# Tony-Tseng/deep-rawburst-sr

Hardware: AMD Instinct MI355X
Metric: bursts/sec 14x48x48 RAW->4x (SyntheticBurstVal shape), DBSR forward (higher is better)
Workload: dtype fp16; 1 GPU; configs[1]: SyntheticBurstVal 14-frame 48x48 -> 384x384 (sr x8 of RAW, x4 of full-res), batch 8 per GPU, full PWC-Net + warp + fusion + decoder; global_batch=8, frames=14, height=48, width=48, out_size=384, parallelism=dp1 (independent bursts per rank), hip_graph=True, fusion_weights_written=True

## Files before the change

deep-rawburst-sr_amd/_lib.py:

```python
import ctypes
import os

import torch

_HERE = os.path.dirname(os.path.abspath(__file__))
LIB_PATH = os.environ.get('DBSR_HIP_LIB', os.path.join(_HERE, 'libdbsr_hip.so'))

DBSR_F32, DBSR_BF16, DBSR_F16 = 0, 1, 2
ACT_NONE, ACT_RELU, ACT_LRELU = 0, 1, 2
OUT_NHWC, OUT_SHUFFLE, OUT_NCHW_F32 = 0, 1, 2
ABI_VERSION = 23
SRC_F32_NCHW, SRC_U8_NHWC = 0, 1
POST_GAINS, POST_CCM, POST_GAMMA, POST_SMOOTHSTEP = 1, 2, 4, 8
LS_SCALE, LS_GROWTH_TRACKER, LS_FOUND_INF, LS_ADAM_STEP, LS_SKIPPED, LS_WORDS = 0, 1, 2, 3, 4, 8


class FrameMap(ctypes.Structure):
    _fields_ = [('fpg', ctypes.c_int), ('group_stride', ctypes.c_int), ('group_offset', ctypes.c_int),
                ('inner_stride', ctypes.c_int)]


IDENTITY = (1, 1, 0, 1)


class Tensor(ctypes.Structure):
    _fields_ = [('ptr', ctypes.c_void_p), ('dtype', ctypes.c_int), ('img_stride', ctypes.c_longlong),
                ('ld', ctypes.c_int), ('c0', ctypes.c_int), ('map', FrameMap)]


class PwcDenseConv(ctypes.Structure):
    _fields_ = [('w', ctypes.c_void_p), ('bias', ctypes.c_void_p), ('kp', ctypes.c_int), ('cg', ctypes.c_int),
                ('start', ctypes.c_int), ('cout', ctypes.c_int), ('out_off', ctypes.c_int)]


class PwcRefineConv(ctypes.Structure):
    _fields_ = [('w', ctypes.c_void_p), ('bias', ctypes.c_void_p), ('cin', ctypes.c_int), ('cout', ctypes.c_int),
                ('ksize', ctypes.c_int), ('dil', ctypes.c_int)]


class PwcExtConv(ctypes.Structure):
    _fields_ = [('w', ctypes.c_void_p), ('bias', ctypes.c_void_p), ('cin', ctypes.c_int), ('cout', ctypes.c_int),
                ('stride', ctypes.c_int)]


class PackJob(ctypes.Structure):
    _fields_ = [('w', ctypes.c_void_p), ('bias', ctypes.c_void_p), ('w_packed', ctypes.c_void_p),
                ('bias_out', ctypes.c_void_p), ('cout', ctypes.c_int), ('cin', ctypes.c_int), ('kh', ctypes.c_int),
                ('kw', ctypes.c_int), ('dtype', ctypes.c_int), ('shuffle', ctypes.c_int), ('transposed', ctypes.c_int),
                ('lo', ctypes.c_int), ('src_cin', ctypes.c_int), ('pad_', ctypes.c_int), ('blk0', ctypes.c_longlong)]


class ConvDesc(ctypes.Structure):
    _fields_ = [('n_frames', ctypes.c_int),
                ('x', Tensor), ('in_h', ctypes.c_int), ('in_w', ctypes.c_int), ('cin', ctypes.c_int),
                ('w', ctypes.c_void_p), ('bias', ctypes.c_void_p), ('cout', ctypes.c_int), ('kh', ctypes.c_int),
                ('kw', ctypes.c_int), ('stride', ctypes.c_int), ('pad', ctypes.c_int), ('dil', ctypes.c_int),
                ('y', Tensor), ('out_h', ctypes.c_int), ('out_w', ctypes.c_int),
                ('act', ctypes.c_int),
                ('res', Tensor), ('post_act', ctypes.c_int),
                ('out_mode', ctypes.c_int), ('shuffle', ctypes.c_int),
                ('workspace', ctypes.c_void_p), ('workspace_bytes', ctypes.c_size_t), ('precise', ctypes.c_int),
                ('max_blocks', ctypes.c_int), ('gate', Tensor), ('plan_h', ctypes.c_int)]


_lib = None


class DBSRLibError(RuntimeError):
    pass


def lib():
    global _lib
    if _lib is None:
        if not os.path.exists(LIB_PATH):
            raise DBSRLibError('libdbsr_hip.so not found at %s: build it with `make` (or __graft_entry__.build())'
                               % LIB_PATH)
        L = ctypes.CDLL(LIB_PATH)
        c_int, c_void_p, c_float, c_ll, c_size_t = (ctypes.c_int, ctypes.c_void_p, ctypes.c_float,
                                                    ctypes.c_longlong, ctypes.c_size_t)
        sigs = {
            'dbsr_abi_version': ([], c_int),
            'dbsr_last_error': ([], ctypes.c_char_p),
            'dbsr_conv_packed_elems': ([c_int, c_int, c_int, c_int], c_size_t),
            'dbsr_weights_round_diffuse': ([c_void_p, c_int, c_int, c_int, c_int, c_int, c_void_p, c_void_p], c_int),
            'dbsr_conv_pack_weights': ([c_void_p, c_void_p, c_int, c_int, c_int, c_int, c_int, c_int, c_void_p,
                                        c_void_p, c_void_p], c_int),
            'dbsr_pack_batch_prepare': ([ctypes.POINTER(PackJob), c_int], c_ll),
            'dbsr_conv_pack_weights_batch': ([c_void_p, c_int, c_ll, c_void_p], c_int),
            'dbsr_conv2d': ([ctypes.POINTER(ConvDesc), c_void_p], c_int),
            'dbsr_set_conv_algo': ([c_int], c_int),
            'dbsr_conv_kernel_for': ([ctypes.POINTER(ConvDesc)], c_int),
            'dbsr_conv_dispatch_variant': ([ctypes.POINTER(ConvDesc)], c_int),
            'dbsr_conv_lane_reach': ([ctypes.POINTER(ConvDesc), c_int], c_int),
            'dbsr_conv_workspace_bytes': ([ctypes.POINTER(ConvDesc)], c_size_t),
            'dbsr_conv2d_head': ([ctypes.POINTER(ConvDesc), c_void_p, c_void_p, c_int, Tensor, c_void_p], c_int),
            'dbsr_conv_head_ok': ([ctypes.POINTER(ConvDesc)], c_int),
            'dbsr_conv_shuffle_blur': ([ctypes.POINTER(ConvDesc), c_void_p, c_void_p], c_int),
            'dbsr_conv_shuffle_blur_ok': ([ctypes.POINTER(ConvDesc)], c_int),
            'dbsr_resblock': ([ctypes.POINTER(ConvDesc), ctypes.POINTER(ConvDesc), c_void_p], c_int),
            'dbsr_resblock_ok': ([ctypes.POINTER(ConvDesc), ctypes.POINTER(ConvDesc)], c_int),
            'dbsr_resblock_head': ([ctypes.POINTER(ConvDesc), ctypes.POINTER(ConvDesc), c_void_p, c_void_p, c_int, Tensor,
                                    c_void_p], c_int),
            'dbsr_correlation': ([c_int, c_int, c_int, c_int, Tensor, Tensor, Tensor, c_int, c_void_p], c_int),
            'dbsr_correlation_backward': ([c_int, c_int, c_int, c_int, Tensor, Tensor, Tensor, Tensor, c_int, Tensor,
                                           Tensor, c_void_p], c_int),
            'dbsr_backwarp': ([c_int, c_int, c_int, c_int, Tensor, Tensor, c_float, Tensor, c_void_p], c_int),
            'dbsr_warp_bilinear': ([c_int, c_int, c_int, c_int, Tensor, c_void_p, c_ll, Tensor, c_void_p], c_int),
            'dbsr_warp_project': ([c_int, c_int, c_int, c_int, Tensor, c_void_p, c_ll, Tensor, c_void_p, c_void_p, c_int,
                                   Tensor, c_void_p], c_int),
            'dbsr_fuse_relu_norm': ([c_int, c_int, c_int, c_int, Tensor, Tensor, Tensor, Tensor, Tensor, c_void_p], c_int),
            'dbsr_burst_mean': ([c_int, c_int, c_int, c_int, Tensor, Tensor, c_void_p], c_int),
            'dbsr_fuse_softmax': ([c_int, c_int, c_int, c_int, Tensor, Tensor, Tensor, Tensor, Tensor, c_void_p],
                                  c_int),
            'dbsr_conv_fuse_softmax': ([ctypes.POINTER(ConvDesc), c_int, c_int, Tensor, Tensor, Tensor, Tensor,
                                        c_void_p], c_int),
            'dbsr_conv_fuse_relu_norm': ([ctypes.POINTER(ConvDesc), c_int, c_int, Tensor, Tensor, Tensor, Tensor,
                                          c_void_p], c_int),
            'dbsr_conv_fuse_ok': ([ctypes.POINTER(ConvDesc), c_int, c_int], c_int),
            'dbsr_fuse_partial': ([c_int, c_int, c_int, c_int, c_int, Tensor, Tensor, Tensor, c_void_p, c_void_p], c_int),
            'dbsr_fuse_combine': ([c_int, c_int, c_int, c_int, c_void_p, Tensor, c_void_p], c_int),
            'dbsr_conv_transpose_k4s2': ([c_int, c_int, c_int, c_int, c_int, Tensor, c_void_p, c_void_p, Tensor,
                                          c_void_p], c_int),
            'dbsr_pack_burst': ([c_int, c_int, c_int, c_int, c_void_p, Tensor, c_int, c_int, Tensor, c_void_p], c_int),
            'dbsr_flow_finalize': ([c_int, c_int, c_int, c_int, Tensor, c_int, c_int, c_int, c_int, c_void_p, c_float,
                                    Tensor, c_void_p], c_int),
            'dbsr_gauss_blur3': ([c_int, c_int, c_int, c_int, Tensor, c_void_p, Tensor, c_void_p], c_int),
            'dbsr_merge_prep': ([c_int, c_int, c_int, c_int, Tensor, Tensor, c_void_p], c_int),
            'dbsr_pwc_assemble': ([c_int, c_int, c_int, c_int, Tensor, Tensor, Tensor, Tensor, c_void_p], c_int),
            'dbsr_zero': ([c_void_p, c_size_t, c_void_p], c_int),
            'dbsr_nhwc_to_nchw_f32': ([c_int, c_int, c_int, Tensor, c_void_p, c_void_p], c_int),
            'dbsr_conv_wgrad_workspace_bytes': ([c_int, c_int, c_int, c_int, c_int, c_int], c_size_t),
            'dbsr_conv_wgrad': ([c_int, c_int, c_int, Tensor, c_int, Tensor, c_int, c_int, c_void_p, c_int, c_void_p,
                                 c_size_t, c_void_p], c_int),
            'dbsr_set_wgrad_algo': ([c_int], c_int),
            'dbsr_conv_wgrad_bias': ([c_int, c_int, c_int, Tensor, c_int, Tensor, c_int, c_int, c_void_p, c_void_p,
                                      c_int, c_void_p, c_size_t, c_void_p], c_int),
            'dbsr_head_forward': ([c_int, c_int, Tensor, c_int, c_void_p, c_void_p, c_int, c_void_p, c_void_p], c_int),
            'dbsr_head_backward_workspace_bytes': ([c_int, c_int, c_int, c_int], c_size_t),
            'dbsr_head_backward': ([c_int, c_int, Tensor, c_int, Tensor, c_void_p, c_int, Tensor, c_void_p, c_void_p,
                                    c_int, c_void_p, c_size_t, c_void_p], c_int),
            'dbsr_chan_sum_workspace_bytes': ([c_int, c_int, c_int], c_size_t),
            'dbsr_chan_sum': ([c_int, c_int, c_int, Tensor, c_void_p, c_int, c_void_p, c_size_t, c_void_p], c_int),
            'dbsr_l1_loss_backward': ([c_int, c_int, c_int, c_int, c_int, c_void_p, c_void_p, Tensor, c_void_p,
                                       c_void_p, c_size_t, c_void_p], c_int),
            'dbsr_relu_grad': ([c_int, c_int, c_int, c_int, c_void_p, c_void_p, Tensor, c_void_p], c_int),
            'dbsr_unshuffle_gate': ([c_int, c_int, c_int, c_int, c_int, Tensor, Tensor, Tensor, c_void_p], c_int),
            'dbsr_fuse_backward': ([c_int, c_int, c_int, c_int, Tensor, Tensor, Tensor, Tensor, Tensor, Tensor, Tensor,
                                    Tensor, c_void_p], c_int),
            'dbsr_merge_prep_backward': ([c_int, c_int, c_int, c_int, Tensor, Tensor, Tensor, c_void_p], c_int),
            'dbsr_warp_backward': ([c_int, c_int, c_int, c_int, Tensor, c_void_p, c_ll, c_void_p, FrameMap, c_ll,
                                    c_void_p], c_int),
            'dbsr_enc_grad_gate': ([c_int, c_int, c_int, c_int, Tensor, c_void_p, Tensor, Tensor, c_void_p], c_int),
            'dbsr_warp_backward_gather_workspace_bytes': ([c_int, c_int, c_int], c_size_t),
            'dbsr_warp_backward_gather': ([c_int, c_int, c_int, c_int, Tensor, c_void_p, c_ll, Tensor, Tensor, c_void_p,
                                           c_size_t, c_void_p], c_int),
            'dbsr_gate_copy': ([c_int, c_int, c_int, Tensor, Tensor, Tensor, c_void_p], c_int),
            'dbsr_warp_flow_backward': ([c_int, c_int, c_int, c_int, Tensor, Tensor, c_void_p, c_ll, c_void_p, c_ll,
                                         c_int, c_void_p], c_int),
            'dbsr_backwarp_backward': ([c_int, c_int, c_int, c_int, Tensor, Tensor, c_float, Tensor, Tensor, Tensor,
                                        c_void_p], c_int),
            'dbsr_offsets_export': ([c_int, c_int, c_int, c_int, c_void_p, c_ll, c_void_p, c_float, Tensor, c_void_p],
                                    c_int),
            'dbsr_adam_step': ([c_ll, c_void_p, c_void_p, c_void_p, c_void_p, c_float, c_float, c_float, c_float, c_int,
                                c_float, c_void_p], c_int),
            'dbsr_l1_loss_backward_scaled': ([c_int, c_int, c_int, c_int, c_int, c_void_p, c_void_p, c_void_p, Tensor,
                                              c_void_p, c_void_p, c_size_t, c_void_p], c_int),
            'dbsr_grad_unscale_check': ([c_ll, c_void_p, c_void_p, c_void_p], c_int),
            'dbsr_adam_step_guarded': ([c_ll, c_void_p, c_void_p, c_void_p, c_void_p, c_float, c_float, c_float,
                                        c_float, c_float, c_void_p, c_void_p], c_int),
            'dbsr_loss_scale_update': ([c_void_p, c_float, c_float, c_int, c_void_p], c_int),
            'dbsr_dgrad_weights': ([c_void_p, c_int, c_int, c_int, c_int, c_void_p, c_void_p], c_int),
            'dbsr_conv_wgrad_sd_workspace_bytes': ([c_int, c_int, c_int, c_int, c_int, c_int], c_size_t),
            'dbsr_conv_wgrad_sd': ([c_int, c_int, c_int, Tensor, c_int, c_int, c_int, Tensor, c_int, c_int, c_int, c_int,
                                    c_int, c_void_p, c_void_p, c_int, c_void_p, c_size_t, c_void_p], c_int),
            'dbsr_dgrad_sd_packed_elems': ([c_int, c_int, c_int], c_size_t),
            'dbsr_dgrad_sd_pack': ([c_void_p, c_int, c_int, c_int, c_int, c_void_p, c_void_p], c_int),
            'dbsr_conv_dgrad_sd': ([c_int, c_int, c_int, Tensor, c_int, c_int, c_int, Tensor, c_int, c_int, c_int, c_int,
                                    c_int, c_void_p, c_void_p], c_int),
            'dbsr_act_backward': ([c_int, c_int, c_int, c_int, Tensor, Tensor, Tensor, c_void_p], c_int),
            'dbsr_flow_finalize_backward': ([c_int, c_int, c_int, c_int, c_int, c_int, c_int, c_void_p, Tensor,
                                             c_void_p], c_int),
            'dbsr_pwc_dense': ([c_int, c_int, c_int, Tensor, c_int, c_void_p, Tensor, c_void_p], c_int),
            'dbsr_pwc_dense_supported': ([c_int, c_int, c_int], c_int),
            'dbsr_pwc_refine': ([c_int, c_int, c_int, Tensor, c_void_p, Tensor, Tensor, c_void_p], c_int),
            'dbsr_pwc_refine_supported': ([c_int, c_int, c_int], c_int),
            'dbsr_pwc_extract': ([c_int, c_int, c_int, Tensor, c_void_p, c_void_p, c_void_p], c_int),
            'dbsr_pwc_extract_supported': ([c_int, c_int], c_int),
            'dbsr_pwc_level_prep': ([c_int, c_int, c_int, c_int, c_float, Tensor, Tensor, Tensor, Tensor, c_int, Tensor,
                                     c_void_p, c_void_p, c_void_p, c_void_p, c_void_p], c_int),
            'dbsr_pwc_level_prep_supported': ([c_int, c_int, c_int], c_int),
            'dbsr_resize_bilinear': ([c_int, c_int, c_int, c_void_p, c_int, c_int, c_float, c_float, c_float, c_void_p,
                                      c_void_p], c_int),
            'dbsr_gauss_reflect': ([c_int, c_int, c_int, c_int, c_void_p, c_void_p, c_void_p, c_void_p], c_int),
            'dbsr_color_fit': ([c_int, c_int, c_int, c_int, c_void_p, c_void_p, c_void_p, c_void_p], c_int),
            'dbsr_color_apply': ([c_int, c_int, c_int, c_int, c_void_p, c_void_p, c_void_p, c_float, c_void_p, c_int,
                                  c_int, c_float, c_float, c_void_p, c_void_p, c_void_p], c_int),
            'dbsr_aligned_l1_workspace_bytes': ([c_int, c_int, c_int], c_size_t),
            'dbsr_aligned_l1_forward': ([c_int, c_int, c_int, c_int, c_void_p, c_void_p, c_void_p, c_void_p, c_void_p,
                                         c_float, c_void_p, c_void_p, c_void_p, c_void_p, c_size_t, c_void_p], c_int),
            'dbsr_aligned_l1_backward': ([c_int, c_int, c_int, c_void_p, c_void_p, c_void_p, c_void_p, c_void_p,
                                          c_void_p, Tensor, c_void_p, c_size_t, c_void_p], c_int),
            'dbsr_ssim_workspace_bytes': ([c_int, c_int, c_int, c_int, c_int], c_size_t),
            'dbsr_ssim_forward': ([c_int, c_int, c_int, c_int, c_int, c_void_p, c_void_p, c_void_p, c_float, c_void_p,
                                   c_void_p, c_void_p, c_void_p, c_size_t, c_void_p], c_int),
            'dbsr_ssim_backward': ([c_int, c_int, c_int, c_int, c_int, c_void_p, c_void_p, c_void_p, c_float,
                                    c_void_p, c_void_p, c_void_p, c_size_t, c_void_p], c_int),
            'dbsr_unprocess_rgb': ([c_int, c_int, c_int, c_void_p, c_int, c_void_p, c_void_p, c_void_p], c_int),
            'dbsr_burst_synth': ([c_int, c_int, c_int, c_int, c_int, c_int, c_void_p, c_void_p, c_void_p, c_void_p,
                                  c_void_p, c_void_p, c_void_p, c_void_p], c_int),
            'dbsr_postprocess_rgb': ([c_int, c_int, c_int, c_void_p, c_void_p, c_int, c_void_p, c_void_p, c_void_p],
                                     c_int),
        }
        for name, (args, res) in sigs.items():
            fn = getattr(L, name)
            fn.argtypes = args
            fn.restype = res
        if L.dbsr_abi_version() != ABI_VERSION:
            raise DBSRLibError('libdbsr_hip.so ABI %d != expected %d' % (L.dbsr_abi_version(), ABI_VERSION))
        _lib = L
    return _lib


EXPORTED = ['dbsr_abi_version', 'dbsr_last_error', 'dbsr_conv_packed_elems', 'dbsr_conv_pack_weights',
            'dbsr_pack_batch_prepare', 'dbsr_conv_pack_weights_batch',
            'dbsr_weights_round_diffuse', 'dbsr_fuse_relu_norm', 'dbsr_burst_mean', 'dbsr_conv2d',
            'dbsr_set_conv_algo', 'dbsr_conv_kernel_for', 'dbsr_conv_dispatch_variant', 'dbsr_conv_lane_reach', 'dbsr_conv_workspace_bytes', 'dbsr_conv2d_head',
            'dbsr_conv_head_ok', 'dbsr_conv_shuffle_blur', 'dbsr_conv_shuffle_blur_ok', 'dbsr_resblock', 'dbsr_resblock_ok', 'dbsr_resblock_head',
            'dbsr_correlation', 'dbsr_correlation_backward', 'dbsr_backwarp', 'dbsr_warp_bilinear', 'dbsr_warp_project', 'dbsr_fuse_softmax',
            'dbsr_fuse_partial', 'dbsr_fuse_combine', 'dbsr_conv_fuse_softmax', 'dbsr_conv_fuse_relu_norm', 'dbsr_conv_fuse_ok',
            'dbsr_conv_transpose_k4s2', 'dbsr_pack_burst', 'dbsr_flow_finalize', 'dbsr_gauss_blur3',
            'dbsr_merge_prep', 'dbsr_pwc_assemble', 'dbsr_zero', 'dbsr_nhwc_to_nchw_f32', 'dbsr_conv_wgrad_workspace_bytes', 'dbsr_conv_wgrad', 'dbsr_conv_wgrad_bias', 'dbsr_set_wgrad_algo', 'dbsr_head_forward', 'dbsr_head_backward_workspace_bytes', 'dbsr_head_backward',
            'dbsr_chan_sum_workspace_bytes', 'dbsr_chan_sum', 'dbsr_l1_loss_backward', 'dbsr_relu_grad', 'dbsr_unshuffle_gate',
            'dbsr_fuse_backward', 'dbsr_merge_prep_backward', 'dbsr_warp_backward', 'dbsr_enc_grad_gate',
            'dbsr_warp_backward_gather_workspace_bytes', 'dbsr_warp_backward_gather', 'dbsr_gate_copy',
            'dbsr_warp_flow_backward', 'dbsr_backwarp_backward', 'dbsr_offsets_export',
            'dbsr_adam_step', 'dbsr_dgrad_weights',
            'dbsr_conv_wgrad_sd_workspace_bytes', 'dbsr_conv_wgrad_sd', 'dbsr_dgrad_sd_packed_elems',
            'dbsr_dgrad_sd_pack', 'dbsr_conv_dgrad_sd', 'dbsr_act_backward', 'dbsr_flow_finalize_backward',
            'dbsr_l1_loss_backward_scaled', 'dbsr_grad_unscale_check', 'dbsr_adam_step_guarded',
            'dbsr_loss_scale_update',
            'dbsr_resize_bilinear', 'dbsr_gauss_reflect', 'dbsr_color_fit', 'dbsr_color_apply', 'dbsr_pwc_dense',
            'dbsr_pwc_dense_supported', 'dbsr_pwc_refine', 'dbsr_pwc_refine_supported', 'dbsr_pwc_extract',
            'dbsr_pwc_extract_supported', 'dbsr_pwc_level_prep', 'dbsr_pwc_level_prep_supported',
            'dbsr_aligned_l1_workspace_bytes', 'dbsr_aligned_l1_forward', 'dbsr_aligned_l1_backward',
            'dbsr_ssim_workspace_bytes', 'dbsr_ssim_forward', 'dbsr_ssim_backward',
            'dbsr_unprocess_rgb', 'dbsr_burst_synth', 'dbsr_postprocess_rgb']


def check(rc, what):
    if rc != 0:
        msg = lib().dbsr_last_error().decode(errors='replace')
        raise DBSRLibError('%s failed (rc=%d): %s' % (what, rc, msg))


def dtype_code(dt):
    if dt == torch.float32:
        return DBSR_F32
    if dt == torch.bfloat16:
        return DBSR_BF16
    if dt == torch.float16:
        return DBSR_F16
    raise ValueError('unsupported dtype %s' % dt)


def tensor_desc(t, ld, c0=0, img_stride=None, fmap=IDENTITY, dtype=None):
    if t is None:
        return Tensor(None, 0, 0, 0, 0, FrameMap(1, 1, 0, 1))
    if img_stride is None:
        img_stride = t[0].numel() if t.dim() > 1 else t.numel()
    return Tensor(t.data_ptr(), dtype_code(t.dtype if dtype is None else dtype), int(img_stride), int(ld), int(c0),
                  FrameMap(*fmap))


NULL_TENSOR = Tensor(None, 0, 0, 0, 0, FrameMap(1, 1, 0, 1))


def stream_ptr(device=None):
    return torch.cuda.current_stream(device).cuda_stream
```

deep-rawburst-sr_amd/csrc/conv2d.hip:

```cpp
#include "conv_core.hpp"

#include <algorithm>
#include <type_traits>
#include <cstdlib>
#include <cstring>
#include <vector>

using namespace dbsr;

namespace {

int g_tiled_enabled = 1;

const dbsr_conv_desc* sel_view(const dbsr_conv_desc* d, dbsr_conv_desc& v) {
    if (d->plan_h <= 0 || d->plan_h == d->out_h) return d;
    v = *d;
    v.in_h = d->in_h + (d->plan_h - d->out_h) * d->stride;
    v.out_h = d->plan_h;
    return &v;
}

__host__ __device__ __forceinline__ int pipe_lane_ch(int cb, int h, int g, int cout) {
    const int c = cb + 32 * h + 8 * g;
    return c < cout ? c : cb;
// ... 986 lines not shown
                    for (int it = 0; it < C::PER; ++it)
                        if ((it * 8) / C::PER == tap) dma(it, nxt, nc, nbuf);
                }
            };
            auto read_frags = [&](int tap, Frag<T> (&a)[WM / 16], Frag<T> (&bq)[C::GW]) {
                const int ky = tap / 3, kx = tap % 3;
#pragma unroll
                for (int i = 0; i < WM / 16; ++i) a[i].v = __builtin_bit_cast(bf16x8_t, lb_w[(tap * (WM / 16) + i) * 64]);
#pragma unroll
                for (int j = 0; j < C::GW; ++j) {
                    const int imm = (j / C::GPR + ky) * C::HWD + (j % C::GPR) * 16 + kx;
                    bq[j].v = __builtin_bit_cast(bf16x8_t, lb_st[in_base[imm & 7] + 4 * imm]);
                }
            };
            auto mfmas = [&](const Frag<T> (&a)[WM / 16], const Frag<T> (&bq)[C::GW]) {
#pragma unroll
                for (int i = 0; i < WM / 16; ++i)
#pragma unroll
                    for (int j = 0; j < C::GW; ++j) acc[i][j] = mma(a[i], bq[j], acc[i][j]);
            };
            Frag<T> a0[WM / 16], b0[C::GW], a1[WM / 16], b1[C::GW];
            read_frags(0, a0, b0);
#pragma unroll
            for (int tap = 0; tap < 9; tap += 2) {
                if (tap == 6) PIPE_STAMP(5 + s * 5);
                vmem(tap);
                if (tap + 1 < 9) read_frags(tap + 1, a1, b1);
                mfmas(a0, b0);
                if (tap + 1 < 9) {
                    vmem(tap + 1);
                    if (tap + 2 < 9) read_frags(tap + 2, a0, b0);
                    mfmas(a1, b1);
                }
            }
            PIPE_STAMP(6 + s * 5);
            if (last) {
                prev = cur;
                cur = nxt;
            }
        }
    }
    dma_barrier();
    epilogue(prev);
#pragma unroll
    for (int q = 0; q < C::NOUT; ++q) store_piece(q, prev);
    PIPE_STAMP(1);
}

int g_num_cus = 0;
int num_cus() {
    if (g_num_cus == 0) {
        int dev = 0, n = 0;
        if (hipGetDevice(&dev) == hipSuccess && hipDeviceGetAttribute(&n, hipDeviceAttributeMultiprocessorCount, dev) == hipSuccess && n > 0)
            g_num_cus = n;
        else
            g_num_cus = 256;
    }
    return g_num_cus;
}

template <typename T, int WM, int TW, int TH>
int launch_pipe(const ConvK& k, int n_frames, hipStream_t s) {
    const int tiles_x = (k.out_w + TW - 1) / TW, tiles_y = (k.out_h + TH - 1) / TH;
    const int nct = (k.cout + WM - 1) / WM;
    const long long nt = (long long)n_frames * tiles_x * tiles_y * nct;
    if (nt >= (1LL << 31)) {
        dbsr_set_error("conv2d: grid too large");
        return DBSR_E_ARG;
    }
    const int cap = k.max_blocks > 0 ? std::min(k.max_blocks, num_cus()) : num_cus();
    int grid = (int)std::min<long long>(nt, cap);
    grid = (grid + 7) / 8 * 8;
    int epi = 0;
    if (k.gt) epi = (TW == 32 && TH == 16) ? 5 : 0;
    else if (k.head_cout > 0) epi = 4;
    else if (!k.r && k.act == DBSR_ACT_RELU) epi = 1;
    else if (k.r && k.act == DBSR_ACT_NONE && k.post_act == DBSR_ACT_RELU) epi = 2;
    else if (!k.r && k.act == DBSR_ACT_NONE) epi = 3;
    else if (!k.r && k.act == DBSR_ACT_LRELU) epi = 6;
#define DBSR_PIPE_LAUNCH(E)                                                                                    \
    hipLaunchKernelGGL((conv3x3_pipe_kernel<T, WM, TW, TH, E>), dim3(grid), dim3(512), 0, s, k, tiles_x, tiles_y, \
                       nct, (int)nt)
    switch (epi) {
        case 4:
            if constexpr (WM == 32) DBSR_PIPE_LAUNCH(4);
            break;
        case 1: DBSR_PIPE_LAUNCH(1); break;
        case 2: DBSR_PIPE_LAUNCH(2); break;
        case 3: DBSR_PIPE_LAUNCH(3); break;
        case 5:
            if constexpr (TW == 32 && TH == 16) DBSR_PIPE_LAUNCH(5);
            break;
        case 6: DBSR_PIPE_LAUNCH(6); break;
        default: DBSR_PIPE_LAUNCH(0); break;
    }
#undef DBSR_PIPE_LAUNCH
    DBSR_LAUNCH_CHECK();
    return 0;
}

int g_pipe_enabled = 1;
int pick_pipe(const dbsr_conv_desc* d) {
    if (!g_pipe_enabled || !is16(d->x.dtype) || d->precise || d->kh != 3 || d->kw != 3 || d->stride != 1 ||
        d->pad != 1 || d->dil != 1 || d->cin <= 16 || d->out_mode != DBSR_OUT_NHWC || d->y.dtype != d->x.dtype)
        return 0;
    if (d->y.ld % 8 || d->y.c0 % 8 || d->cout % 8 || (d->res.ptr && (d->res.ld % 8 || d->res.c0 % 8))) return 0;
    if (d->gate.ptr && (d->gate.ld % 8 || d->gate.c0 % 8 || d->gate.dtype != d->y.dtype)) return 0;
    if (cin_pad(d->cin) * 2 + 64 > ZERO_PAGE_BYTES || d->cout > 512) return 0;
    if ((long long)d->in_h * d->in_w * d->x.ld * 2 >= (1LL << 31)) return 0;
    int cfg = 0, tw = 0, th = 8, wm = 0;
    if (d->cout > 32 && d->out_w % 48 == 0) { cfg = 1; tw = 48; wm = 64; }
    else if (d->cout <= 32 && d->out_w % 64 == 0) { cfg = 2; tw = 64; wm = 32; }
    else if (d->cout > 32 && d->out_w == 16 && d->out_h == 16) { cfg = 3; tw = 16; th = 16; wm = 64; }
    else if (d->cout > 32 && d->out_w % 32 == 0 && d->out_h % 16 == 0) { cfg = 4; tw = 32; th = 16; wm = 64; }
    if (!cfg || d->out_h % th) return 0;
    const long long nt = (long long)d->n_frames * (d->out_w / tw) * (d->out_h / th) * ((d->cout + wm - 1) / wm);
    return (nt >= (cfg == 3 ? 64 : 256) || g_pipe_enabled == 2) ? cfg : 0;
}
bool pipe_fits(int cfg, const dbsr_conv_desc* g) {
    if (cfg == 3) return g->out_h == 16;
    return g->out_h % (cfg == 4 ? 16 : 8) == 0;
}

template <int WM, int TW, int TH, int NCH>
struct WsCfg {
    static constexpr int NWAVES = 8;
    static constexpr int WC = WM / 32;
    static constexpr int WP = NWAVES / WC;
    static constexpr int RPW = TH / WP;
    static constexpr int GPR = TW / 16;
    static constexpr int GW = RPW * GPR;
    static constexpr int HWD = TW + 2, HHT = TH + 2, NQ = HWD * HHT;
    static constexpr int IN_ITEMS = (NQ + 15) / 16;
    static constexpr int ITEMS = NCH * IN_ITEMS;
    static constexpr int PER = (ITEMS + NWAVES - 1) / NWAVES;
    static constexpr int STAGE_U4 = ITEMS * 64;
    static constexpr int STEPS = NCH * 9;
    static constexpr int DMA_STEPS = (STEPS + 1) / 2;
    static constexpr int SPP = WM / 8;
    static constexpr int RES_U4 = TW * TH * SPP;
    static constexpr int RES_ITEMS = RES_U4 / 64;
    static constexpr int RPER = (RES_ITEMS + NWAVES - 1) / NWAVES;
    static_assert(TH % WP == 0 && TW % 16 == 0 && (WM == 64 || WM == 32), "tile shape");
    static constexpr int W_PIECES = (WM / 16) * NCH * 9;
    static constexpr int W_PER = (W_PIECES + NWAVES - 1) / NWAVES;
    static_assert((2 * STAGE_U4 + 2 * RES_U4 + WM / 4) * 16 <= 160 * 1024, "halo + residual stages must fit the LDS");
    static_assert((STAGE_U4 + W_PIECES * 64 + WM / 4) * 16 <= 160 * 1024, "weight staging must fit the LDS");
};

template <typename T, int WM, int TW, int TH, int NCH, int EPI>
__global__ __launch_bounds__(512, 1) void conv3x3_ws_kernel(ConvK k, int tiles_x, int tiles_y, int nct, int nsp,
                                                            int px) {
    using C = WsCfg<WM, TW, TH, NCH>;
    static_assert(EPI >= 0 && EPI <= 5 && EPI != 4, "epilogues 0-3, 5");
    DBSR_OWN_SIMDS();
    constexpr int RES_BUFS = (EPI == 0 || EPI == 2 || EPI == 5) ? 2 : 0;
    constexpr int DMA_STEPS = RES_BUFS > 0 ? C::DMA_STEPS : (2 * C::STEPS) / 3;
    constexpr int BUF_U4 = 2 * C::STAGE_U4 + RES_BUFS * C::RES_U4;
    constexpr int STG_U4 = C::STAGE_U4 + C::W_PIECES * 64;
    __shared__ __attribute__((aligned(16))) u32x4_t lds[(BUF_U4 > STG_U4 ? BUF_U4 : STG_U4) + WM / 4];
    u32x4_t* lres = lds + 2 * C::STAGE_U4;
    float* lbias = (float*)(lds + (BUF_U4 > STG_U4 ? BUF_U4 : STG_U4));

    const int lane = threadIdx.x & 63, wave = __builtin_amdgcn_readfirstlane(threadIdx.x >> 6);
    const int g = lane >> 4, col = lane & 15;
    const int wc = wave % C::WC, wp = wave / C::WC;
    const bool has_res = EPI == 2 || ((EPI == 0 || EPI == 5) && k.r != nullptr);
    const bool has_gate = EPI == 5;
    auto act1 = [&](float v) {
        if constexpr (EPI == 1) return fmaxf(v, 0.f);
        else if constexpr (EPI == 0 || EPI == 5) return apply_act(v, k.act);
        else return v;
    };
    auto act2 = [&](float v) {
        if constexpr (EPI == 2) return fmaxf(v, 0.f);
        else if constexpr (EPI == 0 || EPI == 5) return apply_act(v, k.post_act);
        else return v;
    };

    const int b = blockIdx.x, slot = b >> 3, spx = px / nct;
    const int ct = slot % nct, S = 8 * spx, sid = (b & 7) * spx + slot / nct;
    const int my_tiles = sid < nsp ? (nsp - sid + S - 1) / S : 0;
    if (my_tiles == 0) return;
    PIPE_STAMP(0);

    const int cb = ct * WM + wc * 32;
    {
        const __amdgpu_buffer_rsrc_t w_rsrc = buf_rsrc(k.w_pipe, 0xffffffffu);
        const int p0 = (ct * WM >> 4) * NCH * 9;
#pragma unroll
        for (int it = 0; it < C::W_PER; ++it) {
            const int piece = min(wave + C::NWAVES * it, C::W_PIECES - 1);
            blds16(w_rsrc, lane * 16, (p0 + piece) * 1024, lds + C::STAGE_U4 + piece * 64);
        }
    }
    if (threadIdx.x < WM) {
        const int co = ct * WM + threadIdx.x;
        lbias[threadIdx.x] = (k.bias && co < k.cout) ? k.bias[co] : 0.f;
    }
    const bool cout_ok = cb + 8 * g < k.cout;

    struct Tile { const T* xf; long long y_off, r_off, g_off; int y0, x0; };
    auto decode = [&](int i) {
        int L = sid + i * S;
        const int tx = L % tiles_x; L /= tiles_x;
        const int ty = L % tiles_y;
        const int f = L / tiles_y;
        Tile t;
        t.y0 = ty * TH; t.x0 = tx * TW;
        t.xf = (const T*)k.x + map_frame(k.xm, f) * k.x_is;
        const long long pix = (long long)t.y0 * k.out_w + t.x0;
        t.y_off = map_frame(k.ym, f) * k.y_is + k.y_c0 + cb + pix * k.y_ld;
        t.r_off = has_res ? map_frame(k.rm, f) * k.r_is : 0;
        t.g_off = has_gate ? map_frame(k.gm, f) * k.g_is + k.g_c0 + cb + pix * k.g_ld : 0;
        return t;
    };
    auto px_off = [&](int j) {
        return (long long)(wp * C::RPW + j / C::GPR) * k.out_w + (j % C::GPR) * 16 + col;
    };

    const int pix_b = k.x_ld * (int)sizeof(T);
    const unsigned frame_bytes = (unsigned)((long long)k.in_h * k.in_w * pix_b);
    int h_rc[C::PER], h_off[C::PER];
#pragma unroll
    for (int it = 0; it < C::PER; ++it) {
        const int item = min(wave + C::NWAVES * it, C::ITEMS - 1);
        const int cch = item / C::IN_ITEMS, ii = item - cch * C::IN_ITEMS;
        const int p = ii * 16 + (lane >> 2), ph = lane & 3;
        const int gg = 2 * ((ph & 1) ^ ((p >> 2) & 1)) + (ph >> 1);
        const int r = p / C::HWD, cc = p - r * C::HWD;
        h_rc[it] = p < C::NQ ? (r << 16) | cc : 0x7fff7fff;
        h_off[it] = (r * k.in_w + cc) * pix_b + cch * 64 + gg * 16;
    }
    auto dma = [&](int it, const Tile& t, int buf) {
        const int item = min(wave + C::NWAVES * it, C::ITEMS - 1);
        const int hy = t.y0 - 1 + (h_rc[it] >> 16), hx = t.x0 - 1 + (h_rc[it] & 0xffff);
        const bool ok = (unsigned)hy < (unsigned)k.in_h && (unsigned)hx < (unsigned)k.in_w;
        const int base = ((t.y0 - 1) * k.in_w + (t.x0 - 1)) * pix_b;
        blds16(buf_rsrc(t.xf, frame_bytes), ok ? base + h_off[it] : BUF_OOB, 0, lds + buf * C::STAGE_U4 + item * 64);
    };

    const int P0 = wp * C::RPW * C::HWD + col;
    int in_base[8];
#pragma unroll
    for (int rho = 0; rho < 8; ++rho) in_base[rho] = 4 * P0 + halo_phys(P0 + rho, g);
    auto read_b = [&](const u32x4_t* lb, int step, int j) {
        const int c = step / 9, tap = step % 9, ky = tap / 3, kx = tap % 3;
        const int imm = (j / C::GPR + ky) * C::HWD + (j % C::GPR) * 16 + kx;
        Frag<T> f;
        f.v = __builtin_bit_cast(bf16x8_t, lb[c * C::IN_ITEMS * 64 + in_base[imm & 7] + 4 * imm]);
        return f;
    };

    f32x4_t acc[2][C::GW];
    const unsigned rframe_bytes = (unsigned)((long long)k.out_h * k.out_w * k.r_ld * (int)sizeof(T));
    const int r_cb = k.r_c0 + ct * WM;
    auto res_dma = [&](int it, const Tile& t, int buf) {
        const int q = min(wave + C::NWAVES * it, C::RES_ITEMS - 1);
        const int pp = q * (64 / C::SPP) + lane / C::SPP, ls = (lane % C::SPP) ^ (pp % C::SPP);
        const int off = (((t.y0 + pp / TW) * k.out_w + t.x0 + pp % TW) * k.r_ld + r_cb + ls * 8) * (int)sizeof(T);
        blds16(buf_rsrc((const T*)k.r + t.r_off, rframe_bytes), off, 0, lres + buf * C::RES_U4 + q * 64);
    };
    u32x4_t packed[C::GW];
    auto epilogue = [&](const Tile& t, int rbuf) {
        u32x4_t gatev[EPI == 5 ? C::GW : 1];
        if constexpr (EPI == 5) {
#pragma unroll
            for (int j = 0; j < C::GW; ++j)
                gatev[j] = *(const u32x4_t*)((const T*)k.gt + t.g_off + px_off(j) * k.g_ld +
                                             (ws_lane_ch(ct * WM, wc, g, k.cout) - cb));
        }
        const float4 b0 = *(const float4*)(lbias + wc * 32 + 8 * g);
        const float4 b1 = *(const float4*)(lbias + wc * 32 + 8 * g + 4);
        const float bv[8] = {b0.x, b0.y, b0.z, b0.w, b1.x, b1.y, b1.z, b1.w};
#pragma unroll
        for (int j = 0; j < C::GW; ++j) {
            float v[8];
#pragma unroll
            for (int r = 0; r < 4; ++r) {
                v[r] = act1(acc[0][j][r] + bv[r]);
                v[4 + r] = act1(acc[1][j][r] + bv[4 + r]);
            }
            if (has_res) {
                const int pp = (wp * C::RPW + j / C::GPR) * TW + (j % C::GPR) * 16 + col;
                const u32x4_t rq = lres[rbuf * C::RES_U4 + pp * C::SPP + ((wc * 4 + g) ^ (pp % C::SPP))];
#pragma unroll
                for (int e = 0; e < 4; ++e) {
                    v[2 * e] = act2(v[2 * e] + H16<T>::lo(rq[e]));
                    v[2 * e + 1] = act2(v[2 * e + 1] + H16<T>::hi(rq[e]));
                }
            }
            if constexpr (EPI == 5) {
#pragma unroll
                for (int e = 0; e < 4; ++e) {
                    v[2 * e] = H16<T>::lo(gatev[j][e]) > 0.f ? v[2 * e] : 0.f;
                    v[2 * e + 1] = H16<T>::hi(gatev[j][e]) > 0.f ? v[2 * e + 1] : 0.f;
                }
            }
#pragma unroll
            for (int e = 0; e < 4; ++e) packed[j][e] = H16<T>::pack(v[2 * e], v[2 * e + 1]);
        }
    };
    auto store = [&](const Tile& t) {
#pragma unroll
        for (int j = 0; j < C::GW; ++j)
            if (cout_ok) *(u32x4_t*)((T*)k.y + t.y_off + px_off(j) * k.y_ld + 8 * g) = packed[j];
    };

    Tile cur = decode(0), prev = cur;
#pragma unroll
    for (int it = 0; it < C::PER; ++it) dma(it, cur, 0);
    dma_barrier();
    Frag<T> wr[NCH][9][2];
#pragma unroll
    for (int c = 0; c < NCH; ++c)
#pragma unroll
        for (int tap = 0; tap < 9; ++tap)
#pragma unroll
            for (int h = 0; h < 2; ++h)
                wr[c][tap][h].v = __builtin_bit_cast(
                    bf16x8_t, lds[C::STAGE_U4 + (((wc * 2 + h) * NCH + c) * 9 + tap) * 64 + lane]);

    PIPE_STAMP(2);
    for (int ti = 0; ti < my_tiles; ++ti) {
        PIPE_STAMP(3 + ti * 5);
        vm_drain();
        PIPE_STAMP(4 + ti * 5);
        __syncthreads();
        PIPE_STAMP(5 + ti * 5);
        const bool more = ti + 1 < my_tiles;
        if (ti > 0) store(prev);
        PIPE_STAMP(6 + ti * 5);
        const Tile nxt = more ? decode(ti + 1) : cur;
        const u32x4_t* lb = lds + (ti & 1) * C::STAGE_U4;
        const int nbuf = (ti + 1) & 1;
        Frag<T> bq[C::GW];
#pragma unroll
        for (int j = 0; j < C::GW; ++j) bq[j] = read_b(lb, 0, j);
#pragma unroll
        for (int step = 0; step < C::STEPS; ++step) {
            if (more) {
#pragma unroll
                for (int it = 0; it < C::PER; ++it)
                    if ((it * DMA_STEPS) / C::PER == step) dma(it, nxt, nbuf);
            }
            if constexpr (RES_BUFS > 0) {
                if (has_res && ti == 0) {
#pragma unroll
                    for (int it = 0; it < C::RPER; ++it)
                        if (it == step) res_dma(it, cur, 0);
                }
                if (has_res && more) {
#pragma unroll
                    for (int it = 0; it < C::RPER; ++it)
                        if (DMA_STEPS + (it * (C::STEPS - 2 - DMA_STEPS)) / C::RPER == step)
                            res_dma(it, nxt, nbuf);
                }
            }
            const int c = step / 9, tap = step % 9;
#pragma unroll
            for (int j = 0; j < C::GW; ++j) {
                const f32x4_t z = {0.f, 0.f, 0.f, 0.f};
                acc[0][j] = mma(wr[c][tap][0], bq[j], step == 0 ? z : acc[0][j]);
                acc[1][j] = mma(wr[c][tap][1], bq[j], step == 0 ? z : acc[1][j]);
                if (step + 1 < C::STEPS) bq[j] = read_b(lb, step + 1, j);
            }
#pragma unroll
            for (int j = 0; j < C::GW; ++j) {
                __builtin_amdgcn_sched_group_barrier(0x008, 2, 0);
                __builtin_amdgcn_sched_group_barrier(0x100, 1, 0);
            }
        }
        PIPE_STAMP(7 + ti * 5);
        if constexpr (RES_BUFS > 0) {
            if (has_res && ti == 0) {
                dma_barrier();
            }
        }
        epilogue(cur, ti & 1);
        prev = cur;
        cur = nxt;
    }
    store(prev);
    PIPE_STAMP(1);
}

int g_ws_enabled = 1;
inline bool ws_narrow(const dbsr_conv_desc* d) { return d->cout <= 32; }
inline bool ws_short(const dbsr_conv_desc* d) {
    if (d->gate.ptr && d->cout > 32 && d->cin > 32) return true;
    return !ws_narrow(d) && d->cin > 32 && d->out_w % 16 == 0 && d->out_h % 16 == 0 &&
           (long long)d->n_frames * (d->out_w / 16) * (d->out_h / 16) * ((d->cout + 63) / 64) < 128;
}
int pick_ws(const dbsr_conv_desc* d, const dbsr_conv_desc* g = nullptr) {
    if (!g_ws_enabled || !is16(d->x.dtype) || d->precise || d->kh != 3 || d->kw != 3 || d->stride != 1 ||
        d->pad != 1 || d->dil != 1 || d->cin <= 16 || d->cin > 64 || d->out_mode != DBSR_OUT_NHWC ||
        d->y.dtype != d->x.dtype)
        return 0;
    if (d->gate.ptr && (d->gate.ld % 8 || d->gate.c0 % 8 || d->gate.dtype != d->y.dtype)) return 0;
    if (d->y.ld % 8 || d->y.c0 % 8 || d->cout % 8 || d->cout > 512 ||
        (d->res.ptr && (d->res.ld % 8 || d->res.c0 % 8)))
        return 0;
    const bool narrow = ws_narrow(d);
    const int tw = narrow ? 64 : 16, th = (narrow || ws_short(d)) ? 8 : 16, wm = narrow ? 32 : 64;
    if (narrow && (d->cout < 16 || d->cin > 32)) return 0;
    if (d->out_w % tw || d->out_h % th) return 0;
    if ((long long)d->in_h * d->in_w * d->x.ld * 2 >= (1LL << 31)) return 0;
    if (d->res.ptr && (long long)d->out_h * d->out_w * d->res.ld * 2 >= (1LL << 31)) return 0;
    const int nct = (d->cout + wm - 1) / wm;
    const long long nsp = (long long)d->n_frames * (d->out_w / tw) * (d->out_h / th);
    const int cus = d->max_blocks > 0 ? std::min(d->max_blocks, num_cus()) : num_cus();
    if (cus / 8 / nct < 1 || nsp * nct < 64) return 0;
    if (!g) g = d;
    if (g->out_h % th) return -1;
    const long long nsp_g = (long long)g->n_frames * (g->out_w / tw) * (g->out_h / th);
    const long long want = (nsp_g + 7) / 8;
    const long long spx = std::max<long long>(1, std::min<long long>(cus / 8 / nct, want));
    return (int)(spx * nct);
}

template <typename T, int WM, int TW, int TH, int NCH>
int launch_ws(const ConvK& k, const dbsr_conv_desc* d, int px, hipStream_t s) {
    const int tiles_x = k.out_w / TW, tiles_y = k.out_h / TH;
    const int nct = (k.cout + WM - 1) / WM;
    const int nsp = d->n_frames * tiles_x * tiles_y;
    int epi = 0;
    if (k.gt) epi = 5;
    else if (!k.r && k.act == DBSR_ACT_RELU) epi = 1;
    else if (k.r && k.act == DBSR_ACT_NONE && k.post_act == DBSR_ACT_RELU) epi = 2;
    else if (!k.r && k.act == DBSR_ACT_NONE) epi = 3;
#define DBSR_WS_LAUNCH(E)                                                                                         \
    hipLaunchKernelGGL((conv3x3_ws_kernel<T, WM, TW, TH, NCH, E>), dim3(8 * px), dim3(512), 0, s, k, tiles_x,    \
                       tiles_y, nct, nsp, px)
    switch (epi) {
        case 1: DBSR_WS_LAUNCH(1); break;
        case 2: DBSR_WS_LAUNCH(2); break;
        case 3: DBSR_WS_LAUNCH(3); break;
        case 5: DBSR_WS_LAUNCH(5); break;
        default: DBSR_WS_LAUNCH(0); break;
    }
#undef DBSR_WS_LAUNCH
    DBSR_LAUNCH_CHECK();
    return 0;
}

int g_ks128_enabled = 1;
bool use_ks128(const dbsr_conv_desc* d) {
    if (!g_ks128_enabled || !is16(d->x.dtype) || d->precise || d->kh != 3 || d->kw != 3 || d->stride != 1 ||
        d->pad != 1 || d->dil != 1 || cin_pad(d->cin) != 128 || d->cout != 128 || d->out_mode != DBSR_OUT_NHWC ||
        d->y.dtype != d->x.dtype)
        return false;
    if (d->y.ld % 8 || d->y.c0 % 8 || (d->res.ptr && (d->res.ld % 8 || d->res.c0 % 8))) return false;
    if (d->gate.ptr && (d->gate.ld % 8 || d->gate.c0 % 8 || d->gate.dtype != d->y.dtype)) return false;
    if (d->out_w % ks128::TW || d->out_h % ks128::TH || (d->plan_h > 0 && d->plan_h != d->out_h)) return false;
    if ((long long)d->in_h * d->in_w * d->x.ld * 2 >= (1LL << 31)) return false;
    return (long long)d->n_frames * (d->out_w / ks128::TW) * (d->out_h / ks128::TH) >= 128;
}
int launch_ks128(const ConvK& k, const dbsr_conv_desc* d, hipStream_t s) {
    int epi = 0;
    if (k.gt) epi = 5;
    else if (!k.r && k.act == DBSR_ACT_RELU) epi = 1;
    else if (k.r && k.act == DBSR_ACT_NONE && k.post_act == DBSR_ACT_RELU) epi = 2;
    else if (!k.r && k.act == DBSR_ACT_NONE) epi = 3;
    return ks128_launch(k, d->n_frames, d->x.dtype == DBSR_F16, epi, k.max_blocks, num_cus(), s);
}

namespace rbk {
constexpr int TW = 32, TH = 16;
constexpr int MW = TW + 2, MH = TH + 2, MPX = MW * MH;
constexpr int IW = TW + 4, IH = TH + 4, IPX = IW * IH;
constexpr int IN_PIECES = (IPX + 15) / 16;
constexpr int IN_U4 = IN_PIECES * 64;
constexpr int G1 = (MPX + 15) / 16;
constexpr int MID_U4 = G1 * 16 * 4;
constexpr int G2 = TW * TH / 16;
constexpr int NW = 8;
constexpr int PER = (IN_PIECES + NW - 1) / NW;
constexpr int Q1 = (G1 + NW - 1) / NW;
constexpr int Q2 = G2 / NW;
constexpr int NG = 2;
constexpr int LDS_BYTES = (2 * IN_U4 + MID_U4) * 16 + 64 * 4;
static_assert(LDS_BYTES <= 160 * 1024, "resblock LDS");
}

template <typename T, bool HEAD>
__global__ __launch_bounds__(512, 1) void resblock32_kernel(ConvK k1, ConvK k2, int tiles_x, int tiles_y,
                                                            int ntiles) {
    using namespace rbk;
    DBSR_OWN_SIMDS();
    __shared__ __attribute__((aligned(16))) u32x4_t lds[2 * IN_U4 + MID_U4 + 16 + 34];
    u32x4_t* lmid = lds + 2 * IN_U4;
    float* lbias = (float*)(lds + 2 * IN_U4 + MID_U4);
    float* lhead = lbias + 64;
    const int lane = threadIdx.x & 63, wave = __builtin_amdgcn_readfirstlane(threadIdx.x >> 6);
    const int H = k1.in_h, W = k1.in_w;

    Frag<T> w1[9][2], w2[9][2];
#pragma unroll
    for (int tap = 0; tap < 9; ++tap)
#pragma unroll
        for (int h = 0; h < 2; ++h) {
            w1[tap][h].load((const T*)((const char*)k1.w_pipe + (h * 9 + tap) * 1024 + lane * 16));
            w2[tap][h].load((const T*)((const char*)k2.w_pipe + (h * 9 + tap) * 1024 + lane * 16));
        }
    if (threadIdx.x < 64) {
        const ConvK& kb = threadIdx.x < 32 ? k1 : k2;
        lbias[threadIdx.x] = kb.bias ? kb.bias[threadIdx.x & 31] : 0.f;
    }
    if constexpr (HEAD) {
        if (threadIdx.x < 128) lhead[threadIdx.x] = (int)threadIdx.x < k2.head_cout * 32 ? k2.head_w[threadIdx.x] : 0.f;
        if (threadIdx.x < 4)
            lhead[128 + threadIdx.x] = (k2.head_b && (int)threadIdx.x < k2.head_cout) ? k2.head_b[threadIdx.x] : 0.f;
    }

    struct Tile { const T* xf; long long y_off; int y0, x0; };
    auto decode = [&](int i) {
        const int t = rb_tile(i, blockIdx.x, gridDim.x, ntiles);
        Tile tl;
        const int tx = t % tiles_x, r = t / tiles_x, ty = r % tiles_y, f = r / tiles_y;
        tl.y0 = ty * TH; tl.x0 = tx * TW;
        tl.xf = (const T*)k1.x + map_frame(k1.xm, f) * k1.x_is;
        tl.y_off = HEAD ? map_frame(k2.ym, f) * k2.y_is + (long long)tl.y0 * W + tl.x0
                        : map_frame(k2.ym, f) * k2.y_is + k2.y_c0 + ((long long)tl.y0 * W + tl.x0) * k2.y_ld;
        return tl;
    };
    const int my_tiles = ntiles / (int)gridDim.x + ((int)blockIdx.x < ntiles % (int)gridDim.x ? 1 : 0);
    const int pix_b = k1.x_ld * (int)sizeof(T);
    const unsigned frame_bytes = (unsigned)((long long)H * W * pix_b);
    const unsigned lds0 = (unsigned)(unsigned long long)(__attribute__((address_space(3))) u32x4_t*)lds;
    auto dma = [&](const Tile& tl, int buf) {
        int ln = lane;
        asm volatile("" : "+v"(ln));
#pragma unroll
        for (int it = 0; it < PER; ++it) {
            const int piece = min(wave + NW * it, IN_PIECES - 1);
            const int p = piece * 16 + (ln >> 2), ph = ln & 3;
            const int gg = 2 * ((ph & 1) ^ ((p >> 2) & 1)) + (ph >> 1);
            const int r = p / IW, c = p - r * IW;
            const int hy = tl.y0 - 2 + r, hx = tl.x0 - 2 + c;
            const bool ok = p < IPX && (unsigned)hy < (unsigned)H && (unsigned)hx < (unsigned)W;
            lds_dma16(tl.xf, frame_bytes, ok ? (hy * W + hx) * pix_b + gg * 16 : BUF_OOB, 0,
                      lds0 + (buf * IN_U4 + piece * 64) * 16);
        }
    };

    auto taps = [&](const u32x4_t* img, int iw, int g, const auto& P0, const Frag<T> (&w)[9][2], auto& acc) {
        constexpr int NB = std::extent<std::remove_reference_t<decltype(P0)>>::value;
        int bs[NB][8];
#pragma unroll
        for (int j = 0; j < NB; ++j)
#pragma unroll
            for (int rho = 0; rho < 8; ++rho) bs[j][rho] = 4 * P0[j] + halo_phys(P0[j] + rho, g);
        Frag<T> bq[NB][3];
        auto rd = [&](int j, int tap) {
            const int imm = (tap / 3) * iw + tap % 3;
            Frag<T> b;
            b.v = __builtin_bit_cast(bf16x8_t, img[bs[j][imm & 7] + 4 * imm]);
            return b;
        };
#pragma unroll
        for (int j = 0; j < NB; ++j) {
            bq[j][0] = rd(j, 0);
            bq[j][1] = rd(j, 1);
        }
        StaticFor<0, 9>::run([&](auto t_) {
            constexpr int tap = decltype(t_)::value;
            const f32x4_t z = {0.f, 0.f, 0.f, 0.f};
#pragma unroll
            for (int j = 0; j < NB; ++j) {
                acc[j][0] = mma(w[tap][0], bq[j][tap % 3], tap == 0 ? z : acc[j][0]);
                acc[j][1] = mma(w[tap][1], bq[j][tap % 3], tap == 0 ? z : acc[j][1]);
                if constexpr (tap + 2 < 9) bq[j][(tap + 2) % 3] = rd(j, tap + 2);
            }
        });
        __builtin_amdgcn_iglp_opt(0);
    };

    auto store_out = [&](const Tile& tl, int i, int g, int col, const u32x4_t& o) {
        const int q = wave + NW * i;
        const long long px = (long long)(q >> 1) * W + 16 * (q & 1) + col;
        if constexpr (HEAD) {
            if (g < k2.head_cout) ((float*)k2.y)[tl.y_off + px + (long long)g * H * W] = __uint_as_float(o[0]);
        } else {
            *(u32x4_t*)((T*)k2.y + tl.y_off + px * k2.y_ld + 8 * g) = o;
        }
    };
    Tile cur = decode(0), prev = cur;
    if (my_tiles > 0) dma(cur, 0);
    u32x4_t outv[Q2];
    for (int ti = 0; ti < my_tiles; ++ti) {
        dma_barrier();
        int ln = lane;
        asm volatile("" : "+v"(ln));
        const int g = ln >> 4, col = ln & 15;
        if (ti > 0) {
#pragma unroll
            for (int i = 0; i < Q2; ++i) store_out(prev, i, g, col, outv[i]);
        }
// ... 76 lines not shown
                        float hs[4];
#pragma unroll
                        for (int c = 0; c < 4; ++c) {
                            const float4 w0 = *(const float4*)(lhead + c * 32 + 8 * g);
                            const float4 w1 = *(const float4*)(lhead + c * 32 + 8 * g + 4);
                            float a = v[0] * w0.x;
                            a = fmaf(v[1], w0.y, a); a = fmaf(v[2], w0.z, a); a = fmaf(v[3], w0.w, a);
                            a = fmaf(v[4], w1.x, a); a = fmaf(v[5], w1.y, a); a = fmaf(v[6], w1.z, a);
                            a = fmaf(v[7], w1.w, a);
                            a += __shfl_xor(a, 16, 64);
                            a += __shfl_xor(a, 32, 64);
                            hs[c] = a;
                        }
                        const float hv = g == 0 ? hs[0] : g == 1 ? hs[1] : g == 2 ? hs[2] : hs[3];
                        o = u32x4_t{__float_as_uint(fmaxf(hv + lhead[128 + g], 0.f)), 0u, 0u, 0u};
                    } else {
#pragma unroll
                        for (int e = 0; e < 4; ++e)
                            o[e] = relu16x2(H16<T>::pack(v[2 * e] + H16<T>::lo(rq[e]), v[2 * e + 1] + H16<T>::hi(rq[e])));
                    }
                    outv[NG * bt + j] = o;
                }
            });
        }
        prev = cur;
        cur = nxt;
    }
    if (my_tiles > 0) {
#pragma unroll
        for (int i = 0; i < Q2; ++i) store_out(prev, i, lane >> 4, lane & 15, outv[i]);
    }
    vm_drain();
}

void tensor_span(const dbsr_tensor& t, int n, long long per_img, int es, unsigned long long& lo,
                 unsigned long long& hi) {
    long long mn = 0, mx = 0;
    for (int f = 0; f < n; ++f) {
        const long long img = (long long)(f / t.map.fpg) * t.map.group_stride + t.map.group_offset +
                              (long long)(f % t.map.fpg) * t.map.inner_stride;
        if (f == 0 || img < mn) mn = img;
        if (f == 0 || img > mx) mx = img;
    }
    const unsigned long long base = (unsigned long long)(uintptr_t)t.ptr;
    lo = base + (unsigned long long)((mn * t.img_stride + t.c0) * es);
    hi = base + (unsigned long long)((mx * t.img_stride + per_img) * es);
}
bool resblock_out_disjoint(const dbsr_conv_desc* c1, const dbsr_conv_desc* c2, const dbsr_tensor* head_out,
                           int head_cout) {
    const long long hw = (long long)c1->in_h * c1->in_w;
    const int C = c1->cin;
    unsigned long long xl, xh, yl, yh;
    tensor_span(c1->x, c1->n_frames, (hw - 1) * c1->x.ld + c1->x.c0 + C, 2, xl, xh);
    if (head_out) tensor_span(*head_out, c1->n_frames, (long long)head_cout * hw, 4, yl, yh);
    else tensor_span(c2->y, c1->n_frames, (hw - 1) * c2->y.ld + c2->y.c0 + C, 2, yl, yh);
    return yh <= xl || xh <= yl;
}

int resblock_channels(const dbsr_conv_desc* c1, const dbsr_conv_desc* c2) {
    if (!c1 || !c2) return 0;
    const int C = c1->cin;
    if (C != 32 && C != 64) return 0;
    auto conv_ok = [C](const dbsr_conv_desc* d) {
        return is16(d->x.dtype) && d->y.dtype == d->x.dtype && !d->precise && d->kh == 3 && d->kw == 3 &&
               d->stride == 1 && d->pad == 1 && d->dil == 1 && d->cin == C && d->cout == C &&
               d->out_mode == DBSR_OUT_NHWC && !d->gate.ptr && d->in_h == d->out_h && d->in_w == d->out_w;
    };
    if (!conv_ok(c1) || !conv_ok(c2)) return 0;
    if (c1->act != DBSR_ACT_RELU || c1->res.ptr || c2->act != DBSR_ACT_NONE || c2->post_act != DBSR_ACT_RELU)
        return 0;
    if (c2->res.ptr != c1->x.ptr || c2->res.c0 != c1->x.c0 || c2->res.ld != c1->x.ld ||
        c2->res.img_stride != c1->x.img_stride || c2->res.dtype != c1->x.dtype ||
        std::memcmp(&c2->res.map, &c1->x.map, sizeof(dbsr_frame_map)) != 0)
        return 0;
    if (c1->n_frames != c2->n_frames || c1->in_h != c2->in_h || c1->in_w != c2->in_w || c1->x.dtype != c2->y.dtype)
        return 0;
    if (C == 32 ? (c1->in_w % rbk::TW || c1->in_h % rbk::TH) : (c1->in_w % rb64::TW || c1->in_h % rb64::TH)) return 0;
    if (C == 64) {
        const long long tiles = (long long)c1->n_frames * (c1->in_w / rb64::TW) * (c1->in_h / rb64::TH);
        const int cus = c1->max_blocks > 0 ? std::min(c1->max_blocks, num_cus()) : num_cus();
        if (tiles > 2LL * cus) return 0;
    }
    if (c1->x.ld % 8 || c1->x.c0 % 8 || c1->x.c0 + C > c1->x.ld) return 0;
    if (c2->y.ld % 8 || c2->y.c0 % 8 || c2->y.c0 + C > c2->y.ld) return 0;
    return (long long)c1->in_h * c1->in_w * c1->x.ld * 2 < (1LL << 31) ? C : 0;
}

template <typename T>
int dispatch_ws(int px, const ConvK& k, const dbsr_conv_desc* d, const dbsr_conv_desc* sel, hipStream_t s) {
    if (ws_narrow(sel)) return launch_ws<T, 32, 64, 8, 1>(k, d, px, s);
    if (ws_short(sel)) return launch_ws<T, 64, 16, 8, 2>(k, d, px, s);
    if (k.CG / 4 == 1) return launch_ws<T, 64, 16, 16, 1>(k, d, px, s);
    return launch_ws<T, 64, 16, 16, 2>(k, d, px, s);
}

template <typename T>
int dispatch_pipe(int cfg, const ConvK& k, const dbsr_conv_desc* d, hipStream_t s) {
    if (cfg == 1) return launch_pipe<T, 64, 48, 8>(k, d->n_frames, s);
    if (cfg == 3) return launch_pipe<T, 64, 16, 16>(k, d->n_frames, s);
    if (cfg == 4) return launch_pipe<T, 64, 32, 16>(k, d->n_frames, s);
    return launch_pipe<T, 32, 64, 8>(k, d->n_frames, s);
}

template <typename T, int MT, int NT, typename XT = T>
int launch_conv(const ConvK& k0, hipStream_t s) {
    ConvK k = k0;
    k.stage_epi = MT * NT >= 2 && sizeof(T) == 2 && sizeof(XT) == 2 && k.ksplit == 1 &&
                  k.out_mode == DBSR_OUT_NHWC && !k.y_f32 && !k.r && !k.gt && k.cout % 8 == 0 && k.y_ld % 8 == 0 &&
                  k.y_c0 % 8 == 0 && k.head_cout == 0;
    dim3 grid((k.npix + 4 * NT * 16 - 1) / (4 * NT * 16), (k.cout + MT * 16 - 1) / (MT * 16), k.ksplit);
    hipLaunchKernelGGL((conv2d_kernel<T, MT, NT, XT>), grid, dim3(256), 0, s, k);
    DBSR_LAUNCH_CHECK();
    if (k.ksplit > 1) {
        const long long n = (long long)k.npix * (k.cw / 4);
        hipLaunchKernelGGL((conv_splitk_finalize<T>), dim3((unsigned)((n + 255) / 256)), dim3(256), 0, s, k);
        DBSR_LAUNCH_CHECK();
    }
    return 0;
}

int choose_ksplit(const ConvK& k, int mt, int nt) {
    const long long blocks = (long long)((k.npix + 64 * nt - 1) / (64 * nt)) * ((k.cout + 16 * mt - 1) / (16 * mt));
    const int nks = k.KGp >> 2;
    const long long target = nks >= 64 ? 1024 : 512;
    if (blocks >= target / 2 || nks < 16) return 1;
    int sp = (int)((target + blocks - 1) / blocks);
    sp = std::min(sp, nks / 8);
    sp = std::min(sp, 32);
    return std::max(sp, 1);
}
size_t splitk_bytes(const ConvK& k, int sp) {
    return sp > 1 ? (size_t)sp * k.npix * k.cw * sizeof(float) : 0;
}
void pick_generic_tile(const ConvK& k, int& best_m, int& best_n) {
    const int mts[3] = {4, 2, 1}, nts[3] = {4, 2, 1};
    const long long minb = 512;
    best_m = 1;
    best_n = 1;
    for (int a = 0; a < 3; ++a) {
        if (mts[a] > 1 && k.cout <= (mts[a] / 2) * 16) continue;
        for (int b = 0; b < 3; ++b) {
            const long long blocks = (long long)((k.npix + 64 * nts[b] - 1) / (64 * nts[b])) *
                                     ((k.cout + 16 * mts[a] - 1) / (16 * mts[a]));
            if (blocks >= minb) {
                best_m = mts[a];
                best_n = nts[b];
                return;
            }
        }
    }
}

template <typename T>
__global__ __launch_bounds__(256) void conv3x3_small_kernel(ConvK k, int groups_x, long long ngroups) {
    const int lane = threadIdx.x & 63, g = lane >> 4, col = lane & 15;
    const int nco = k.cout / 16;
    Frag<T> a[4][3];
    f32x4_t bias[4];
#pragma unroll
    for (int b = 0; b < 4; ++b) {
        bias[b] = load_bias4(k, min(b, nco - 1) * 16 + g * 4);
#pragma unroll
        for (int st = 0; st < 3; ++st)
            a[b][st].load((const T*)k.w + (long long)(min(b, nco - 1) * 16 + col) * k.Kp + 32 * st + 8 * g);
    }
    const long long wave0 = ((long long)blockIdx.x * blockDim.x + threadIdx.x) >> 6;
    const long long nwaves = ((long long)gridDim.x * blockDim.x) >> 6;
    for (long long gi = wave0; gi < ngroups; gi += nwaves) {
        const int gx = (int)(gi % groups_x);
        const long long r = gi / groups_x;
        const int y = (int)(r % k.out_h), f = (int)(r / k.out_h);
        const int x = gx * 16 + col;
        const T* xf = (const T*)k.x + map_frame(k.xm, f) * k.x_is;
        Frag<T> bq[3];
#pragma unroll
        for (int st = 0; st < 3; ++st) {
            const int tap = 4 * st + g, ky = tap / 3, kx = tap - 3 * (tap / 3);
            const int iy = y + ky - 1, ix = x + kx - 1;
            if (tap < 9 && (unsigned)iy < (unsigned)k.in_h && (unsigned)ix < (unsigned)k.in_w)
                bq[st].load(xf + ((long long)iy * k.in_w + ix) * k.x_ld);
            else
                bq[st].zero();
        }
        f32x4_t acc[4];
#pragma unroll
        for (int b = 0; b < 4; ++b) {
            acc[b] = f32x4_t{0.f, 0.f, 0.f, 0.f};
#pragma unroll
            for (int st = 0; st < 3; ++st) acc[b] = mma(a[b][st], bq[st], acc[b]);
        }
        if (x < k.out_w) {
            T* yp = (T*)k.y + map_frame(k.ym, f) * k.y_is + k.y_c0 + ((long long)y * k.out_w + x) * k.y_ld + 4 * g;
#pragma unroll
            for (int b = 0; b < 4; ++b) {
                if (b >= nco) break;
                uint2 o;
                o.x = H16<T>::pack(apply_act(acc[b][0] + bias[b][0], k.act), apply_act(acc[b][1] + bias[b][1], k.act));
                o.y = H16<T>::pack(apply_act(acc[b][2] + bias[b][2], k.act), apply_act(acc[b][3] + bias[b][3], k.act));
                *(uint2*)(yp + 16 * b) = o;
            }
        }
    }
}

int g_small_enabled = 1;
bool use_small(const dbsr_conv_desc* d) {
    return g_small_enabled && is16(d->x.dtype) && !d->precise && d->kh == 3 && d->kw == 3 && d->stride == 1 &&
           d->pad == 1 && d->dil == 1 && d->cin <= 8 && d->cout % 16 == 0 && d->cout <= 64 &&
           d->out_mode == DBSR_OUT_NHWC && d->y.dtype == d->x.dtype && d->y.ld % 4 == 0 && d->y.c0 % 4 == 0 &&
           !d->res.ptr && !d->gate.ptr;
}
template <typename T>
int launch_small(const ConvK& k, const dbsr_conv_desc* d, hipStream_t s) {
    const int gx = (d->out_w + 15) / 16;
    const long long ng = (long long)d->n_frames * d->out_h * gx;
    const long long want = (ng + 15) / 16;
    const unsigned grid = (unsigned)std::max<long long>(1, std::min<long long>(want, 4096));
    hipLaunchKernelGGL((conv3x3_small_kernel<T>), dim3(grid), dim3(256), 0, s, k, gx, ng);
    DBSR_LAUNCH_CHECK();
    return 0;
}

int g_narrow_enabled = 1;
bool use_narrow(const dbsr_conv_desc* d) {
    return g_narrow_enabled && is16(d->x.dtype) && !d->precise && d->kh == 3 && d->kw == 3 && d->stride == 1 &&
           d->pad == 1 && d->dil == 1 && d->cout <= 4 && d->cin >= 256 && d->out_mode == DBSR_OUT_NHWC &&
           !d->gate.ptr;
}
template <typename T>
int launch_narrow(const ConvK& k, const dbsr_conv_desc* d, hipStream_t s) {
    const int tiles_x = (d->out_w + 15) / 16, tiles_y = (d->out_h + 3) / 4;
    const long long blocks = (long long)d->n_frames * tiles_x * tiles_y;
    DBSR_CHECK_ARG(blocks < (1LL << 31), "conv2d: too many narrow tiles");
    hipLaunchKernelGGL((conv3x3_narrow_kernel<T>), dim3((unsigned)blocks), dim3(256), 0, s, k, tiles_x, tiles_y);
    DBSR_LAUNCH_CHECK();
    return 0;
}

bool use_tiled(const dbsr_conv_desc* d) {
    const bool bf = is16(d->x.dtype);
    const bool dil_ok = (d->dil == 1 || d->dil == 2 || d->dil == 4 || (d->dil == 8 && bf)) && d->pad == d->dil;
    return !d->precise && cin_pad(d->cin) * (bf ? 2 : 4) + 64 <= ZERO_PAGE_BYTES && d->kh == 3 && d->kw == 3 &&
           d->stride == 1 && dil_ok && d->cin > 16 && d->out_h >= 8 && d->out_w >= 8 &&
           d->out_mode == DBSR_OUT_NHWC && g_tiled_enabled;
}

int tiled_blocks(const dbsr_conv_desc* d, int wm, int wn) {
    const int th = 4 * wn / 16;
    return d->n_frames * ((d->out_w + 15) / 16) * ((d->out_h + th - 1) / th) * ((d->cout + wm - 1) / wm);
}
#ifndef DBSR_TILE_WM32_MAX_COUT
#define DBSR_TILE_WM32_MAX_COUT 64
#endif
void pick_tiled_tile(const dbsr_conv_desc* d, int& wm, int& wn) {
    wm = d->cout <= 32 ? 32 : 64;
    wn = (wm == 32 && d->out_h >= 32) ? 128 : 64;
    if (tiled_blocks(d, wm, wn) >= 512) return;
    if (wm == 64) {
        if (d->cout > DBSR_TILE_WM32_MAX_COUT && d->out_w > 8) return;
        wm = 32;
        if (tiled_blocks(d, wm, wn) >= 512) return;
    }
    wn = 64;
    if (tiled_blocks(d, wm, wn) >= 512) return;
    wn = 16;
}

int g_tiled_split_enabled = 1;
int tiled_ksplit(const dbsr_conv_desc* d, int& wm, int& wn) {
    if (!g_tiled_split_enabled || !is16(d->x.dtype) || d->dil != 1 || d->cout < 64) return 1;
    const int nch = cin_pad(d->cin) / 32;
    const int wm0 = 64;
    const int nb = tiled_blocks(d, wm0, 64);
    if (nb >= 256 || nch < 8) return 1;
    const int sp = std::min(nch / 2, (512 + nb - 1) / nb);
    if (sp < 2) return 1;
    wm = wm0;
    wn = 64;
    return sp;
}

template <typename T, int D>
int dispatch_tiled_d(const ConvK& k0, const dbsr_conv_desc* d, const dbsr_conv_desc* sel, hipStream_t s) {
    int wm, wn;
    pick_tiled_tile(sel, wm, wn);
    ConvK k = k0;
    k.ksplit = tiled_ksplit(sel, wm, wn);
    if (k.ksplit > 1 && splitk_bytes(k, k.ksplit) > d->workspace_bytes) {
        k.ksplit = 1;
        pick_tiled_tile(sel, wm, wn);
    }
    if (wm == 64) return launch_tiled<T, 64, 64, D>(k, d->n_frames, s);
    if (wn == 128) return launch_tiled<T, 32, 128, D>(k, d->n_frames, s);
    if (wn == 64) return launch_tiled<T, 32, 64, D>(k, d->n_frames, s);
    return launch_tiled<T, 32, 16, D>(k, d->n_frames, s);
}

ConvK make_convk(const dbsr_conv_desc* d);

int slab_misfit(const dbsr_conv_desc* d, const dbsr_conv_desc* sel) {
    dbsr_set_error("conv2d: a %d-row slab cannot take the tile chosen for plan_h = %d rows (use a multiple of 16)",
                   d->out_h, sel->out_h);
    return DBSR_E_ARG;
}

template <typename T>
int dispatch_conv(const ConvK& k, const dbsr_conv_desc* d, const dbsr_conv_desc* sel, hipStream_t s) {
    if constexpr (sizeof(T) == 2) {
        const int px = pick_ws(sel, d);
        if (px < 0) return slab_misfit(d, sel);
        if (px) return dispatch_ws<T>(px, k, d, sel, s);
        if (use_ks128(sel)) return launch_ks128(k, d, s);
        const int cfg = pick_pipe(sel);
        if (cfg && !pipe_fits(cfg, d)) return slab_misfit(d, sel);
        if (cfg) return dispatch_pipe<T>(cfg, k, d, s);
        if (use_narrow(sel)) return launch_narrow<T>(k, d, s);
        if (use_small(sel)) return launch_small<T>(k, d, s);
    }
    if (use_tiled(sel)) {
        switch (d->dil) {
            case 1: return dispatch_tiled_d<T, 1>(k, d, sel, s);
            case 2: return dispatch_tiled_d<T, 2>(k, d, sel, s);
            case 4: return dispatch_tiled_d<T, 4>(k, d, sel, s);
            default:
                if constexpr (sizeof(T) == 2) return dispatch_tiled_d<T, 8>(k, d, sel, s);
                dbsr_set_error("conv2d: no fp32 tile for dilation %d", d->dil);
                return DBSR_E_ARG;
        }
    }
    int best_m, best_n;
    const ConvK ksel = sel == d ? k : make_convk(sel);
    pick_generic_tile(ksel, best_m, best_n);
    ConvK kk = k;
    kk.ksplit = choose_ksplit(ksel, best_m, best_n);
    if (kk.ksplit > 1 && splitk_bytes(k, kk.ksplit) > d->workspace_bytes) kk.ksplit = 1;
#define DBSR_CONV_CASE(M, N) if (best_m == M && best_n == N) return launch_conv<T, M, N>(kk, s);
    DBSR_CONV_CASE(4, 4) DBSR_CONV_CASE(4, 2) DBSR_CONV_CASE(4, 1)
    DBSR_CONV_CASE(2, 4) DBSR_CONV_CASE(2, 2) DBSR_CONV_CASE(2, 1)
    DBSR_CONV_CASE(1, 4) DBSR_CONV_CASE(1, 2) DBSR_CONV_CASE(1, 1)
#undef DBSR_CONV_CASE
    return launch_conv<T, 1, 1>(kk, s);
}

template <typename T, int PG, int KS>
__global__ __launch_bounds__(512) void upsample_shuffle_kernel(ConvK k) {
    const int lane = threadIdx.x & 63, wave = threadIdx.x >> 6;
    const int g = lane >> 4, col = lane & 15;
    const int s = k.shuffle, s2 = s * s;
    const int hw = k.out_h * k.out_w;
    Frag<T> b[PG][KS];
    int pf[PG], py[PG], px[PG];
#pragma unroll
    for (int j = 0; j < PG; ++j) {
        const int p = blockIdx.x * (PG * 16) + j * 16 + col;
        const bool ok = p < k.npix;
        const int f = ok ? p / hw : 0, rr = ok ? p - f * hw : 0;
        pf[j] = ok ? f : -1;
        py[j] = rr / k.out_w;
        px[j] = rr - py[j] * k.out_w;
        const T* xp = (const T*)k.x + map_frame(k.xm, f) * k.x_is + (long long)rr * k.x_ld + g * 8;
#pragma unroll
        for (int ks = 0; ks < KS; ++ks) {
            if (ok) b[j][ks].load(xp + ks * 32);
            else b[j][ks].zero();
        }
    }
    const int m_row = 8 * (col >> 2) + (col & 3);
    auto load_a = [&](int sub, Frag<T> (&a)[2][KS]) {
#pragma unroll
        for (int h = 0; h < 2; ++h)
#pragma unroll
// ... 559 lines not shown
        pick_tiled_tile(sel, wm, wn);
        return splitk_bytes(make_convk(d), tiled_ksplit(sel, wm, wn));
    }
    if (kf != 0) return 0;
    const ConvK ksel = make_convk(sel);
    int m, n;
    pick_generic_tile(ksel, m, n);
    return splitk_bytes(make_convk(d), choose_ksplit(ksel, m, n));
}

extern "C" int dbsr_set_conv_algo(int algo) {
    DBSR_CHECK_ARG(algo >= 0 && algo <= 5, "set_conv_algo: 0 generic, 1 two-barrier tiled, 2 weight-stationary + "
                   "K-split 128-channel + pipelined + tiled (default), 3 pipelined wherever the shape allows, 4 as 2 "
                   "without the weight-stationary kernels, 5 as 2 without the K-split 128-channel kernel");
    g_tiled_enabled = algo >= 1;
    g_pipe_enabled = algo == 3 ? 2 : algo >= 2 ? 1 : 0;
    g_ws_enabled = algo == 2 || algo == 5;
    g_ks128_enabled = algo == 2;
    g_narrow_enabled = algo >= 2;
    g_small_enabled = algo >= 2;
    return 0;
}

inline bool has_pipe_copy(int cin, int kh, int kw) { return kh == 3 && kw == 3 && cin > 16; }

extern "C" size_t dbsr_conv_packed_elems(int cout, int cin, int kh, int kw) {
    const int KGp = round_up(kh * kw * (cin_pad(cin) / 8), 4);
    const size_t rows = (size_t)round_up(cout, 64) * KGp * 8;
    return has_pipe_copy(cin, kh, kw) ? 2 * rows : rows;
}

extern "C" int dbsr_conv_pack_weights(const float* w_f32, const float* bias_f32, int cout, int cin, int kh, int kw,
                                      int dtype, int shuffle, void* w_packed, float* bias_out, void* stream) {
    DBSR_CHECK_ARG(w_f32 && w_packed, "pack_weights: null pointer");
    DBSR_CHECK_ARG(cout > 0 && cin > 0 && kh > 0 && kw > 0, "pack_weights: bad shape");
    DBSR_CHECK_ARG(dtype == DBSR_F32 || is16(dtype), "pack_weights: bad dtype");
    if (shuffle > 1)
        DBSR_CHECK_ARG(cout % (shuffle * shuffle) == 0 && (cout / (shuffle * shuffle)) % 4 == 0,
                       "pack_weights: cout %d not divisible for shuffle %d", cout, shuffle);
    const int CG = cin_pad(cin) / 8, KG = kh * kw * CG, KGp = round_up(KG, 4), Kp = KGp * 8;
    const int cout_pad = round_up(cout, 64);
    const long long total = (long long)cout_pad * Kp;
    hipLaunchKernelGGL(pack_weights_kernel, dim3((unsigned)((total + 255) / 256)), dim3(256), 0, (hipStream_t)stream,
                       w_f32, bias_f32, cout, cin, kh, kw, CG, KG, Kp, cout_pad, shuffle, dtype,
                       w_packed, bias_out);
    DBSR_LAUNCH_CHECK();
    if (has_pipe_copy(cin, kh, kw) && is16(dtype)) {
        hipLaunchKernelGGL(pack_weights_pipe_kernel, dim3((unsigned)((total + 255) / 256)), dim3(256), 0,
                           (hipStream_t)stream, (const bf16_t*)w_packed, CG, Kp, cout <= 32 ? 32 : 64, total,
                           (bf16_t*)w_packed + total);
        DBSR_LAUNCH_CHECK();
    }
    return 0;
}

extern "C" long long dbsr_pack_batch_prepare(dbsr_pack_job* jobs, int n) {
    if (!jobs || n <= 0) { dbsr_set_error("pack_batch_prepare: no jobs"); return -1; }
    long long blk = 0;
    for (int i = 0; i < n; ++i) {
        dbsr_pack_job& j = jobs[i];
        if (!j.w || !j.w_packed || j.cout <= 0 || j.cin <= 0 || j.kh <= 0 || j.kw <= 0 ||
            !(j.dtype == DBSR_F32 || is16(j.dtype)) || j.shuffle < 1) {
            dbsr_set_error("pack_batch_prepare: bad job %d", i);
            return -1;
        }
        if (j.shuffle > 1 && (j.transposed || j.cout % (j.shuffle * j.shuffle) || (j.cout / (j.shuffle * j.shuffle)) % 4)) {
            dbsr_set_error("pack_batch_prepare: job %d: cout %d not divisible for shuffle %d", i, j.cout, j.shuffle);
            return -1;
        }
        if (j.transposed && (j.lo < 0 || j.src_cin < j.lo + j.cout)) {
            dbsr_set_error("pack_batch_prepare: job %d: rows [%d, %d) past the source's %d input channels", i, j.lo,
                      j.lo + j.cout, j.src_cin);
            return -1;
        }
        const PackGeom g = pack_geom(j);
        j.blk0 = blk;
        blk += ((g.pipe ? 2 : 1) * g.rows + 255) / 256;
    }
    if (blk >= (1LL << 31)) { dbsr_set_error("pack_batch_prepare: too many elements"); return -1; }
    return blk;
}

extern "C" int dbsr_conv_pack_weights_batch(const dbsr_pack_job* jobs_dev, int n, long long n_blocks, void* stream) {
    DBSR_CHECK_ARG(jobs_dev && n > 0 && n_blocks > 0 && n_blocks < (1LL << 31), "pack_weights_batch: bad arguments");
    hipLaunchKernelGGL(pack_weights_batch_kernel, dim3((unsigned)n_blocks), dim3(256), 0, (hipStream_t)stream,
                       jobs_dev, n);
    DBSR_LAUNCH_CHECK();
    return 0;
}

extern "C" int dbsr_conv2d(const dbsr_conv_desc* d, void* stream) {
    DBSR_CHECK_ARG(d, "conv2d: null desc");
    DBSR_CHECK_ARG(d->x.ptr && d->w && d->y.ptr, "conv2d: null pointer");
    DBSR_CHECK_ARG(d->x.dtype == DBSR_F32 || is16(d->x.dtype), "conv2d: bad input dtype");
    DBSR_CHECK_ARG(d->y.dtype == DBSR_F32 || d->y.dtype == d->x.dtype, "conv2d: output dtype must be f32 or input dtype");
    DBSR_CHECK_ARG(d->n_frames > 0 && d->in_h > 0 && d->in_w > 0 && d->out_h > 0 && d->out_w > 0, "conv2d: bad sizes");
    DBSR_CHECK_ARG(d->cin > 0 && d->cout > 0 && d->kh > 0 && d->kw > 0 && d->stride > 0 && d->dil > 0, "conv2d: bad shape");
    DBSR_CHECK_ARG(d->x.ld % 8 == 0 && d->x.c0 % 8 == 0, "conv2d: input ld/c0 must be multiples of 8 (got %d/%d)",
                   d->x.ld, d->x.c0);
    DBSR_CHECK_ARG(d->x.c0 + cin_pad(d->cin) <= d->x.ld, "conv2d: input slice [c0, c0+cin_pad) exceeds ld");
    DBSR_CHECK_ARG(d->x.map.fpg > 0 && d->y.map.fpg > 0, "conv2d: frame map fpg must be > 0");
    DBSR_CHECK_ARG(d->out_h == (d->in_h + 2 * d->pad - d->dil * (d->kh - 1) - 1) / d->stride + 1 &&
                   d->out_w == (d->in_w + 2 * d->pad - d->dil * (d->kw - 1) - 1) / d->stride + 1,
                   "conv2d: output size inconsistent with conv geometry");
    DBSR_CHECK_ARG(d->out_mode >= 0 && d->out_mode <= 2, "conv2d: bad out_mode");
    if (d->out_mode == DBSR_OUT_SHUFFLE) {
        const int s2 = d->shuffle * d->shuffle;
        DBSR_CHECK_ARG(d->shuffle > 1 && d->cout % s2 == 0 && (d->cout / s2) % 4 == 0, "conv2d: bad shuffle");
        DBSR_CHECK_ARG(d->res.ptr == nullptr, "conv2d: residual not supported with shuffle output");
    }
    if (d->out_mode == DBSR_OUT_NHWC) DBSR_CHECK_ARG(d->y.c0 + d->cout <= d->y.ld, "conv2d: output slice exceeds ld");
    if (d->out_mode == DBSR_OUT_NCHW_F32) DBSR_CHECK_ARG(d->y.dtype == DBSR_F32 && !d->res.ptr, "conv2d: NCHW out is f32, no residual");
    if (d->res.ptr) DBSR_CHECK_ARG(d->res.dtype == d->y.dtype && d->res.map.fpg > 0, "conv2d: residual dtype must equal output dtype");
    if (d->gate.ptr)
        DBSR_CHECK_ARG(d->gate.dtype == d->y.dtype && d->gate.map.fpg > 0 && d->out_mode == DBSR_OUT_NHWC && !d->precise,
                       "conv2d: gate must be an NHWC tensor of the output dtype (NHWC output)");
    if (d->res.ptr) DBSR_CHECK_ARG(d->res.c0 + d->cout <= d->res.ld, "conv2d: residual slice exceeds ld");
    if (d->gate.ptr) DBSR_CHECK_ARG(d->gate.c0 + d->cout <= d->gate.ld, "conv2d: gate slice exceeds ld");
    for (int w = 0; w < 3; ++w) {
        const dbsr_tensor& t = w == 0 ? d->y : w == 1 ? d->res : d->gate;
        const int reach = conv_lane_reach(d, w);
        DBSR_CHECK_ARG(reach < t.ld, "conv2d: a lane of the %s would address channel %d of a %d-channel pixel",
                       w == 0 ? "output" : w == 1 ? "residual" : "gate", reach, t.ld);
    }
    const long long npix = (long long)d->n_frames * d->out_h * d->out_w;
    DBSR_CHECK_ARG(npix < (1LL << 31), "conv2d: too many pixels");

    DBSR_CHECK_ARG(d->plan_h >= 0, "conv2d: plan_h must be >= 0");
    ConvK k = make_convk(d);
    hipStream_t s = (hipStream_t)stream;
    dbsr_conv_desc v;
    const dbsr_conv_desc* sel = sel_view(d, v);
    const long long npix_sel = (long long)sel->n_frames * sel->out_h * sel->out_w;
    if (d->precise && d->x.dtype == DBSR_F16) {
        DBSR_CHECK_ARG(d->y.dtype == DBSR_F32 && d->cout <= 16, "conv2d: precise mode needs fp32 output, cout <= 16");
        k.ksplit = 1;
        if (npix_sel >= 512 * 256) return launch_conv<float, 1, 4, f16_t>(k, s);
        if (npix_sel >= 512 * 128) return launch_conv<float, 1, 2, f16_t>(k, s);
        return launch_conv<float, 1, 1, f16_t>(k, s);
    }
    if (d->precise && d->x.dtype == DBSR_BF16) {
        DBSR_CHECK_ARG(d->y.dtype == DBSR_F32 && d->cout <= 16, "conv2d: precise mode needs fp32 output, cout <= 16");
        k.ksplit = 1;
        if (npix_sel >= 512 * 256) return launch_conv<float, 1, 4, bf16_t>(k, s);
        if (npix_sel >= 512 * 128) return launch_conv<float, 1, 2, bf16_t>(k, s);
        return launch_conv<float, 1, 1, bf16_t>(k, s);
    }
    if (use_upsample(sel, k)) return d->x.dtype == DBSR_F16 ? launch_upsample<f16_t>(k, s) : launch_upsample<bf16_t>(k, s);
    if (use_pointwise(sel)) return d->x.dtype == DBSR_F16 ? launch_pointwise<f16_t>(k, s) : launch_pointwise<bf16_t>(k, s);
    if (d->x.dtype == DBSR_F16) return dispatch_conv<f16_t>(k, d, sel, s);
    return d->x.dtype == DBSR_BF16 ? dispatch_conv<bf16_t>(k, d, sel, s) : dispatch_conv<float>(k, d, sel, s);
}

extern "C" int dbsr_resblock_ok(const dbsr_conv_desc* c1, const dbsr_conv_desc* c2) {
    return resblock_channels(c1, c2) && c2->y.ptr && resblock_out_disjoint(c1, c2, nullptr, 0) ? 1 : 0;
}

int resblock_launch(const dbsr_conv_desc* c1, const dbsr_conv_desc* c2, const float* head_w, const float* head_b,
                    int head_cout, const dbsr_tensor* head_out, void* stream) {
    DBSR_CHECK_ARG(c1 && c2 && c1->x.ptr && c1->w && c2->w, "resblock: null pointer");
    DBSR_CHECK_ARG(head_out || c2->y.ptr, "resblock: null output");
    DBSR_CHECK_ARG(c1->x.map.fpg > 0 && c2->y.map.fpg > 0 && c1->n_frames > 0, "resblock: bad frame map / sizes");
    const int C = resblock_channels(c1, c2);
    DBSR_CHECK_ARG(C, "resblock: needs two 16-bit 3x3/s1/p1 C -> C convs, C = 32 or 64 (conv1 ReLU; conv2 residual = "
                   "conv1's input, post-ReLU), frames a multiple of 32 x 16 (C 32) / 16 x 16 (C 64), NHWC slices "
                   "aligned to 8");
    DBSR_CHECK_ARG(!head_out || C == 32, "resblock_head: 32-channel ResBlocks only");
    const ConvK k1 = make_convk(c1);
    ConvK k2 = make_convk(c2);
    if (C == 64) {
        DBSR_CHECK_ARG(resblock_out_disjoint(c1, c2, nullptr, 0),
                       "resblock: the output must not overlap the input x (other blocks still read x's halos)");
        return resblock64_launch(k1, k2, c1->n_frames, c1->x.dtype == DBSR_F16, c1->max_blocks, num_cus(),
                                 (hipStream_t)stream);
    }
    if (head_out) {
        DBSR_CHECK_ARG(head_w && head_out->ptr, "resblock_head: null pointer");
        DBSR_CHECK_ARG(head_cout >= 1 && head_cout <= 4, "resblock_head: head_cout must be 1..4");
        DBSR_CHECK_ARG(head_out->dtype == DBSR_F32 && head_out->map.fpg > 0, "resblock_head: fp32 NCHW output");
        k2.head_w = head_w; k2.head_b = head_b; k2.head_cout = head_cout;
        k2.y = head_out->ptr; k2.y_f32 = 1; k2.y_is = head_out->img_stride; k2.y_ld = 1; k2.y_c0 = 0;
        k2.ym = head_out->map;
    }
    DBSR_CHECK_ARG(resblock_out_disjoint(c1, c2, head_out, head_cout),
                   "resblock: the output must not overlap the input x (other blocks still read x's halos)");
    const int tiles_x = c1->in_w / rbk::TW, tiles_y = c1->in_h / rbk::TH;
    const int ntiles = c1->n_frames * tiles_x * tiles_y;
    int grid = c1->max_blocks > 0 ? std::min(c1->max_blocks, num_cus()) : num_cus();
    grid = std::min(grid, ntiles);
    DBSR_CHECK_ARG(rb_mapping_ok(grid, ntiles), "resblock: tile mapping out of range (grid %d, %d tiles)", grid, ntiles);
    hipStream_t s = (hipStream_t)stream;
    if (k2.head_w) {
        if (c1->x.dtype == DBSR_F16)
            hipLaunchKernelGGL((resblock32_kernel<f16_t, true>), dim3(grid), dim3(512), 0, s, k1, k2, tiles_x, tiles_y, ntiles);
        else
            hipLaunchKernelGGL((resblock32_kernel<bf16_t, true>), dim3(grid), dim3(512), 0, s, k1, k2, tiles_x, tiles_y, ntiles);
    } else {
        if (c1->x.dtype == DBSR_F16)
            hipLaunchKernelGGL((resblock32_kernel<f16_t, false>), dim3(grid), dim3(512), 0, s, k1, k2, tiles_x, tiles_y, ntiles);
        else
            hipLaunchKernelGGL((resblock32_kernel<bf16_t, false>), dim3(grid), dim3(512), 0, s, k1, k2, tiles_x, tiles_y, ntiles);
    }
    DBSR_LAUNCH_CHECK();
    return 0;
}

extern "C" int dbsr_resblock(const dbsr_conv_desc* c1, const dbsr_conv_desc* c2, void* stream) {
    return resblock_launch(c1, c2, nullptr, nullptr, 0, nullptr, stream);
}

extern "C" int dbsr_resblock_head(const dbsr_conv_desc* c1, const dbsr_conv_desc* c2, const float* head_w,
                                  const float* head_b, int head_cout, dbsr_tensor head_out, void* stream) {
    return resblock_launch(c1, c2, head_w, head_b, head_cout, &head_out, stream);
}

extern "C" int dbsr_conv_shuffle_blur_ok(const dbsr_conv_desc* d) { return use_upsample_blur(d) ? 1 : 0; }

extern "C" int dbsr_conv_shuffle_blur(const dbsr_conv_desc* d, const float* k9, void* stream) {
    DBSR_CHECK_ARG(d && k9 && d->x.ptr && d->w && d->y.ptr, "conv_shuffle_blur: null pointer");
    DBSR_CHECK_ARG(d->x.map.fpg > 0 && d->y.map.fpg > 0, "conv_shuffle_blur: frame map fpg must be > 0");
    DBSR_CHECK_ARG(d->n_frames > 0, "conv_shuffle_blur: bad sizes");
    DBSR_CHECK_ARG(use_upsample_blur(d), "conv_shuffle_blur: needs a 16-bit 1x1 conv cin <= 64 -> 2048 with "
                   "PixelShuffle(8) output (32 channels), a low-res frame of multiples of 4, aligned NHWC slices");
    const ConvK k = make_convk(d);
    Blur3 kk;
    DBSR_CHECK_ARG(blur_separable(k9, kk), "conv_shuffle_blur: the blur kernel must be separable (a Gaussian)");
    const int tiles_x = d->in_w / ub::LT, tiles_y = d->in_h / ub::LT;
    const int ntiles = d->n_frames * tiles_x * tiles_y;
    int grid = d->max_blocks > 0 ? std::min(d->max_blocks, num_cus()) : num_cus();
    grid = std::min(grid, ntiles);
    hipStream_t s = (hipStream_t)stream;
#define DBSR_UB(TT, KS, ACT) \
    hipLaunchKernelGGL((upsample_blur_kernel<TT, KS, ACT>), dim3(grid), dim3(512), 0, s, k, kk, tiles_x, tiles_y, ntiles)
#define DBSR_UB_ACT(TT, KS)                                   \
    switch (d->act) {                                         \
        case DBSR_ACT_RELU: DBSR_UB(TT, KS, DBSR_ACT_RELU); break;   \
        case DBSR_ACT_LRELU: DBSR_UB(TT, KS, DBSR_ACT_LRELU); break; \
        default: DBSR_UB(TT, KS, DBSR_ACT_NONE); break;             \
    }
    if (k.Kp == 64) {
        if (d->x.dtype == DBSR_F16) { DBSR_UB_ACT(f16_t, 2) } else { DBSR_UB_ACT(bf16_t, 2) }
    } else {
        if (d->x.dtype == DBSR_F16) { DBSR_UB_ACT(f16_t, 1) } else { DBSR_UB_ACT(bf16_t, 1) }
    }
#undef DBSR_UB_ACT
#undef DBSR_UB
    DBSR_LAUNCH_CHECK();
    return 0;
}

extern "C" int dbsr_conv2d_head(const dbsr_conv_desc* d, const float* head_w, const float* head_b, int head_cout,
                                dbsr_tensor head_out, void* stream) {
    DBSR_CHECK_ARG(d && head_w && head_out.ptr, "conv2d_head: null pointer");
    DBSR_CHECK_ARG(dbsr_conv_head_ok(d), "conv2d_head: the conv must be a pipelined 32-channel ResBlock conv2 "
                   "(bf16 3x3/s1/p1, residual, act none, post-act ReLU, width %% 64 == 0, height %% 8 == 0)");
    DBSR_CHECK_ARG(head_cout >= 1 && head_cout <= 4, "conv2d_head: head_cout must be 1..4");
    DBSR_CHECK_ARG(head_out.dtype == DBSR_F32 && head_out.map.fpg > 0, "conv2d_head: fp32 NCHW output");
    DBSR_CHECK_ARG(d->x.ld % 8 == 0 && d->x.c0 % 8 == 0 && d->x.c0 + cin_pad(d->cin) <= d->x.ld,
                   "conv2d_head: bad input slice");
    DBSR_CHECK_ARG(d->res.dtype == d->x.dtype && d->res.map.fpg > 0, "conv2d_head: residual dtype must equal input dtype");
    ConvK k = make_convk(d);
    k.head_w = head_w; k.head_b = head_b; k.head_cout = head_cout;
    k.y = head_out.ptr; k.y_f32 = 1; k.y_is = head_out.img_stride; k.y_ld = 1; k.y_c0 = 0; k.ym = head_out.map;
    if (d->x.dtype == DBSR_F16) return launch_pipe<f16_t, 32, 64, 8>(k, d->n_frames, (hipStream_t)stream);
    return launch_pipe<bf16_t, 32, 64, 8>(k, d->n_frames, (hipStream_t)stream);
}
```

deep-rawburst-sr_amd/engine.py:

```python
import ctypes
import math
import os
import types

import torch

from . import _lib as L
from ._lib import IDENTITY

BACKWARP_SCALE = {5: 0.625, 4: 1.25, 3: 2.5, 2: 5.0}
PWC_LEVEL_CH = {1: 16, 2: 32, 3: 64, 4: 96, 5: 128, 6: 196}
DENSE_OUT = [128, 128, 96, 64, 32]
DENSE_OFF = [320, 192, 96, 32, 0]
BASE_OFF = 448
REFINER_TAIL = [(128, 128, 3, 2), (128, 128, 3, 4), (128, 96, 3, 8), (96, 64, 3, 16), (64, 32, 3, 1), (32, 2, 3, 1)]


def r8(c):
    return (c + 7) // 8 * 8


def cpad(c):
    return r8(c) if c <= 16 else (c + 31) // 32 * 32

# ... 31 lines not shown
    def __init__(self, n, h, w, ld, dtype, device):
        self.n, self.h, self.w, self.ld, self.dtype = n, h, w, ld, dtype
        self.t = torch.zeros(n, h, w, ld, dtype=dtype, device=device)

    def d(self, c0=0, fmap=IDENTITY):
        return L.tensor_desc(self.t, self.ld, c0, img_stride=self.h * self.w * self.ld, fmap=fmap)

    def rows(self, y0, y1):
        v = NHWC.__new__(NHWC)
        v.n, v.h, v.w, v.ld, v.dtype = self.n, y1 - y0, self.w, self.ld, self.dtype
        v.t = self.t[:, y0:y1]
        v.full_h = self.h
        v.d = lambda c0=0, fmap=IDENTITY: L.tensor_desc(v.t, v.ld, c0, img_stride=self.h * self.w * self.ld,
                                                        fmap=fmap)
        return v


class DBSRAux(dict):

    def __init__(self, offsets, native_fw):
        super().__init__(offsets=offsets, fusion_weights=None)
        self.native_fusion_weights = native_fw
        self._done = native_fw is None

    def _materialize(self):
        if self._done:
            return
        v = self.native_fusion_weights
        B, N, C, H, W = v.shape
        src = v.permute(0, 1, 3, 4, 2)
        out = torch.empty(B, N, C, H, W, dtype=torch.float32, device=v.device)
        L.check(L.lib().dbsr_nhwc_to_nchw_f32(B * N, H * W, C, L.tensor_desc(src, src.stride(-2), 0,
                                                                               img_stride=src.stride(1)),
                                              out.data_ptr(), L.stream_ptr(v.device)), 'dbsr_nhwc_to_nchw_f32')
        dict.__setitem__(self, 'fusion_weights', out)
        self._done = True

    def __getitem__(self, k):
        if k == 'fusion_weights':
            self._materialize()
        return dict.__getitem__(self, k)

    def get(self, k, default=None):
        if k == 'fusion_weights':
            self._materialize()
        return dict.get(self, k, default)

    def items(self):
        self._materialize()
        return dict.items(self)

    def values(self):
        self._materialize()
        return dict.values(self)

    def copy(self):
        self._materialize()
        return dict(self)


class PackedConv:
    def __init__(self, conv, dtype, device, stream, shuffle=1, recipe=None, rounding='nearest'):
        self.recipe = recipe or (lambda: (conv.weight, conv.bias))
        self.dtype, self.device, self.shuffle = dtype, device, shuffle
        self.rounding = rounding if dtype in (torch.float16, torch.bfloat16) else 'nearest'
        w, b = self.recipe()
        self.cout, self.cin, self.kh, self.kw = w.shape
        self.stride, self.pad, self.dil = conv.stride[0], conv.padding[0], conv.dilation[0]
        n = L.lib().dbsr_conv_packed_elems(self.cout, self.cin, self.kh, self.kw)
        self.w = torch.empty(n, dtype=dtype, device=device)
        self.bias = torch.empty(self.cout, dtype=torch.float32, device=device) if b is not None else None
        self.repack(stream)

    def repack(self, stream):
        w, b = self.recipe()
        w = w.detach().to(device=self.device, dtype=torch.float32).contiguous()
        b = b.detach().to(device=self.device, dtype=torch.float32).contiguous() if b is not None else None
        if self.rounding == 'diffuse':
            wr = torch.empty_like(w)
            L.check(L.lib().dbsr_weights_round_diffuse(w.data_ptr(), self.cout, self.cin, self.kh, self.kw,
                                                       L.dtype_code(self.dtype), wr.data_ptr(), stream),
                    'dbsr_weights_round_diffuse')
            w = wr
        L.check(L.lib().dbsr_conv_pack_weights(w.data_ptr(), b.data_ptr() if b is not None else None, self.cout,
                                               self.cin, self.kh, self.kw, L.dtype_code(self.dtype), self.shuffle,
                                               self.w.data_ptr(),
                                               self.bias.data_ptr() if self.bias is not None else None, stream),
                'dbsr_conv_pack_weights')
        self._keep = (w, b)

    def out_hw(self, h, w):
        return ((h + 2 * self.pad - self.dil * (self.kh - 1) - 1) // self.stride + 1,
                (w + 2 * self.pad - self.dil * (self.kw - 1) - 1) // self.stride + 1)


class Plan:
    FORK, JOIN = '__fork__', '__join__'
    MULTI_STREAM = os.environ.get('DBSR_SINGLE_STREAM', '0') != '1'

    def __init__(self):
        self.ops = []
        self.keep = []
        self.work = {}
        self.kernel = {}
        self.hbm = {}
        self.convs = []
        self.lane = 0
        self.lanes = {0}
        self.streams = {}
        self.max_blocks = 0
        self.max_blocks_cap = 0
        self.early_names, self.early_cap = (), 0
        self.plan_rows = None

    def add(self, name, fn, *args, work=None):
        if work is not None:
            self.work[len(self.ops)] = work
        self.ops.append((fn, args, name, self.lane))

    def fork(self, lane, device, priority=0):
        assert self.lane == 0 and lane != 0
        if not Plan.MULTI_STREAM:
            return
        if lane not in self.streams:
            self.streams[lane] = Plan.side_stream(device, lane, priority)
        self.lanes.add(lane)
        self.ops.append((Plan.FORK, (torch.cuda.Event(),), f'sync.fork{lane}', lane))
        self.lane = lane

    _side_streams = {}

    @staticmethod
    def side_stream(device, lane, priority):
        dev = torch.device(device)
        key = (dev.index if dev.index is not None else torch.cuda.current_device(), lane, priority)
        st = Plan._side_streams.get(key)
        if st is None:
            st = Plan._side_streams[key] = torch.cuda.Stream(device=device, priority=priority)
        return st

    def switch(self, lane):
        assert lane == 0 or lane in self.streams or not Plan.MULTI_STREAM
        self.lane = lane if Plan.MULTI_STREAM else 0

    def join(self, lane):
        if not Plan.MULTI_STREAM:
            return
        assert lane != 0 and lane in self.streams
        self.ops.append((Plan.JOIN, (torch.cuda.Event(),), f'sync.join{lane}', lane))
        self.lane = 0

    def conv(self, name, pc, n_frames, x, xc0, in_hw, y, yc0, act, xmap=IDENTITY, ymap=IDENTITY, res=None,
             rc0=0, rmap=IDENTITY, post_act=L.ACT_NONE, out_mode=L.OUT_NHWC, shuffle=0, y_desc=None, cin=None,
             precise=False, head=None, gate=None, gc0=0, gmap=IDENTITY):
        d = self._desc(name, pc, n_frames, x, xc0, in_hw, y, yc0, act, xmap, ymap, res, rc0, rmap, post_act,
                       out_mode, shuffle, y_desc, cin, precise, gate, gc0, gmap)
        self.convs.append((d, self.lane))
        oh, ow = d.out_h, d.out_w
        flop = 2.0 * n_frames * oh * ow * pc.cout * d.cin * pc.kh * pc.kw
        d.fused_head = bool(head is not None and L.lib().dbsr_conv_head_ok(ctypes.byref(d)))
        if d.fused_head:
            hname, hw, hb, hdesc = head
            self.keep.extend([hw, hb, hdesc])
            flop += 2.0 * n_frames * oh * ow * hw.shape[0] * hw.shape[1]
            self.add(name + '+' + hname, L.lib().dbsr_conv2d_head, ctypes.byref(d), hw.data_ptr(),
                     hb.data_ptr() if hb is not None else None, hw.shape[0], hdesc, work=('flop', flop))
            self.kernel[len(self.ops) - 1] = 'conv3x3_pipe'
            return d
        self.add(name, L.lib().dbsr_conv2d, ctypes.byref(d), work=('flop', flop))
        self.kernel[len(self.ops) - 1] = {4: 'conv3x3_ws', 7: 'conv3x3_ks128', 2: 'conv3x3_pipe', 1: 'conv3x3_tiled', 3: 'conv1x1_shuffle', 5: 'conv1x1', 6: 'conv3x3_narrow', 8: 'conv3x3_small'}.get(L.lib().dbsr_conv_kernel_for(d),
                                                                                      'conv2d_generic')
        return d

    def conv_fuse(self, name, pc, B, N, x, in_hw, ref, oth, fused, weights, xmap=IDENTITY, softmax=True):
        d = self._desc(name, pc, B * N, x, 0, in_hw, None, 0, L.ACT_NONE, xmap, IDENTITY, None, 0, IDENTITY,
                       L.ACT_NONE, L.OUT_NHWC, 0, L.NULL_TENSOR, None, False, None, 0, IDENTITY)
        if not L.lib().dbsr_conv_fuse_ok(ctypes.byref(d), B, N):
            return None
        H, W = in_hw
        flop = 2.0 * B * N * H * W * pc.cout * d.cin * pc.kh * pc.kw
        fn = L.lib().dbsr_conv_fuse_softmax if softmax else L.lib().dbsr_conv_fuse_relu_norm
        self.add(name, fn, ctypes.byref(d), B, N, ref, oth, fused, weights,
                 work=('flop', flop))
        self.kernel[len(self.ops) - 1] = 'conv_fuse'
        es, C = (4 if x.dtype == torch.float32 else 2), pc.cout
        self.hbm[len(self.ops) - 1] = es * B * H * W * (N * d.cin + N * C + (N * C if weights.ptr else 0) + C)
        return len(self.ops) - 1

    def resblock(self, name, c1, c2, n_frames, x, mid, y, hw, head=None, yc0=0):
        d1 = self._desc(name + '.conv1', c1, n_frames, x, 0, hw, mid, 0, L.ACT_RELU, IDENTITY, IDENTITY, None, 0,
                        IDENTITY, L.ACT_NONE, L.OUT_NHWC, 0, None, None, False, None, 0, IDENTITY)
        d2 = self._desc(name + '.conv2', c2, n_frames, mid, 0, hw, y, yc0, L.ACT_NONE, IDENTITY, IDENTITY, x, 0,
                        IDENTITY, L.ACT_RELU, L.OUT_NHWC, 0, None, None, False, None, 0, IDENTITY)
        if (c1.cout == 64 and not DBSREngine.FUSED_RESBLOCK64) or \
                not L.lib().dbsr_resblock_ok(ctypes.byref(d1), ctypes.byref(d2)):
            return False
        self.convs.extend([(d1, self.lane), (d2, self.lane)])
        oh, ow = d1.out_h, d1.out_w
        flop = 2.0 * n_frames * oh * ow * (c1.cout * d1.cin * 9 + c2.cout * d2.cin * 9)
        if head is not None:
            hname, hw_, hb, hdesc = head
            self.keep.extend([hw_, hb, hdesc])
            flop += 2.0 * n_frames * oh * ow * hw_.shape[0] * hw_.shape[1]
            self.add(name + '+' + hname, L.lib().dbsr_resblock_head, ctypes.byref(d1), ctypes.byref(d2),
                     hw_.data_ptr(), hb.data_ptr() if hb is not None else None, hw_.shape[0], hdesc,
                     work=('flop', flop))
        else:
            self.add(name, L.lib().dbsr_resblock, ctypes.byref(d1), ctypes.byref(d2), work=('flop', flop))
        self.kernel[len(self.ops) - 1] = 'resblock32' if c1.cout == 32 else 'resblock64'
        self.hbm[len(self.ops) - 1] = n_frames * oh * ow * (2 * d1.cin + (4 * head[1].shape[0] if head is not None
                                                                         else 2 * c2.cout))
        return True

    def conv_shuffle_blur(self, name, pc, n_frames, x, in_hw, y, act, k9):
        d = self._desc(name, pc, n_frames, x, 0, in_hw, y, 0, act, IDENTITY, IDENTITY, None, 0, IDENTITY,
                       L.ACT_NONE, L.OUT_SHUFFLE, pc.shuffle, None, None, False, None, 0, IDENTITY)
        if not L.lib().dbsr_conv_shuffle_blur_ok(ctypes.byref(d)):
            return None
        kbuf = (ctypes.c_float * 9)(*k9)
        self.keep.append(kbuf)
        self.convs.append((d, self.lane))
        flop = 2.0 * n_frames * d.out_h * d.out_w * pc.cout * d.cin
        self.add(name, L.lib().dbsr_conv_shuffle_blur, ctypes.byref(d), kbuf, work=('flop', flop))
        self.kernel[len(self.ops) - 1] = 'conv1x1_shuffle_blur'
        s = pc.shuffle
        self.hbm[len(self.ops) - 1] = 2 * n_frames * d.out_h * d.out_w * (d.cin + pc.cout // (s * s) * s * s)
        return d

    def _desc(self, name, pc, n_frames, x, xc0, in_hw, y, yc0, act, xmap, ymap, res, rc0, rmap, post_act, out_mode,
              shuffle, y_desc, cin, precise, gate, gc0, gmap):
        oh, ow = pc.out_hw(*in_hw)
        assert cin is None or cin == pc.cin, (name, cin, pc.cin)
        d = L.ConvDesc()
        d.n_frames = n_frames
        d.x = x.d(xc0, xmap)
        d.in_h, d.in_w = in_hw
        d.cin = pc.cin if cin is None else cin
        d.w = pc.w.data_ptr()
        d.bias = pc.bias.data_ptr() if pc.bias is not None else None
        d.cout, d.kh, d.kw, d.stride, d.pad, d.dil = pc.cout, pc.kh, pc.kw, pc.stride, pc.pad, pc.dil
        d.y = y_desc if y_desc is not None else y.d(yc0, ymap)
        d.out_h, d.out_w = oh, ow
        d.act = act
        d.res = res.d(rc0, rmap) if res is not None else L.NULL_TENSOR
        d.gate = gate.d(gc0, gmap) if gate is not None else L.NULL_TENSOR
        d.post_act = post_act
        d.out_mode, d.shuffle = out_mode, shuffle
        d.workspace, d.workspace_bytes = None, 0
        d.precise = 1 if precise else 0
        d.max_blocks = (self.early_cap if name in self.early_names and self.max_blocks else self.max_blocks) \
            if self.lane == 0 else 0
        if self.plan_rows is not None:
            slab, full = self.plan_rows
            if oh % slab == 0:
                d.plan_h = full * (oh // slab)
        self.keep.append(d)
        return d

    def finalize_workspace(self, device):
        assert self.lane == 0, 'unjoined side lane'
        self.ws = {}
        for lane in sorted(self.lanes):
            ds = [d for d, ln in self.convs if ln == lane]
            need = max([L.lib().dbsr_conv_workspace_bytes(d) for d in ds] + [0])
            self.ws[lane] = torch.zeros(max(need // 4, 1), dtype=torch.float32, device=device)
            for d in ds:
                d.workspace, d.workspace_bytes = self.ws[lane].data_ptr(), need

    def run(self, stream):
        main = torch.cuda.current_stream()
        if self.streams:
            assert main.cuda_stream == stream, 'Plan.run: lanes fork from the current stream'
        for fn, args, name, lane in self.ops:
            if fn is Plan.FORK:
                args[0].record(main)
                self.streams[lane].wait_event(args[0])
            elif fn is Plan.JOIN:
                args[0].record(self.streams[lane])
                main.wait_event(args[0])
            else:
                rc = fn(*args, stream if lane == 0 else self.streams[lane].cuda_stream)
                if rc != 0:
                    L.check(rc, name)

    def run_list(self, ops, stream):
        for fn, args, name, lane in ops:
            if fn is Plan.FORK or fn is Plan.JOIN:
                continue
            rc = fn(*args, stream)
            if rc != 0:
                L.check(rc, name)

    def time_ops(self, stream, reps=10, full_chip=True):
        capped = [(d, d.max_blocks) for d, _ in self.convs if d.max_blocks] if full_chip else []
        for d, _ in capped:
            d.max_blocks = 0
        try:
            return self._time_ops(stream, reps)
        finally:
            for d, mb in capped:
                d.max_blocks = mb

    def time_ops_in_step(self, stream, reps=3, hold_cycles=40_000_000):
        main = torch.cuda.current_stream()
        assert main.cuda_stream == stream, 'time_ops_in_step: lanes fork from the current stream'
        tot = [0.0] * len(self.ops)
        for _ in range(reps):
            torch.cuda._sleep(hold_cycles)
            evs = []
            for fn, args, name, lane in self.ops:
                if fn is Plan.FORK:
                    args[0].record(main)
                    self.streams[lane].wait_event(args[0])
                    evs.append(None)
                    continue
                if fn is Plan.JOIN:
                    args[0].record(self.streams[lane])
                    main.wait_event(args[0])
                    evs.append(None)
                    continue
                st = main if lane == 0 else self.streams[lane]
                e0, e1 = torch.cuda.Event(enable_timing=True), torch.cuda.Event(enable_timing=True)
                e0.record(st)
                rc = fn(*args, stream if lane == 0 else st.cuda_stream)
                if rc != 0:
                    L.check(rc, name)
                e1.record(st)
                evs.append((e0, e1))
            torch.cuda.synchronize()
            for i, ev in enumerate(evs):
                if ev is not None:
                    tot[i] += ev[0].elapsed_time(ev[1])
        return [(name, t / reps) for (fn, args, name, lane), t in zip(self.ops, tot)]

    def _time_ops(self, stream, reps):
        out = []
        for fn, args, name, lane in self.ops:
            if fn is Plan.FORK or fn is Plan.JOIN:
                out.append((name, 0.0))
                continue
            e0, e1 = torch.cuda.Event(enable_timing=True), torch.cuda.Event(enable_timing=True)
            fn(*args, stream)
            torch.cuda._sleep(2_000_000)
            e0.record()
            for _ in range(reps):
                fn(*args, stream)
            e1.record()
            e1.synchronize()
            out.append((name, e0.elapsed_time(e1) / reps))
        return out


class _Weights:
    def __init__(self, dtype, device, stream, rounding='nearest'):
        self.dtype, self.device, self.stream, self.rounding = dtype, device, stream, rounding

    def conv(self, module, shuffle=1, recipe=None):
        return PackedConv(module, self.dtype, self.device, self.stream, shuffle=shuffle, recipe=recipe,
                          rounding=self.rounding)


def _param_signature(module):
    return tuple((p.data_ptr(), p._version) for p in module.parameters())


class PWCPlanner:
    FUSED_DENSE = True
    FUSED_EXTRACT = True
    FUSED_PREP = True
    FUSED_REFINER = os.environ.get('DBSR_FUSED_REFINER', '1') != '0'
    def __init__(self, pwc_module, W):
        net = pwc_module.net
        ex = net.netExtractor
        self.ext = []
        for lvl in ['netOne', 'netTwo', 'netThr', 'netFou', 'netFiv', 'netSix']:
            seq = getattr(ex, lvl)
            self.ext.append([W.conv(seq[0]), W.conv(seq[2]), W.conv(seq[4])])
        self.dec = {}
        for level, name in zip([2, 3, 4, 5, 6], ['netTwo', 'netThr', 'netFou', 'netFiv', 'netSix']):
            d = getattr(net, name)
            ent = {'dense': [W.conv(getattr(d, n)[0]) for n in ['netOne', 'netTwo', 'netThr', 'netFou', 'netFiv']],
                   'flow': W.conv(d.netSix[0])}
            if level < 6:
                ent['upflow'] = pack_convt(d.netUpflow, W.device)
                ent['upfeat'] = pack_convt(d.netUpfeat, W.device)
                if W.dtype != torch.float32:
                    wt = ent['upfeat'][0]
                    cin = wt.shape[-1]
                    ent['upfeat16'] = torch.nn.functional.pad(wt.reshape(32, cin), (0, (cin + 31) // 32 * 32 - cin)) \
                        .to(W.dtype).contiguous()
            self.dec[level] = ent
        self.ref = [W.conv(net.netRefiner.netMain[i]) for i in range(0, 13, 2)]
        self._W, self._refiner, self._ref_center = W, net.netRefiner, {}

    def ref_center(self, i):
        if i not in self._ref_center:
            m = self._refiner.netMain[2 * i]
            self._ref_center[i] = self._W.conv(types.SimpleNamespace(
                weight=m.weight.detach()[:, :, 1:2, 1:2].contiguous(), bias=m.bias, stride=(1,), padding=(0,),
                dilation=(1,)))
        return self._ref_center[i]

    def build(self, plan, dtype, device, nF, Hp, Wp, P, first_map, second_map, rgb, flow_out, rgb_map=IDENTITY):
        lib = L.lib()
        levels = {}
        if PWCPlanner.FUSED_EXTRACT and dtype != torch.float32 and lib.dbsr_pwc_extract_supported(Hp, Wp):
            convs = (L.PwcExtConv * 18)()
            lv = (L.Tensor * 6)()
            hw, flop = (Hp, Wp), 0.0
            for k in range(6):
                C = PWC_LEVEL_CH[k + 1]
                oh, ow = self.ext[k][0].out_hw(*hw)
                levels[k + 1] = NHWC(nF, oh, ow, cpad(C), dtype, device)
                lv[k] = levels[k + 1].d(0)
                for j in range(3):
                    pc = self.ext[k][j]
                    convs[3 * k + j] = L.PwcExtConv(pc.w.data_ptr(), pc.bias.data_ptr(), pc.cin, pc.cout, pc.stride)
                    flop += 2.0 * nF * oh * ow * pc.cout * pc.cin * 9
                hw = (oh, ow)
            plan.keep.extend([convs, lv])
            plan.add('pwc.extract', lib.dbsr_pwc_extract, nF, Hp, Wp, rgb.d(0, rgb_map), convs, lv, work=('flop', flop))
            plan.kernel[len(plan.ops) - 1] = 'pwc_extract'
        else:
            x, hw = rgb, (Hp, Wp)
            for k in range(6):
                C = PWC_LEVEL_CH[k + 1]
                oh, ow = self.ext[k][0].out_hw(*hw)
                ta = NHWC(nF, oh, ow, cpad(C), dtype, device)
                tb = NHWC(nF, oh, ow, cpad(C), dtype, device)
                lv = NHWC(nF, oh, ow, cpad(C), dtype, device)
                plan.conv(f'pwc.ext{k + 1}.0', self.ext[k][0], nF, x, 0, hw, ta, 0, L.ACT_LRELU,
                          xmap=rgb_map if k == 0 else IDENTITY)
                plan.conv(f'pwc.ext{k + 1}.2', self.ext[k][1], nF, ta, 0, (oh, ow), tb, 0, L.ACT_LRELU)
                plan.conv(f'pwc.ext{k + 1}.4', self.ext[k][2], nF, tb, 0, (oh, ow), lv, 0, L.ACT_LRELU)
                levels[k + 1] = lv
                plan.keep.extend([ta, tb])
                x, hw = lv, (oh, ow)
        plan.keep.append(levels)
        prev = None
        for level in [6, 5, 4, 3, 2]:
            feat = levels[level]
            h, w, C = feat.h, feat.w, PWC_LEVEL_CH[level]
            base_real = 81 if level == 6 else 81 + C + 4
            ld = BASE_OFF + cpad(base_real)
            D = NHWC(P, h, w, ld, dtype, device)
            ent = self.dec[level]
            if PWCPlanner.FUSED_PREP and dtype != torch.float32 and lib.dbsr_pwc_level_prep_supported(h, w, C):
                if prev is None:
                    pargs = (L.NULL_TENSOR, 0, L.NULL_TENSOR, None, None, None, None)
                else:
                    pD, pflow, pbase = prev
                    wf, bf = ent['upflow']
                    bt = ent['upfeat'][1]
                    pargs = (pD.d(0), BASE_OFF + pbase, pflow.d(0), wf.data_ptr(), bf.data_ptr(),
                             ent['upfeat16'].data_ptr(), bt.data_ptr())
                plan.add(f'pwc.dec{level}.prep', lib.dbsr_pwc_level_prep, P, h, w, C, BACKWARP_SCALE.get(level, 1.0),
                         feat.d(0, first_map), feat.d(0, second_map), D.d(BASE_OFF), *pargs)
            else:
                if prev is None:
                    second = feat.d(0, second_map)
                else:
                    pD, pflow, pbase = prev
                    fu = NHWC(P, h, w, 8, torch.float32, device)
                    fe = NHWC(P, h, w, 2, torch.float32, device)
                    wt, bs = ent['upflow']
                    plan.add(f'pwc.dec{level}.upflow', lib.dbsr_conv_transpose_k4s2, P, pD.h, pD.w, 2, 2, pflow.d(0),
                             wt.data_ptr(), bs.data_ptr(), fu.d(0))
                    wt, bs = ent['upfeat']
                    plan.add(f'pwc.dec{level}.upfeat', lib.dbsr_conv_transpose_k4s2, P, pD.h, pD.w, BASE_OFF + pbase,
                             2, pD.d(0), wt.data_ptr(), bs.data_ptr(), fe.d(0))
                    ws = NHWC(P, h, w, cpad(C), dtype, device)
                    plan.add(f'pwc.dec{level}.backwarp', lib.dbsr_backwarp, P, h, w, C, feat.d(0, second_map), fu.d(0),
                             BACKWARP_SCALE[level], ws.d(0))
                    plan.add(f'pwc.dec{level}.assemble', lib.dbsr_pwc_assemble, P, h, w, C, feat.d(0, first_map),
                             fu.d(0), fe.d(0), D.d(BASE_OFF))
                    second = ws.d(0)
                    plan.keep.extend([fu, fe, ws])
                plan.add(f'pwc.dec{level}.corr', lib.dbsr_correlation, P, h, w, C, feat.d(0, first_map), second,
                         D.d(BASE_OFF), 1)
            fl = NHWC(P, h, w, 8, torch.float32, device)
            if PWCPlanner.FUSED_DENSE and dtype != torch.float32 and lib.dbsr_pwc_dense_supported(h, w, ld):
                convs = (L.PwcDenseConv * 6)()
                cin, flop = base_real, 0.0
                for i, pc in enumerate(ent['dense'] + [ent['flow']]):
                    start = 0 if i == 5 else (BASE_OFF if i == 0 else DENSE_OFF[i - 1])
                    cg = cpad(pc.cin) // 8
                    convs[i] = L.PwcDenseConv(pc.w.data_ptr(), pc.bias.data_ptr() if pc.bias is not None else None,
                                              9 * cg * 8, cg, start, pc.cout, DENSE_OFF[i] if i < 5 else 0)
                    flop += 2.0 * P * h * w * pc.cout * pc.cin * 9
                plan.keep.append(convs)
                plan.add(f'pwc.dec{level}.dense', lib.dbsr_pwc_dense, P, h, w, D.d(0), BASE_OFF, convs, fl.d(0),
                         work=('flop', flop))
                plan.kernel[len(plan.ops) - 1] = 'pwc_dense'
                cin = base_real + sum(DENSE_OUT)
            else:
                cin = base_real
                for i, (pc, off) in enumerate(zip(ent['dense'], DENSE_OFF)):
                    start = BASE_OFF if i == 0 else DENSE_OFF[i - 1]
                    plan.conv(f'pwc.dec{level}.dense{i}', pc, P, D, start, (h, w), D, off, L.ACT_LRELU, cin=cin)
                    cin += DENSE_OUT[i]
                plan.conv(f'pwc.dec{level}.flow', ent['flow'], P, D, 0, (h, w), None, 0, L.ACT_NONE, cin=cin,
                          y_desc=fl.d(0))
            plan.keep.extend([D, fl])
            prev = (D, fl, base_real)
        D2, fl2, base2 = prev
        h, w = D2.h, D2.w
        chans = [128, 128, 128, 96, 64, 32]
        bufs = [NHWC(P, h, w, cpad(c), dtype, device) for c in chans]
        x, xc0, cin = D2, 0, BASE_OFF + base2
        fused = PWCPlanner.FUSED_REFINER and dtype != torch.float32 and \
            lib.dbsr_pwc_refine_supported(h, w, L.dtype_code(dtype)) and \
            [(pc.cin, pc.cout, pc.kh, pc.dil) for pc in self.ref[1:]] == REFINER_TAIL
        for i in range(1 if fused else 6):
            pc = self.ref[i]
            if pc.dil >= h and pc.dil >= w and pc.kh == 3:
                pc = self.ref_center(i)
            plan.conv(f'pwc.refiner{i}', pc, P, x, xc0, (h, w), bufs[i], 0, L.ACT_LRELU, cin=cin)
            x, xc0, cin = bufs[i], 0, chans[i]
        if fused:
            pcs = [self.ref_center(i) if i == 4 else self.ref[i] for i in range(1, 7)]
            convs = (L.PwcRefineConv * 6)(*[
                L.PwcRefineConv(pc.w.data_ptr(), pc.bias.data_ptr() if pc.bias is not None else None, pc.cin, pc.cout,
                                pc.kh, pc.dil) for pc in pcs])
            flop = sum(2.0 * P * h * w * pc.cout * pc.cin * pc.kh * pc.kw for pc in pcs)
            plan.keep.append(convs)
            plan.add('pwc.refiner1-6', lib.dbsr_pwc_refine, P, h, w, x.d(0), convs, fl2.d(0), flow_out.d(0),
                     work=('flop', flop))
            plan.kernel[len(plan.ops) - 1] = 'pwc_dense'
        else:
            plan.conv('pwc.refiner6', self.ref[6], P, x, 0, (h, w), None, 0, L.ACT_NONE, y_desc=flow_out.d(0),
                      res=fl2)
        plan.keep.extend(bufs)


class DBSREngine:
    LANE0_CU_SHARE = 0.5625
    LANE0_EARLY_CONVS = 0
    LANE0_EARLY_SHARE = 0.5
    FUSED_HEAD = True
    FUSED_UPSAMPLE_BLUR = True
    FUSED_RESBLOCK = True
    FUSED_RESBLOCK64 = True
    FUSED_WARP_PROJ = False
    LINEAR_SPLIT = True
    FUSED_WP_OUT = True
    WEIGHT_ROUNDING = 'diffuse'

    def __init__(self, net):
        self.net = net
        self.dtype = net.compute_dtype
        self.zero_flow = bool(getattr(net, 'zero_flow', False))
        self.device = None
        self.sig = None
        self.plans = {}
        self.slots = {}
        self.graphs = {}
        self.weights_stale = False

    def matches(self, net):
        return (net is self.net and self.dtype == net.compute_dtype and self.sig == _param_signature(net)
                and self.zero_flow == bool(getattr(net, 'zero_flow', False)))

    def _pack(self, device):
        net = self.net
        stream = L.stream_ptr(device)
        W = _Weights(self.dtype, device, stream, rounding=DBSREngine.WEIGHT_ROUNDING)
        enc, mer, dec = net.encoder, net.merging, net.decoder
        self.pwc = PWCPlanner(enc.alignment_net, _Weights(self.dtype, device, stream))
        self.enc_init = W.conv(enc.init_layer[0])
        self.enc_res = [(W.conv(b.conv1[0]), W.conv(b.conv2[0])) for b in enc.res_layers]
        self.enc_out = W.conv(enc.out_layer[0])
        self.proj = W.conv(mer.feat_project_layer[0])
        ofe = list(mer.offset_feat_extractor)
        self.ofe_init = W.conv(ofe[0][0])
        self.ofe_res = [(W.conv(b.conv1[0]), W.conv(b.conv2[0])) for b in ofe[1:]]
        wp = list(mer.weight_predictor)
        self.wp_init = W.conv(wp[0][0])
        self.softmax, self.ref_base, self.offset_modulo = merging_variant(mer)
        pd = mer.feat_project_layer[0].out_channels
        self.wp_split = None
        if DBSREngine.LINEAR_SPLIT and pd % 32 == 0:
            c0 = wp[0][0]
            geo = types.SimpleNamespace(stride=(1,), padding=c0.padding, dilation=c0.dilation)
            rest = lambda: (c0.weight.detach().float()[:, pd:], c0.bias)
            base = lambda: (c0.weight.detach().float()[:, :pd] - c0.weight.detach().float()[:, pd:2 * pd], None)
            self.wp_split = (W.conv(geo, recipe=rest), W.conv(geo, recipe=base))
        elif not self.ref_base:
            raise NotImplementedError('use_base_frame=False runs on the linearity split: needs project_dim % 32 == 0 '
                                      '(and DBSREngine.LINEAR_SPLIT)')
        self.wp_res = [(W.conv(b.conv1[0]), W.conv(b.conv2[0])) for b in wp[1:-1]]
        self.wp_out = W.conv(wp[-1][0])
        self.dec_init = W.conv(dec.init_layer[0])
        self.dec_pre = [(W.conv(b.conv1[0]), W.conv(b.conv2[0])) for b in dec.pre_res_layers]
        up = dec.upsample_layer
        self.s = up.upsample_factor
        self.dec_up = W.conv(up.conv_layer[0], shuffle=self.s)
        self.blur = gauss_kernel3(up.gauss_blur_sd, up.gauss_ksz) if up.gauss_blur_sd is not None else None
        if self.blur is not None and up.gauss_ksz != 3:
            raise NotImplementedError('gauss_ksz != 3')
        self.dec_post = [(W.conv(b.conv1[0]), W.conv(b.conv2[0])) for b in dec.post_res_layers]
        self.pred = PackedConv(dec.predictor[0], torch.float32, device, stream)
        pm = dec.predictor[0]
        self.head_w = pm.weight.detach().to(device=device, dtype=torch.float32).reshape(pm.out_channels, -1).contiguous()
        self.head_b = (pm.bias.detach().to(device=device, dtype=torch.float32).contiguous()
                       if pm.bias is not None else None)
        self.device = device
        self.sig = _param_signature(net)
        self.plans, self.slots, self.graphs = {}, {}, {}
        self.weights_stale = False

    def refresh_weights(self):
        stream = L.stream_ptr(self.device)
        convs = [self.enc_init, self.enc_out, self.proj, self.ofe_init, self.wp_init, self.wp_out, self.dec_init,
                 self.dec_up, self.pred]
        for lst in (self.enc_res, self.ofe_res, self.wp_res, self.dec_pre, self.dec_post):
            for c1, c2 in lst:
                convs += [c1, c2]
        if self.wp_split is not None:
            convs += list(self.wp_split)
        for pc in convs:
            pc.repack(stream)
        pm = self.net.decoder.predictor[0]
        self.head_w.copy_(pm.weight.detach().reshape(pm.out_channels, -1))
        if self.head_b is not None:
            self.head_b.copy_(pm.bias.detach())
        self.weights_stale = False

    def _resblocks(self, plan, name, blocks, n, hw, bufs, x_idx, dtype, head=None):
        a = x_idx
        fused = False
        for i, (c1, c2) in enumerate(blocks):
            b, c = [j for j in range(3) if j != a]
            hd = head if head is not None and i == len(blocks) - 1 else None
            if DBSREngine.FUSED_RESBLOCK and \
                    plan.resblock(f'{name}{i}', c1, c2, n, bufs[a], bufs[b], bufs[c], hw, head=hd):
                fused = hd is not None
                a = c
                continue
            plan.conv(f'{name}{i}.conv1', c1, n, bufs[a], 0, hw, bufs[b], 0, L.ACT_RELU)
            d = plan.conv(f'{name}{i}.conv2', c2, n, bufs[b], 0, hw, bufs[c], 0, L.ACT_NONE, res=bufs[a],
                          post_act=L.ACT_RELU, head=head if i == len(blocks) - 1 else None)
            fused = d.fused_head
            a = c
        return (a, fused) if head is not None else a

    def _emit_flow(self, plan, grp, N, H, W, sh):
        dt, dev = self.dtype, self.device
        lib = L.lib()
        g0, g1 = grp
        Bg, Fg, Pg = g1 - g0, (g1 - g0) * N, (g1 - g0) * (N - 1)
        off_f, off_p = g0 * N, g0 * (N - 1)
        Hp, Wp = sh['Hp'], sh['Wp']
        hw = (H, W)
        fmap = (1, 1, off_f, 0)
        if not self.zero_flow:
            flow_out = NHWC(Pg, Hp // 4, Wp // 4, 2, torch.float32, dev)
            self.pwc.build(plan, dt, dev, Fg, Hp, Wp, Pg, first_map=(N - 1, N, 0, 0), second_map=(N - 1, N, 1, 1),
                           rgb=sh['rgb'], flow_out=flow_out, rgb_map=fmap)
            plan.add('flow_finalize', lib.dbsr_flow_finalize, Bg, N, Hp // 4, Wp // 4, flow_out.d(0), H, W, Hp, Wp,
                     sh['offsets'][off_p:].data_ptr(), self.offset_modulo, sh['om'].d(0, fmap))
            plan.keep.append(flow_out)
        pd, od = self.proj.cout, self.ofe_init.cout
        oc = pd if self.wp_split is not None else 2 * pd
        WP = NHWC(Fg, H, W, oc + od, dt, dev)
        plan.keep.append(WP)
        return WP

    def _emit_ofe(self, plan, grp, N, H, W, sh, WP):
        dt, dev = self.dtype, self.device
        g0, g1 = grp
        Fg = (g1 - g0) * N
        fmap = (1, 1, g0 * N, 0)
        hw = (H, W)
        pd, od = self.proj.cout, self.ofe_init.cout
        oc = pd if self.wp_split is not None else 2 * pd
        o = [NHWC(Fg, H, W, od, dt, dev) for _ in range(3)]
        plan.conv('merge.ofe.init', self.ofe_init, Fg, sh['om'], 0, hw, o[0], 0, L.ACT_RELU, xmap=fmap)
        a = 0
        if not self.ofe_res:
            raise NotImplementedError('num_offset_feat_extractor_res must be >= 1')
        for k, (c1, c2) in enumerate(self.ofe_res):
            b, c = [j for j in range(3) if j != a]
            last = k == len(self.ofe_res) - 1
            if DBSREngine.FUSED_RESBLOCK and plan.resblock(f'merge.ofe.res{k}', c1, c2, Fg, o[a], o[b],
                                                           WP if last else o[c], hw, yc0=oc if last else 0):
                a = c
                continue
            plan.conv(f'merge.ofe.res{k}.conv1', c1, Fg, o[a], 0, hw, o[b], 0, L.ACT_RELU)
            if last:
                plan.conv(f'merge.ofe.res{k}.conv2', c2, Fg, o[b], 0, hw, WP, oc, L.ACT_NONE, res=o[a],
                          post_act=L.ACT_RELU)
            else:
                plan.conv(f'merge.ofe.res{k}.conv2', c2, Fg, o[b], 0, hw, o[c], 0, L.ACT_NONE, res=o[a],
                          post_act=L.ACT_RELU)
                a = c
        plan.keep.append(o)

    def _emit_base(self, plan, grp, N, H, W, sh, WP):
        g0, g1 = grp
        Bg = g1 - g0
        rest, basec = self.wp_split
        plan.conv('merge.proj_ref', self.proj, Bg, sh['E'], 0, (H, W), WP, 0, L.ACT_RELU, xmap=(1, N, g0 * N, 1),
                  ymap=(1, N, 0, 1))
        if not self.ref_base:
            return None
        BS = NHWC(Bg, H, W, r8(basec.cout), self.dtype, self.device)
        plan.conv('merge.wp.base', basec, Bg, WP, 0, (H, W), BS, 0, L.ACT_NONE, xmap=(1, N, 0, 1))
        plan.keep.append(BS)
        return BS

    def _emit_mean_base(self, plan, grp, N, H, W, WP):
        g0, g1 = grp
        Bg = g1 - g0
        basec = self.wp_split[1]
        pd = self.proj.cout
        MB = NHWC(Bg, H, W, cpad(pd), self.dtype, self.device)
        plan.add('merge.base_mean', L.lib().dbsr_burst_mean, Bg, N, H * W, pd, WP.d(0), MB.d(0),
                 work=('byte', (N + 1.0) * Bg * H * W * pd * (4 if self.dtype == torch.float32 else 2)))
        BS = NHWC(Bg, H, W, r8(basec.cout), self.dtype, self.device)
        plan.conv('merge.wp.base', basec, Bg, MB, 0, (H, W), BS, 0, L.ACT_NONE)
        plan.keep.extend([MB, BS])
        return BS

    def _emit_warp(self, plan, grp, N, H, W, sh, WP):
        dt, dev = self.dtype, self.device
        g0, g1 = grp
        Pg = (g1 - g0) * (N - 1)
        off_f, off_p = g0 * N, g0 * (N - 1)
        C, E = self.enc_out.cout, sh['E']
        Wf = NHWC(max(Pg, 1), H, W, C, dt, dev)
        es = 4 if dt == torch.float32 else 2
        if Pg > 0:
            pd = self.proj.cout
            fused = (self.wp_split is not None and DBSREngine.FUSED_WARP_PROJ and dt != torch.float32 and C == 512
                     and pd % 16 == 0 and pd <= 64 and self.proj.kh == 1 and self.proj.cin == C)
            if fused:
                plan.add('warp+proj', L.lib().dbsr_warp_project, Pg, H, W, C, E.d(0, (N - 1, N, 1 + off_f, 1)),
                         sh['offsets'][off_p:].data_ptr(), 2 * H * W, Wf.d(0), self.proj.w.data_ptr(),
                         self.proj.bias.data_ptr() if self.proj.bias is not None else None, pd,
                         WP.d(0, (N - 1, N, 1, 1)),
                         work=('byte', 2.0 * Pg * C * H * W * es + 8.0 * Pg * H * W + 1.0 * Pg * pd * H * W * es))
                plan.kernel[len(plan.ops) - 1] = 'warp'
            else:
                plan.add('warp', L.lib().dbsr_warp_bilinear, Pg, H, W, C, E.d(0, (N - 1, N, 1 + off_f, 1)),
                         sh['offsets'][off_p:].data_ptr(), 2 * H * W, Wf.d(0),
                         work=('byte', 2.0 * Pg * C * H * W * es + 8.0 * Pg * H * W))
                if self.wp_split is not None:
                    plan.conv('merge.proj_oth', self.proj, Pg, Wf, 0, (H, W), WP, 0, L.ACT_RELU,
                              ymap=(N - 1, N, 1, 1))
        plan.keep.append(Wf)
        return Wf

    def _emit_merge(self, plan, grp, N, H, W, sh, WP, BS=None, Wf=None):
        dt, dev = self.dtype, self.device
        lib = L.lib()
        g0, g1 = grp
        Bg, Fg, Pg = g1 - g0, (g1 - g0) * N, (g1 - g0) * (N - 1)
        off_f = g0 * N
        PJ = sh['PJ']
        hw = (H, W)
        pd = self.proj.cout
        if Wf is None:
            Wf = self._emit_warp(plan, grp, N, H, W, sh, WP)
        q = [NHWC(Fg, H, W, self.wp_init.cout, dt, dev) for _ in range(3)]
        if self.wp_split is not None:
            rest = self.wp_split[0]
            if BS is None:
                BS = self._emit_mean_base(plan, grp, N, H, W, WP)
            plan.conv('merge.wp.init', rest, Fg, WP, 0, hw, q[0], 0, L.ACT_NONE, res=BS, rmap=(N, 1, 0, 0),
                      post_act=L.ACT_RELU)
        else:
            if Pg > 0:
                plan.conv('merge.proj_oth', self.proj, Pg, Wf, 0, hw, PJ, 0, L.ACT_RELU,
                          ymap=(N - 1, N, 1 + off_f, 1))
            plan.add('merge.prep', lib.dbsr_merge_prep, Bg, N, H * W, pd, PJ.d(0, (1, 1, off_f, 0)), WP.d(0))
            plan.conv('merge.wp.init', self.wp_init, Fg, WP, 0, hw, q[0], 0, L.ACT_RELU)
        i = self._resblocks(plan, 'merge.wp.res', self.wp_res, Fg, hw, q, 0, dt)
        plan.keep.append(q)
        return q[i], Wf

    def _emit_logits(self, plan, Fg, H, W, h):
        LG = NHWC(Fg, H, W, self.enc_out.cout, self.dtype, self.device)
        plan.conv('merge.wp.out', self.wp_out, Fg, h, 0, (H, W), LG, 0, L.ACT_NONE)
        plan.keep.append(LG)
        return LG

    def _build(self, B, N, H, W, mode='full', first_frame=0):
        dt, dev = self.dtype, self.device
        lib = L.lib()
        plan = Plan()
        F, P = B * N, B * (N - 1)
        C = self.enc_out.cout
        hw = (H, W)
        bufs = {}
        bufs['burst'] = torch.zeros(B, N, 4, H, W, dtype=torch.float32, device=dev)
        raw = NHWC(F, H, W, 8, dt, dev)
        Hp, Wp = int(math.ceil(H / 64.0) * 64), int(math.ceil(W / 64.0) * 64)
        rgb = NHWC(F, Hp, Wp, 8, dt, dev)
        bufs['offsets'] = torch.zeros(P, 2, H, W, dtype=torch.float32, device=dev)
        om = NHWC(F, H, W, 8, dt, dev)
        E = NHWC(F, H, W, C, dt, dev)
        PJ = NHWC(F, H, W, r8(self.proj.cout), dt, dev) if self.wp_split is None else None
        sh = {'rgb': rgb, 'offsets': bufs['offsets'], 'om': om, 'E': E, 'PJ': PJ, 'Hp': Hp, 'Wp': Wp}
        grp = (0, B)
        plan.add('pack_burst', lib.dbsr_pack_burst, B, N, H, W, bufs['burst'].data_ptr(), raw.d(0), Hp, Wp,
                 rgb.d(0) if not self.zero_flow else L.NULL_TENSOR)
        plan_cap = int(torch.cuda.get_device_properties(dev).multi_processor_count * DBSREngine.LANE0_CU_SHARE) \
            if Plan.MULTI_STREAM else 0
        plan.fork(1, dev, priority=0)
        WP = self._emit_flow(plan, grp, N, H, W, sh)
        plan.switch(0)
        plan.max_blocks = plan.max_blocks_cap = plan_cap
        if plan_cap and DBSREngine.LANE0_EARLY_CONVS:
            names = ['enc.init'] + [f'enc.res{i}.conv{j}' for i in range(len(self.enc_res)) for j in (1, 2)]
            plan.early_names = set(names[:DBSREngine.LANE0_EARLY_CONVS])
            plan.early_cap = int(torch.cuda.get_device_properties(dev).multi_processor_count *
                                 DBSREngine.LANE0_EARLY_SHARE)
        e = [NHWC(F, H, W, r8(self.enc_init.cout), dt, dev) for _ in range(3)]
        plan.conv('enc.init', self.enc_init, F, raw, 0, hw, e[0], 0, L.ACT_RELU)
        i = self._resblocks(plan, 'enc.res', self.enc_res, F, hw, e, 0, dt)
        plan.conv('enc.out', self.enc_out, F, e[i], 0, hw, E, 0, L.ACT_RELU)
        if self.wp_split is None:
            plan.conv('merge.proj_ref', self.proj, B, E, 0, hw, PJ, 0, L.ACT_RELU, xmap=(1, N, 0, 1),
                      ymap=(1, N, 0, 1))
        plan.keep.extend([raw, rgb, om, e, E, PJ])
        FW = NHWC(F, H, W, C, dt, dev) if mode == 'full' else None
        if mode == 'full':
            bufs['pred'] = torch.zeros(B, 3, H * self.s, W * self.s, dtype=torch.float32, device=dev)
        plan.fuse_ops = []
        es = 4 if dt == torch.float32 else 2
        BS = self._emit_base(plan, grp, N, H, W, sh, WP) if self.wp_split is not None else None
        plan.join(1)
        plan.max_blocks = 0
        plan.switch(1)
        self._emit_ofe(plan, grp, N, H, W, sh, WP)
        plan.switch(0)
        Wf = self._emit_warp(plan, grp, N, H, W, sh, WP)
        plan.join(1)
        h, Wf = self._emit_merge(plan, grp, N, H, W, sh, WP, BS=BS, Wf=Wf)
        if mode == 'partial':
            LG = self._emit_logits(plan, B * N, H, W, h)
            ST = torch.zeros(B, H, W, 3 * C, dtype=torch.float32, device=dev)
            plan.add('merge.fuse_partial', lib.dbsr_fuse_partial, B, N, H * W, C, first_frame, LG.d(0),
                     E.d(0, (1, N, 0, 1)), Wf.d(0), ST.data_ptr())
            bufs['stats'] = ST
        else:
            FUS = NHWC(B, H, W, C, dt, dev)
            feats = [E.d(0, (1, N, 0, 1)), Wf.d(0), FUS.d(0), FW.d(0)]
            idx = plan.conv_fuse('merge.wp.out+fuse', self.wp_out, B, N, h, hw, *feats, softmax=self.softmax) \
                if DBSREngine.FUSED_WP_OUT else None
            if idx is not None:
                plan.fuse_ops.append((idx, plan.ops[idx][1], FW.d(0), None))
            else:
                LG = self._emit_logits(plan, B * N, H, W, h)
                args = [B, N, H * W, C, LG.d(0)] + feats
                if self.softmax:
                    plan.add('merge.fuse', lib.dbsr_fuse_softmax, *args)
                else:
                    plan.add('merge.fuse_relu_norm', lib.dbsr_fuse_relu_norm, *args)
                plan.fuse_ops.append((len(plan.ops) - 1, args, FW.d(0),
                                      ((2.0 * N + 1) * B * C * H * W * es, 1.0 * N * B * C * H * W * es)))
            self._decoder(plan, B, H, W, FUS, bufs, pred_out=bufs['pred'])
            plan.keep.append(FUS)
        plan.max_blocks = 0
        plan.keep.append(FW)
        plan.finalize_workspace(dev)
        plan.bufs = bufs
        plan.FW = FW
        plan.shape = (B, N, H, W)
        return plan

    def _decoder(self, plan, B, H, W, FUS, bufs, pred_out=None):
        dt, dev = self.dtype, self.device
        lib = L.lib()
        hw = (H, W)
        S = self.s
        gd = self.dec_init.cout
        g = [NHWC(B, H, W, gd, dt, dev) for _ in range(3)]
        plan.conv('dec.init', self.dec_init, B, FUS, 0, hw, g[0], 0, L.ACT_RELU)
        i = self._resblocks(plan, 'dec.pre', self.dec_pre, B, hw, g, 0, dt)
        pc = self.dec_up.cout // (S * S)
        sh = [NHWC(B, H * S, W * S, pc, dt, dev) for _ in range(3)]
        a = 0
        if self.blur is not None and DBSREngine.FUSED_UPSAMPLE_BLUR and \
                plan.conv_shuffle_blur('dec.upsample+blur', self.dec_up, B, g[i], hw, sh[1], L.ACT_RELU,
                                       self.blur) is not None:
            a = 1
        else:
            plan.conv('dec.upsample', self.dec_up, B, g[i], 0, hw, sh[0], 0, L.ACT_RELU, out_mode=L.OUT_SHUFFLE,
                      shuffle=S)
            if self.blur is not None:
                kbuf = (ctypes.c_float * 9)(*self.blur)
                plan.keep.append(kbuf)
                plan.add('dec.blur', lib.dbsr_gauss_blur3, B, H * S, W * S, pc, sh[0].d(0), kbuf, sh[1].d(0))
                a = 1
        if pred_out is None:
            pred_out = bufs['pred'] = torch.zeros(B, 3, H * S, W * S, dtype=torch.float32, device=dev)
        pdesc = L.tensor_desc(pred_out, 1, 0, img_stride=3 * H * S * W * S, dtype=torch.float32)
        head = None
        if dt != torch.float32 and self.dec_post and DBSREngine.FUSED_HEAD:
            head = ('predictor', self.head_w, self.head_b, pdesc)
        if head is not None:
            i, fused = self._resblocks(plan, 'dec.post', self.dec_post, B, (H * S, W * S), sh, a, dt, head=head)
        else:
            i, fused = self._resblocks(plan, 'dec.post', self.dec_post, B, (H * S, W * S), sh, a, dt), False
        if not fused:
            plan.conv('dec.predictor', self.pred, B, sh[i], 0, (H * S, W * S), None, 0, L.ACT_RELU,
                      out_mode=L.OUT_NCHW_F32, y_desc=pdesc, precise=(dt != torch.float32))
        plan.keep.extend([g, sh])

    @staticmethod
    def _capture(plan, dev):
        g = torch.cuda.CUDAGraph()
        with torch.cuda.graph(g):
            plan.run(L.stream_ptr(dev))
        return g

    def _set_fw(self, plan, want):
        for idx, args, fw_desc, nbytes in plan.fuse_ops:
            fn, _, name, lane = plan.ops[idx]
            a = list(args)
            a[-1] = fw_desc if want else L.NULL_TENSOR
            plan.ops[idx] = (fn, tuple(a), name, lane)
            if nbytes is not None:
                plan.work[idx] = ('byte', nbytes[0] + (nbytes[1] if want else 0.0))

    OUTPUT_SLOTS = 3

    @staticmethod
    def _uses(t):
        return torch._C._storage_Use_Count(t.untyped_storage()._cdata)

    def _outputs(self, plan):
        return [plan.bufs['pred'], plan.bufs['offsets']] + ([plan.FW.t] if plan.FW is not None else [])

    def _slot_free(self, plan):
        return all(self._uses(t) <= b for t, b in zip(self._outputs(plan), plan.out_base))

    def _new_slot(self, key):
        plan = self._build(*key)
        plan.out_base = [self._uses(t) for t in self._outputs(plan)]
        self.slots.setdefault(key, []).append(plan)
        if len(self.slots[key]) == 1:
            self.plans[key] = plan
        return plan

    def forward(self, burst):
        if not burst.is_cuda:
            raise RuntimeError('DBSRNet (MI355X engine) needs the burst on a HIP device; got %s' % burst.device)
        if burst.dim() != 5 or burst.shape[2] != 4:
            raise ValueError('burst must be [B,N,4,H,W]')
        B, N, _, H, W = burst.shape
        if N < 2:
            raise ValueError('burst needs at least 2 frames')
        dev = burst.device
        if self.device != dev or self.sig != _param_signature(self.net):
            self._pack(dev)
        elif self.weights_stale:
            self.refresh_weights()
        key = (B, N, H, W)
        if key not in self.slots:
            self._new_slot(key)
        slots = self.slots[key]
        nzc = DBSREngine.OUTPUT_SLOTS - 1
        if getattr(self.net, 'graph_zero_copy', False):
            si = 0
        else:
            si = next((i for i, p in enumerate(slots[:nzc]) if self._slot_free(p)), None)
            if si is None and len(slots) < nzc:
                self._new_slot(key)
                si = len(slots) - 1
        copy = si is None
        if copy:
            while len(slots) < DBSREngine.OUTPUT_SLOTS:
                self._new_slot(key)
            si = DBSREngine.OUTPUT_SLOTS - 1
        plan = self.slots[key][si]
        want_fw = bool(getattr(self.net, 'return_fusion_weights', True))
        self._set_fw(plan, want_fw)
        stream = L.stream_ptr(dev)
        plan.bufs['burst'].copy_(burst.to(torch.float32), non_blocking=True)
        if getattr(self.net, 'use_graph', False):
            g = self.graphs.get((key, si, want_fw))
            if g is None:
                plan.run(stream)
                g = self._capture(plan, dev)
                self.graphs[(key, si, want_fw)] = g
            g.replay()
        else:
            plan.run(stream)
        pred, offs = plan.bufs['pred'], plan.bufs['offsets']
        fw_t = plan.FW.t if want_fw else None
        if copy:
            pred, offs = pred.clone(), offs.clone()
            fw_t = fw_t.clone() if want_fw else None
        native = fw_t.view(B, N, H, W, -1).permute(0, 1, 4, 2, 3) if want_fw else None
        return pred.view(pred.shape), DBSRAux(offs.view(B, N - 1, 2, H, W), native)

    def decoder_halo(self):
        from .parallel import decoder_halo_rows
        return decoder_halo_rows(len(self.dec_pre), len(self.dec_post), self.s, self.blur is not None)

    def _build_combine(self, R, B, H, W, rows=None):
        dt, dev = self.dtype, self.device
        C = self.enc_out.cout
        plan = Plan()
        bufs = {'gathered': torch.zeros(R, B, H, W, 3 * C, dtype=torch.float32, device=dev)}
        FUS = NHWC(B, H, W, C, dt, dev)
        plan.add('merge.fuse_combine', L.lib().dbsr_fuse_combine, R, B, H * W, C, bufs['gathered'].data_ptr(),
                 FUS.d(0))
        if rows is None:
            self._decoder(plan, B, H, W, FUS, bufs)
            plan.valid = (0, H * self.s)
        else:
            lo, hi = rows
            from .parallel import decoder_slab
            y0, y1 = decoder_slab(lo, hi, H, self.decoder_halo())
            plan.plan_rows = (y1 - y0, H)
            self._decoder(plan, B, y1 - y0, W, FUS.rows(y0, y1), bufs)
            plan.plan_rows = None
            plan.valid = ((lo - y0) * self.s, (hi - y0) * self.s)
        plan.keep.append(FUS)
        plan.finalize_workspace(dev)
        plan.bufs = bufs
        return plan

    def _ready(self, burst):
        if not burst.is_cuda:
            raise RuntimeError('DBSRNet (MI355X engine) needs the burst on a HIP device; got %s' % burst.device)
        if self.device != burst.device or self.sig != _param_signature(self.net):
            self._pack(burst.device)
        elif self.weights_stale:
# ... 93 lines not shown
```

include/dbsr_hip.h:

```cpp
#ifndef DBSR_HIP_H
#define DBSR_HIP_H

#include <stddef.h>
#include <stdint.h>

#ifdef __cplusplus
extern "C" {
#endif

#define DBSR_ABI_VERSION 23

enum { DBSR_F32 = 0, DBSR_BF16 = 1, DBSR_F16 = 2 };
enum { DBSR_ACT_NONE = 0, DBSR_ACT_RELU = 1, DBSR_ACT_LRELU = 2 };
enum { DBSR_OUT_NHWC = 0, DBSR_OUT_SHUFFLE = 1, DBSR_OUT_NCHW_F32 = 2 };
enum { DBSR_E_ARG = -1, DBSR_E_UNSUPPORTED = -2 };

typedef struct dbsr_frame_map {
    int fpg;
    int group_stride;
    int group_offset;
    int inner_stride;
} dbsr_frame_map;

typedef struct dbsr_tensor {
    void* ptr;
    int dtype;
    long long img_stride;
    int ld;
    int c0;
    dbsr_frame_map map;
} dbsr_tensor;

typedef struct dbsr_conv_desc {
    int n_frames;
    dbsr_tensor x;  int in_h, in_w, cin;
    const void* w;  const float* bias;  int cout, kh, kw, stride, pad, dil;
    dbsr_tensor y;  int out_h, out_w;
    int act;
    dbsr_tensor res;
    int post_act;
    int out_mode, shuffle;
    void* workspace;
    size_t workspace_bytes;
    int precise;
    int max_blocks;
    dbsr_tensor gate;
    int plan_h;
} dbsr_conv_desc;

size_t dbsr_conv_packed_elems(int cout, int cin, int kh, int kw);
int dbsr_conv_pack_weights(const float* w_f32, const float* bias_f32, int cout, int cin, int kh, int kw,
                           int dtype, int shuffle, void* w_packed, float* bias_out, void* stream);
typedef struct dbsr_pack_job {
    const float* w;
    const float* bias;
    void* w_packed;
    float* bias_out;
    int cout, cin, kh, kw;
    int dtype, shuffle;
    int transposed, lo, src_cin;
    int pad_;
    long long blk0;
} dbsr_pack_job;
long long dbsr_pack_batch_prepare(dbsr_pack_job* jobs, int n);
int dbsr_conv_pack_weights_batch(const dbsr_pack_job* jobs_dev, int n, long long n_blocks, void* stream);
int dbsr_conv2d(const dbsr_conv_desc* d, void* stream);
int dbsr_weights_round_diffuse(const float* w, int cout, int cin, int kh, int kw, int dtype, float* w_out,
                               void* stream);
int dbsr_set_conv_algo(int algo);
int dbsr_conv_kernel_for(const dbsr_conv_desc* d);
int dbsr_conv_dispatch_variant(const dbsr_conv_desc* d);
int dbsr_conv_lane_reach(const dbsr_conv_desc* d, int which);
int dbsr_conv2d_head(const dbsr_conv_desc* d, const float* head_w, const float* head_b, int head_cout,
                     dbsr_tensor head_out, void* stream);
int dbsr_conv_shuffle_blur(const dbsr_conv_desc* d, const float* k9, void* stream);
int dbsr_conv_shuffle_blur_ok(const dbsr_conv_desc* d);
int dbsr_resblock(const dbsr_conv_desc* c1, const dbsr_conv_desc* c2, void* stream);
int dbsr_resblock_ok(const dbsr_conv_desc* c1, const dbsr_conv_desc* c2);
int dbsr_resblock_head(const dbsr_conv_desc* c1, const dbsr_conv_desc* c2, const float* head_w, const float* head_b,
                       int head_cout, dbsr_tensor head_out, void* stream);
int dbsr_conv_head_ok(const dbsr_conv_desc* d);
size_t dbsr_conv_workspace_bytes(const dbsr_conv_desc* d);

int dbsr_correlation(int n_pairs, int h, int w, int c, dbsr_tensor first, dbsr_tensor second,
                     dbsr_tensor out, int leaky, void* stream);

int dbsr_correlation_backward(int n_pairs, int h, int w, int c, dbsr_tensor first, dbsr_tensor second,
                              dbsr_tensor out, dbsr_tensor gout, int leaky, dbsr_tensor dfirst, dbsr_tensor dsecond,
                              void* stream);

int dbsr_backwarp(int n, int h, int w, int c, dbsr_tensor in, dbsr_tensor flow, float scale,
                  dbsr_tensor out, void* stream);

int dbsr_warp_bilinear(int n, int h, int w, int c, dbsr_tensor feat, const float* flow,
                       long long flow_img_stride, dbsr_tensor out, void* stream);
int dbsr_warp_project(int n, int h, int w, int c, dbsr_tensor feat, const float* flow, long long flow_img_stride,
                      dbsr_tensor out, const void* proj_w, const float* proj_b, int proj_cout, dbsr_tensor proj_out,
                      void* stream);

int dbsr_fuse_softmax(int B, int N, int hw, int c, dbsr_tensor logits, dbsr_tensor ref, dbsr_tensor oth,
                      dbsr_tensor fused, dbsr_tensor weights, void* stream);

int dbsr_fuse_relu_norm(int B, int N, int hw, int c, dbsr_tensor logits, dbsr_tensor ref, dbsr_tensor oth,
                        dbsr_tensor fused, dbsr_tensor weights, void* stream);
int dbsr_burst_mean(int B, int N, int hw, int c, dbsr_tensor in, dbsr_tensor out, void* stream);

int dbsr_conv_fuse_softmax(const dbsr_conv_desc* d, int B, int N, dbsr_tensor ref, dbsr_tensor oth,
                           dbsr_tensor fused, dbsr_tensor weights, void* stream);
int dbsr_conv_fuse_relu_norm(const dbsr_conv_desc* d, int B, int N, dbsr_tensor ref, dbsr_tensor oth,
                             dbsr_tensor fused, dbsr_tensor weights, void* stream);
int dbsr_conv_fuse_ok(const dbsr_conv_desc* d, int B, int N);

int dbsr_fuse_partial(int B, int N, int hw, int c, int first_frame, dbsr_tensor logits, dbsr_tensor ref,
                      dbsr_tensor oth, float* stats, void* stream);
int dbsr_fuse_combine(int R, int B, int hw, int c, const float* stats, dbsr_tensor fused, void* stream);

int dbsr_conv_transpose_k4s2(int n, int h, int w, int cin, int cout, dbsr_tensor in, const float* wgt,
                             const float* bias, dbsr_tensor out, void* stream);

int dbsr_pack_burst(int B, int N, int H, int W, const float* burst, dbsr_tensor raw, int Hp, int Wp,
                    dbsr_tensor rgb, void* stream);

int dbsr_flow_finalize(int B, int N, int hf, int wf, dbsr_tensor flow, int H, int W, int Hp, int Wp,
                       float* offsets, float modulo, dbsr_tensor offs_mod, void* stream);

int dbsr_gauss_blur3(int n, int h, int w, int c, dbsr_tensor in, const float* k_host, dbsr_tensor out,
                     void* stream);

int dbsr_merge_prep(int B, int N, int hw, int c, dbsr_tensor proj, dbsr_tensor out, void* stream);

int dbsr_pwc_assemble(int n_pairs, int h, int w, int c, dbsr_tensor first, dbsr_tensor flow,
                      dbsr_tensor feat, dbsr_tensor out, void* stream);

typedef struct {
    const void* w;
    const float* bias;
    int kp, cg;
    int start;
    int cout, out_off;
} dbsr_pwc_dense_conv;
int dbsr_pwc_dense(int P, int h, int w, dbsr_tensor D, int dense_ch, const dbsr_pwc_dense_conv* convs,
                   dbsr_tensor flow, void* stream);
int dbsr_pwc_dense_supported(int h, int w, int ld);

typedef struct {
    const void* w;
    const float* bias;
    int cin, cout, ksize, dil;
} dbsr_pwc_refine_conv;
int dbsr_pwc_refine(int P, int h, int w, dbsr_tensor x, const dbsr_pwc_refine_conv* convs, dbsr_tensor res_flow,
                    dbsr_tensor flow_out, void* stream);
int dbsr_pwc_refine_supported(int h, int w, int dtype);

typedef struct {
    const void* w;
    const float* bias;
    int cin, cout, stride;
} dbsr_pwc_ext_conv;
int dbsr_pwc_extract(int F, int Hp, int Wp, dbsr_tensor rgb, const dbsr_pwc_ext_conv* convs,
                     const dbsr_tensor* levels, void* stream);
int dbsr_pwc_extract_supported(int Hp, int Wp);
int dbsr_pwc_level_prep(int P, int h, int w, int c, float scale, dbsr_tensor first, dbsr_tensor second, dbsr_tensor D,
                        dbsr_tensor prev_D, int prev_cin, dbsr_tensor prev_flow, const float* w_upflow,
                        const float* b_upflow, const void* w_upfeat, const float* b_upfeat, void* stream);
int dbsr_pwc_level_prep_supported(int h, int w, int c);

int dbsr_resize_bilinear(int planes, int ih, int iw, const float* in, int oh, int ow, float rh, float rw, float mul,
                         float* out, void* stream);
int dbsr_gauss_reflect(int planes, int h, int w, int ksz, const float* k_host, const float* in, float* out,
                       void* stream);
int dbsr_color_fit(int n, int h, int w, int bi, const float* ref, const float* q, float* c_mat, void* stream);
int dbsr_color_apply(int n, int h, int w, int bi, const float* ref, const float* q, const float* c_mat, float thresh,
                     const float* test, int oh, int ow, float rh, float rw, float* out, unsigned char* valid,
                     void* stream);

size_t dbsr_aligned_l1_workspace_bytes(int B, int H, int W);
int dbsr_aligned_l1_forward(int B, int H, int W, int boundary_ignore, const float* pred, const float* flow,
                            const float* c_mat, const unsigned char* valid, const float* gt, float weight,
                            float* g_pw, float* loss, float* stats, void* workspace, size_t workspace_bytes,
                            void* stream);
int dbsr_aligned_l1_backward(int B, int H, int W, const float* pred, const float* flow, const float* g_pw,
                             const float* c_mat, const float* scale, float* gpred, dbsr_tensor dpre, void* workspace,
                             size_t workspace_bytes, void* stream);

size_t dbsr_ssim_workspace_bytes(int B, int C, int H, int W, int boundary_ignore);
int dbsr_ssim_forward(int B, int C, int H, int W, int boundary_ignore, const float* pred, const float* gt,
                      const unsigned char* valid, float val_range, float* map, float* sums, float* result,
                      void* workspace, size_t workspace_bytes, void* stream);
int dbsr_ssim_backward(int B, int C, int H, int W, int boundary_ignore, const float* pred, const float* gt,
                       const unsigned char* valid, float val_range, const float* scale, float* gpred, void* workspace,
                       size_t workspace_bytes, void* stream);

enum { DBSR_SRC_F32_NCHW = 0, DBSR_SRC_U8_NHWC = 1 };
enum { DBSR_POST_GAINS = 1, DBSR_POST_CCM = 2, DBSR_POST_GAMMA = 4, DBSR_POST_SMOOTHSTEP = 8 };
int dbsr_unprocess_rgb(int B, int Hc, int Wc, const void* src, int src_format, const float* params, float* lin,
                       void* stream);
int dbsr_burst_synth(int B, int N, int Hc, int Wc, int bc, int f, const float* lin, const float* ainv,
                     const float* noise_levels, const float* z, float* burst, float* burst_rgb, float* flow,
                     void* stream);
int dbsr_postprocess_rgb(int B, int H, int W, const float* img, const float* params, int flags, float* out_f32,
                         unsigned char* out_u8, void* stream);


size_t dbsr_conv_wgrad_workspace_bytes(int n_frames, int h, int w, int cin, int cout, int k);
int dbsr_conv_wgrad(int n_frames, int h, int w, dbsr_tensor x, int cin, dbsr_tensor dy, int cout, int k,
                    float* dw, int accumulate, void* workspace, size_t workspace_bytes, void* stream);
int dbsr_set_wgrad_algo(int algo);
int dbsr_conv_wgrad_bias(int n_frames, int h, int w, dbsr_tensor x, int cin, dbsr_tensor dy, int cout, int k,
                         float* dw, float* db, int accumulate, void* workspace, size_t workspace_bytes, void* stream);
int dbsr_head_forward(int n, int hw, dbsr_tensor h, int cin, const float* w, const float* b, int hc, float* out,
                      void* stream);
size_t dbsr_head_backward_workspace_bytes(int n, int hw, int cin, int hc);
int dbsr_head_backward(int n, int hw, dbsr_tensor h, int cin, dbsr_tensor dp, const float* w, int hc, dbsr_tensor dh,
                       float* dw, float* db, int accumulate, void* workspace, size_t workspace_bytes, void* stream);
size_t dbsr_chan_sum_workspace_bytes(int n, int hw, int c);
int dbsr_chan_sum(int n, int hw, int c, dbsr_tensor t, float* out, int accumulate, void* workspace,
                  size_t workspace_bytes, void* stream);
int dbsr_l1_loss_backward(int B, int C, int H, int W, int boundary_ignore, const float* pred, const float* gt,
                          dbsr_tensor dpre, float* loss, void* workspace, size_t workspace_bytes, void* stream);
int dbsr_relu_grad(int B, int C, int H, int W, const float* pred, const float* gout, dbsr_tensor dpre, void* stream);
int dbsr_unshuffle_gate(int B, int H, int W, int s, int c, dbsr_tensor ds, dbsr_tensor gate, dbsr_tensor du,
                        void* stream);
int dbsr_fuse_backward(int B, int N, int hw, int c, dbsr_tensor weights, dbsr_tensor ref, dbsr_tensor oth,
                       dbsr_tensor fused, dbsr_tensor dfused, dbsr_tensor dlogits, dbsr_tensor dref,
                       dbsr_tensor doth, void* stream);
int dbsr_merge_prep_backward(int B, int N, int hw, int c, dbsr_tensor dwp, dbsr_tensor proj, dbsr_tensor dproj,
                             void* stream);
int dbsr_warp_backward(int n, int h, int w, int c, dbsr_tensor dout, const float* flow, long long flow_img_stride,
                       float* dfeat32, dbsr_frame_map fmap, long long dfeat_img_stride, void* stream);
int dbsr_enc_grad_gate(int B, int N, int hw, int c, dbsr_tensor dref, const float* dsrc32, dbsr_tensor e,
                       dbsr_tensor de, void* stream);
size_t dbsr_warp_backward_gather_workspace_bytes(int n, int h, int w);
int dbsr_warp_backward_gather(int n, int h, int w, int c, dbsr_tensor dout, const float* flow,
                              long long flow_img_stride, dbsr_tensor gate, dbsr_tensor dfeat, void* workspace,
                              size_t workspace_bytes, void* stream);
// ... 45 lines not shown
```

Measured before the change: 3409 bursts/s.

## Read planar fp32 burst directly in first conv; K-slice split dec.init conv

Two independent changes. First, the encoder's first 3x3 conv (4 input channels) now reads the planar fp32 burst directly and rounds it to 16-bit on load, so the NHWC raw repack buffer is no longer built and pack_burst only writes the rgb pyramid input, moved to the flow lane. Second, the decoder init conv (cin 128-512, cout 64) gains a K-slice variant of the work-stealing 3x3 kernel: each block handles a 64-channel input slice and writes fp32 partials to a workspace, and a split-K finalize kernel reduces them. This targets poor CU utilisation at small batch, at the cost of extra workspace traffic and an additional launch.

```diff
diff --git a/deep-rawburst-sr_amd/_lib.py b/deep-rawburst-sr_amd/_lib.py
--- a/deep-rawburst-sr_amd/_lib.py
+++ b/deep-rawburst-sr_amd/_lib.py
@@ -94,6 +94,11 @@
             'dbsr_conv_dispatch_variant': ([ctypes.POINTER(ConvDesc)], c_int),
             'dbsr_conv_lane_reach': ([ctypes.POINTER(ConvDesc), c_int], c_int),
             'dbsr_conv_workspace_bytes': ([ctypes.POINTER(ConvDesc)], c_size_t),
+            'dbsr_conv3x3_planar4': ([ctypes.POINTER(ConvDesc), c_void_p, c_void_p], c_int),
+            'dbsr_conv3x3_planar4_ok': ([ctypes.POINTER(ConvDesc)], c_int),
+            'dbsr_conv3x3_kslice': ([ctypes.POINTER(ConvDesc), c_void_p], c_int),
+            'dbsr_conv3x3_kslice_ok': ([ctypes.POINTER(ConvDesc)], c_int),
+            'dbsr_conv3x3_kslice_workspace_bytes': ([ctypes.POINTER(ConvDesc)], c_size_t),
             'dbsr_conv2d_head': ([ctypes.POINTER(ConvDesc), c_void_p, c_void_p, c_int, Tensor, c_void_p], c_int),
             'dbsr_conv_head_ok': ([ctypes.POINTER(ConvDesc)], c_int),
             'dbsr_conv_shuffle_blur': ([ctypes.POINTER(ConvDesc), c_void_p, c_void_p], c_int),
@@ -239,7 +244,8 @@
             'dbsr_conv_wgrad_sd_workspace_bytes', 'dbsr_conv_wgrad_sd', 'dbsr_dgrad_sd_packed_elems',
             'dbsr_dgrad_sd_pack', 'dbsr_conv_dgrad_sd', 'dbsr_act_backward', 'dbsr_flow_finalize_backward',
             'dbsr_l1_loss_backward_scaled', 'dbsr_grad_unscale_check', 'dbsr_adam_step_guarded',
-            'dbsr_loss_scale_update',
+            'dbsr_loss_scale_update', 'dbsr_conv3x3_planar4', 'dbsr_conv3x3_planar4_ok',
+            'dbsr_conv3x3_kslice', 'dbsr_conv3x3_kslice_ok', 'dbsr_conv3x3_kslice_workspace_bytes',
             'dbsr_resize_bilinear', 'dbsr_gauss_reflect', 'dbsr_color_fit', 'dbsr_color_apply', 'dbsr_pwc_dense',
             'dbsr_pwc_dense_supported', 'dbsr_pwc_refine', 'dbsr_pwc_refine_supported', 'dbsr_pwc_extract',
             'dbsr_pwc_extract_supported', 'dbsr_pwc_level_prep', 'dbsr_pwc_level_prep_supported',
diff --git a/deep-rawburst-sr_amd/csrc/conv2d.hip b/deep-rawburst-sr_amd/csrc/conv2d.hip
--- a/deep-rawburst-sr_amd/csrc/conv2d.hip
+++ b/deep-rawburst-sr_amd/csrc/conv2d.hip
@@ -1162,8 +1162,9 @@
 __global__ __launch_bounds__(512, 1) void conv3x3_ws_kernel(ConvK k, int tiles_x, int tiles_y, int nct, int nsp,
                                                             int px) {
     using C = WsCfg<WM, TW, TH, NCH>;
-    static_assert(EPI >= 0 && EPI <= 5 && EPI != 4, "epilogues 0-3, 5");
+    static_assert(EPI >= 0 && EPI <= 6 && EPI != 4, "epilogues 0-3, 5, 6");
     DBSR_OWN_SIMDS();
+    constexpr bool KSL = EPI == 6;
     constexpr int RES_BUFS = (EPI == 0 || EPI == 2 || EPI == 5) ? 2 : 0;
     constexpr int DMA_STEPS = RES_BUFS > 0 ? C::DMA_STEPS : (2 * C::STEPS) / 3;
     constexpr int BUF_U4 = 2 * C::STAGE_U4 + RES_BUFS * C::RES_U4;
@@ -1194,21 +1195,26 @@
     if (my_tiles == 0) return;
     PIPE_STAMP(0);
 
-    const int cb = ct * WM + wc * 32;
+    const int cb = (KSL ? 0 : ct * WM) + wc * 32;
     {
         const __amdgpu_buffer_rsrc_t w_rsrc = buf_rsrc(k.w_pipe, 0xffffffffu);
         const int p0 = (ct * WM >> 4) * NCH * 9;
 #pragma unroll
         for (int it = 0; it < C::W_PER; ++it) {
             const int piece = min(wave + C::NWAVES * it, C::W_PIECES - 1);
-            blds16(w_rsrc, lane * 16, (p0 + piece) * 1024, lds + C::STAGE_U4 + piece * 64);
+            int src = p0 + piece;
+            if constexpr (KSL) {
+                const int blk = piece / (NCH * 9);
+                src = (blk * nct + ct) * (NCH * 9) + (piece - blk * (NCH * 9));
+            }
+            blds16(w_rsrc, lane * 16, src * 1024, lds + C::STAGE_U4 + piece * 64);
         }
     }
     if (threadIdx.x < WM) {
         const int co = ct * WM + threadIdx.x;
-        lbias[threadIdx.x] = (k.bias && co < k.cout) ? k.bias[co] : 0.f;
-    }
-    const bool cout_ok = cb + 8 * g < k.cout;
+        lbias[threadIdx.x] = (!KSL && k.bias && co < k.cout) ? k.bias[co] : 0.f;
+    }
+    const bool cout_ok = KSL || cb + 8 * g < k.cout;
 
     struct Tile { const T* xf; long long y_off, r_off, g_off; int y0, x0; };
     auto decode = [&](int i) {
@@ -1220,7 +1226,8 @@
         t.y0 = ty * TH; t.x0 = tx * TW;
         t.xf = (const T*)k.x + map_frame(k.xm, f) * k.x_is;
         const long long pix = (long long)t.y0 * k.out_w + t.x0;
-        t.y_off = map_frame(k.ym, f) * k.y_is + k.y_c0 + cb + pix * k.y_ld;
+        if constexpr (KSL) t.y_off = (((long long)ct * k.npix + (long long)f * k.out_h * k.out_w + pix) * WM) + cb;
+        else t.y_off = map_frame(k.ym, f) * k.y_is + k.y_c0 + cb + pix * k.y_ld;
         t.r_off = has_res ? map_frame(k.rm, f) * k.r_is : 0;
         t.g_off = has_gate ? map_frame(k.gm, f) * k.g_is + k.g_c0 + cb + pix * k.g_ld : 0;
         return t;
@@ -1240,7 +1247,7 @@
         const int gg = 2 * ((ph & 1) ^ ((p >> 2) & 1)) + (ph >> 1);
         const int r = p / C::HWD, cc = p - r * C::HWD;
         h_rc[it] = p < C::NQ ? (r << 16) | cc : 0x7fff7fff;
-        h_off[it] = (r * k.in_w + cc) * pix_b + cch * 64 + gg * 16;
+        h_off[it] = (r * k.in_w + cc) * pix_b + ((KSL ? ct * NCH : 0) + cch) * 64 + gg * 16;
     }
     auto dma = [&](int it, const Tile& t, int buf) {
         const int item = min(wave + C::NWAVES * it, C::ITEMS - 1);
@@ -1272,7 +1279,16 @@
         blds16(buf_rsrc((const T*)k.r + t.r_off, rframe_bytes), off, 0, lres + buf * C::RES_U4 + q * 64);
     };
     u32x4_t packed[C::GW];
+    f32x4_t part[KSL ? 2 : 1][KSL ? C::GW : 1];
     auto epilogue = [&](const Tile& t, int rbuf) {
+        if constexpr (KSL) {
+#pragma unroll
+            for (int j = 0; j < C::GW; ++j) {
+                part[0][j] = acc[0][j];
+                part[1][j] = acc[1][j];
+            }
+            return;
+        }
         u32x4_t gatev[EPI == 5 ? C::GW : 1];
         if constexpr (EPI == 5) {
 #pragma unroll
@@ -1312,6 +1328,15 @@
         }
     };
     auto store = [&](const Tile& t) {
+        if constexpr (KSL) {
+#pragma unroll
+            for (int j = 0; j < C::GW; ++j) {
+                float* wp = k.ws + t.y_off + px_off(j) * WM + 8 * g;
+                *(f32x4_t*)wp = part[0][j];
+                *(f32x4_t*)(wp + 4) = part[1][j];
+            }
+            return;
+        }
 #pragma unroll
         for (int j = 0; j < C::GW; ++j)
             if (cout_ok) *(u32x4_t*)((T*)k.y + t.y_off + px_off(j) * k.y_ld + 8 * g) = packed[j];
@@ -1391,6 +1416,7 @@
         prev = cur;
         cur = nxt;
     }
+    if constexpr (KSL) vm_drain();
     store(prev);
     PIPE_STAMP(1);
 }
@@ -1454,6 +1480,42 @@
     return 0;
 }
 
+int kslice_px(const dbsr_conv_desc* d) {
+    if (!d || !is16(d->x.dtype) || d->precise || d->kh != 3 || d->kw != 3 || d->stride != 1 || d->pad != 1 ||
+        d->dil != 1 || d->cin % 64 || d->cin < 128 || d->cin > 512 || d->cout != 64 ||
+        d->out_mode != DBSR_OUT_NHWC || d->y.dtype != d->x.dtype || d->gate.ptr)
+        return 0;
+    if (d->n_frames <= 0 || d->in_h != d->out_h || d->in_w != d->out_w || d->out_w <= 0 || d->out_w % 16 ||
+        d->out_h <= 0 || d->out_h % 8)
+        return 0;
+    if (d->x.ld % 8 || d->x.c0 % 8 || d->x.c0 + d->cin > d->x.ld) return 0;
+    if ((long long)d->in_h * d->in_w * d->x.ld * 2 >= (1LL << 31)) return 0;
+    if ((long long)d->n_frames * d->out_h * d->out_w >= (1LL << 31) / 64) return 0;
+    const int nct = d->cin / 64;
+    const long long nsp = (long long)d->n_frames * (d->out_w / 16) * (d->out_h / 8);
+    const int cus = d->max_blocks > 0 ? std::min(d->max_blocks, num_cus()) : num_cus();
+    if (cus / 8 / nct < 1) return 0;
+    const long long spx = std::max<long long>(1, std::min<long long>(cus / 8 / nct, (nsp + 7) / 8));
+    return (int)(spx * nct);
+}
+size_t kslice_bytes(const dbsr_conv_desc* d) {
+    return (size_t)(d->cin / 64) * d->n_frames * d->out_h * d->out_w * 64 * sizeof(float);
+}
+template <typename T>
+int launch_kslice(const ConvK& k0, const dbsr_conv_desc* d, int px, hipStream_t s) {
+    ConvK k = k0;
+    const int nct = d->cin / 64, tiles_x = k.out_w / 16, tiles_y = k.out_h / 8;
+    const int nsp = d->n_frames * tiles_x * tiles_y;
+    k.ksplit = nct;
+    hipLaunchKernelGGL((conv3x3_ws_kernel<T, 64, 16, 8, 2, 6>), dim3(8 * px), dim3(512), 0, s, k, tiles_x, tiles_y, nct,
+                       nsp, px);
+    DBSR_LAUNCH_CHECK();
+    const long long n = (long long)k.npix * (k.cw / 4);
+    hipLaunchKernelGGL((conv_splitk_finalize<T>), dim3((unsigned)((n + 255) / 256)), dim3(256), 0, s, k);
+    DBSR_LAUNCH_CHECK();
+    return 0;
+}
+
 int g_ks128_enabled = 1;
 bool use_ks128(const dbsr_conv_desc* d) {
     if (!g_ks128_enabled || !is16(d->x.dtype) || d->precise || d->kh != 3 || d->kw != 3 || d->stride != 1 ||
@@ -1836,7 +1898,15 @@
 }
 
 template <typename T>
-__global__ __launch_bounds__(256) void conv3x3_small_kernel(ConvK k, int groups_x, long long ngroups) {
+__device__ __forceinline__ short round16_bits(float v) {
+    T t;
+    elem<T>::st(&t, v);
+    return __builtin_bit_cast(short, t);
+}
+
+template <typename T, bool PLANAR>
+__global__ __launch_bounds__(256) void conv3x3_small_kernel(ConvK k, int groups_x, long long ngroups,
+                                                            const float* __restrict__ src) {
     const int lane = threadIdx.x & 63, g = lane >> 4, col = lane & 15;
     const int nco = k.cout / 16;
     Frag<T> a[4][3];
@@ -1855,16 +1925,25 @@
         const long long r = gi / groups_x;
         const int y = (int)(r % k.out_h), f = (int)(r / k.out_h);
         const int x = gx * 16 + col;
-        const T* xf = (const T*)k.x + map_frame(k.xm, f) * k.x_is;
+        const long long plane = (long long)k.in_h * k.in_w;
+        const T* xf = PLANAR ? nullptr : (const T*)k.x + map_frame(k.xm, f) * k.x_is;
+        const float* sf = PLANAR ? src + map_frame(k.xm, f) * 4 * plane : nullptr;
         Frag<T> bq[3];
 #pragma unroll
         for (int st = 0; st < 3; ++st) {
             const int tap = 4 * st + g, ky = tap / 3, kx = tap - 3 * (tap / 3);
             const int iy = y + ky - 1, ix = x + kx - 1;
-            if (tap < 9 && (unsigned)iy < (unsigned)k.in_h && (unsigned)ix < (unsigned)k.in_w)
-                bq[st].load(xf + ((long long)iy * k.in_w + ix) * k.x_ld);
-            else
+            if (tap < 9 && (unsigned)iy < (unsigned)k.in_h && (unsigned)ix < (unsigned)k.in_w) {
+                if constexpr (PLANAR) {
+                    const float* p = sf + (long long)iy * k.in_w + ix;
+                    bq[st].v = bf16x8_t{round16_bits<T>(p[0]), round16_bits<T>(p[plane]),
+                                        round16_bits<T>(p[2 * plane]), round16_bits<T>(p[3 * plane]), 0, 0, 0, 0};
+                } else {
+                    bq[st].load(xf + ((long long)iy * k.in_w + ix) * k.x_ld);
+                }
+            } else {
                 bq[st].zero();
+            }
         }
         f32x4_t acc[4];
 #pragma unroll
@@ -1895,12 +1974,13 @@
            !d->res.ptr && !d->gate.ptr;
 }
 template <typename T>
-int launch_small(const ConvK& k, const dbsr_conv_desc* d, hipStream_t s) {
+int launch_small(const ConvK& k, const dbsr_conv_desc* d, hipStream_t s, const float* src = nullptr) {
     const int gx = (d->out_w + 15) / 16;
     const long long ng = (long long)d->n_frames * d->out_h * gx;
     const long long want = (ng + 15) / 16;
     const unsigned grid = (unsigned)std::max<long long>(1, std::min<long long>(want, 4096));
-    hipLaunchKernelGGL((conv3x3_small_kernel<T>), dim3(grid), dim3(256), 0, s, k, gx, ng);
+    if (src) hipLaunchKernelGGL((conv3x3_small_kernel<T, true>), dim3(grid), dim3(256), 0, s, k, gx, ng, src);
+    else hipLaunchKernelGGL((conv3x3_small_kernel<T, false>), dim3(grid), dim3(256), 0, s, k, gx, ng, src);
     DBSR_LAUNCH_CHECK();
     return 0;
 }
@@ -2766,6 +2846,54 @@
     return d->x.dtype == DBSR_BF16 ? dispatch_conv<bf16_t>(k, d, sel, s) : dispatch_conv<float>(k, d, sel, s);
 }
 
+bool planar4_ok(const dbsr_conv_desc* d) {
+    return d && is16(d->x.dtype) && !d->precise && d->kh == 3 && d->kw == 3 && d->stride == 1 && d->pad == 1 &&
+           d->dil == 1 && d->cin == 4 && d->cout > 0 && d->cout % 16 == 0 && d->cout <= 64 &&
+           d->out_mode == DBSR_OUT_NHWC && d->y.dtype == d->x.dtype && d->y.ld % 4 == 0 && d->y.c0 % 4 == 0 &&
+           !d->res.ptr && !d->gate.ptr;
+}
+
+extern "C" int dbsr_conv3x3_planar4_ok(const dbsr_conv_desc* d) { return g_small_enabled && planar4_ok(d) ? 1 : 0; }
+
+extern "C" int dbsr_conv3x3_planar4(const dbsr_conv_desc* d, const float* src, void* stream) {
+    DBSR_CHECK_ARG(d && src && d->w && d->y.ptr, "conv3x3_planar4: null pointer");
+    DBSR_CHECK_ARG(planar4_ok(d), "conv3x3_planar4: needs a 16-bit 3x3/s1/p1/d1 conv 4 -> 16 | 32 | 48 | 64 with an "
+                   "NHWC output of x.dtype (y.ld, y.c0 multiples of 4), no residual or gate");
+    DBSR_CHECK_ARG(d->n_frames > 0 && d->in_h > 0 && d->in_w > 0 && d->out_h == d->in_h && d->out_w == d->in_w,
+                   "conv3x3_planar4: bad sizes");
+    DBSR_CHECK_ARG(d->x.map.fpg > 0 && d->y.map.fpg > 0, "conv3x3_planar4: frame map fpg must be > 0");
+    DBSR_CHECK_ARG(d->y.c0 + d->cout <= d->y.ld, "conv3x3_planar4: output slice exceeds ld");
+    DBSR_CHECK_ARG((long long)d->n_frames * d->out_h * d->out_w < (1LL << 31), "conv3x3_planar4: too many pixels");
+    const ConvK k = make_convk(d);
+    if (d->x.dtype == DBSR_F16) return launch_small<f16_t>(k, d, (hipStream_t)stream, src);
+    return launch_small<bf16_t>(k, d, (hipStream_t)stream, src);
+}
+
+extern "C" int dbsr_conv3x3_kslice_ok(const dbsr_conv_desc* d) { return g_ws_enabled && kslice_px(d) > 0 ? 1 : 0; }
+
+extern "C" size_t dbsr_conv3x3_kslice_workspace_bytes(const dbsr_conv_desc* d) {
+    return kslice_px(d) > 0 ? kslice_bytes(d) : 0;
+}
+
+extern "C" int dbsr_conv3x3_kslice(const dbsr_conv_desc* d, void* stream) {
+    DBSR_CHECK_ARG(d && d->x.ptr && d->w && d->y.ptr, "conv3x3_kslice: null pointer");
+    const int px = kslice_px(d);
+    DBSR_CHECK_ARG(px > 0, "conv3x3_kslice: needs a 16-bit 3x3/s1/p1/d1 conv, cin a multiple of 64 in [128, 512], "
+                   "cout 64, frames a multiple of 16 x 8, NHWC output of x.dtype, no gate, and at least 8 * cin / 64 "
+                   "CUs (max_blocks)");
+    DBSR_CHECK_ARG(d->x.map.fpg > 0 && d->y.map.fpg > 0, "conv3x3_kslice: frame map fpg must be > 0");
+    DBSR_CHECK_ARG(d->y.c0 + d->cout <= d->y.ld, "conv3x3_kslice: output slice exceeds ld");
+    if (d->res.ptr)
+        DBSR_CHECK_ARG(d->res.dtype == d->y.dtype && d->res.map.fpg > 0 && d->res.c0 + d->cout <= d->res.ld,
+                       "conv3x3_kslice: residual must be an NHWC tensor of the output dtype holding cout channels");
+    DBSR_CHECK_ARG(d->workspace && d->workspace_bytes >= kslice_bytes(d) && (uintptr_t)d->workspace % 16 == 0,
+                   "conv3x3_kslice: needs a 16-B aligned workspace of dbsr_conv3x3_kslice_workspace_bytes (%zu) bytes",
+                   kslice_bytes(d));
+    const ConvK k = make_convk(d);
+    if (d->x.dtype == DBSR_F16) return launch_kslice<f16_t>(k, d, px, (hipStream_t)stream);
+    return launch_kslice<bf16_t>(k, d, px, (hipStream_t)stream);
+}
+
 extern "C" int dbsr_resblock_ok(const dbsr_conv_desc* c1, const dbsr_conv_desc* c2) {
     return resblock_channels(c1, c2) && c2->y.ptr && resblock_out_disjoint(c1, c2, nullptr, 0) ? 1 : 0;
 }
diff --git a/deep-rawburst-sr_amd/engine.py b/deep-rawburst-sr_amd/engine.py
--- a/deep-rawburst-sr_amd/engine.py
+++ b/deep-rawburst-sr_amd/engine.py
@@ -207,7 +207,7 @@
 
     def conv(self, name, pc, n_frames, x, xc0, in_hw, y, yc0, act, xmap=IDENTITY, ymap=IDENTITY, res=None,
              rc0=0, rmap=IDENTITY, post_act=L.ACT_NONE, out_mode=L.OUT_NHWC, shuffle=0, y_desc=None, cin=None,
-             precise=False, head=None, gate=None, gc0=0, gmap=IDENTITY):
+             precise=False, head=None, gate=None, gc0=0, gmap=IDENTITY, kslice=False):
         d = self._desc(name, pc, n_frames, x, xc0, in_hw, y, yc0, act, xmap, ymap, res, rc0, rmap, post_act,
                        out_mode, shuffle, y_desc, cin, precise, gate, gc0, gmap)
         self.convs.append((d, self.lane))
@@ -222,9 +222,28 @@
                      hb.data_ptr() if hb is not None else None, hw.shape[0], hdesc, work=('flop', flop))
             self.kernel[len(self.ops) - 1] = 'conv3x3_pipe'
             return d
+        d.kslice = bool(kslice and L.lib().dbsr_conv3x3_kslice_ok(ctypes.byref(d)))
+        if d.kslice:
+            self.add(name, L.lib().dbsr_conv3x3_kslice, ctypes.byref(d), work=('flop', flop))
+            self.kernel[len(self.ops) - 1] = 'conv3x3_ws'
+            return d
         self.add(name, L.lib().dbsr_conv2d, ctypes.byref(d), work=('flop', flop))
         self.kernel[len(self.ops) - 1] = {4: 'conv3x3_ws', 7: 'conv3x3_ks128', 2: 'conv3x3_pipe', 1: 'conv3x3_tiled', 3: 'conv1x1_shuffle', 5: 'conv1x1', 6: 'conv3x3_narrow', 8: 'conv3x3_small'}.get(L.lib().dbsr_conv_kernel_for(d),
                                                                                       'conv2d_generic')
+        return d
+
+    def conv_planar4(self, name, pc, n_frames, src, in_hw, y, act, dry=False):
+        d = self._desc(name, pc, n_frames, y, 0, in_hw, y, 0, act, IDENTITY, IDENTITY, None, 0, IDENTITY,
+                       L.ACT_NONE, L.OUT_NHWC, 0, None, None, False, None, 0, IDENTITY)
+        d.x = L.Tensor(None, L.dtype_code(y.dtype), 0, 0, 0, L.FrameMap(*IDENTITY))
+        if not L.lib().dbsr_conv3x3_planar4_ok(ctypes.byref(d)):
+            return None
+        if dry:
+            return d
+        self.keep.append(src)
+        flop = 2.0 * n_frames * d.out_h * d.out_w * pc.cout * d.cin * pc.kh * pc.kw
+        self.add(name, L.lib().dbsr_conv3x3_planar4, ctypes.byref(d), src.data_ptr(), work=('flop', flop))
+        self.kernel[len(self.ops) - 1] = 'conv3x3_small'
         return d
 
     def conv_fuse(self, name, pc, B, N, x, in_hw, ref, oth, fused, weights, xmap=IDENTITY, softmax=True):
@@ -317,7 +336,8 @@
         self.ws = {}
         for lane in sorted(self.lanes):
             ds = [d for d, ln in self.convs if ln == lane]
-            need = max([L.lib().dbsr_conv_workspace_bytes(d) for d in ds] + [0])
+            need = max([L.lib().dbsr_conv3x3_kslice_workspace_bytes(d) if getattr(d, 'kslice', False)
+                        else L.lib().dbsr_conv_workspace_bytes(d) for d in ds] + [0])
             self.ws[lane] = torch.zeros(max(need // 4, 1), dtype=torch.float32, device=device)
             for d in ds:
                 d.workspace, d.workspace_bytes = self.ws[lane].data_ptr(), need
@@ -599,6 +619,8 @@
     FUSED_WARP_PROJ = False
     LINEAR_SPLIT = True
     FUSED_WP_OUT = True
+    PLANAR_FIRST_CONV = os.environ.get('DBSR_PLANAR_FIRST_CONV', '1') != '0'
+    KSLICE_DEC_INIT = os.environ.get('DBSR_KSLICE_DEC_INIT', '1') != '0'
     WEIGHT_ROUNDING = 'diffuse'
 
     def __init__(self, net):
@@ -849,7 +871,6 @@
         hw = (H, W)
         bufs = {}
         bufs['burst'] = torch.zeros(B, N, 4, H, W, dtype=torch.float32, device=dev)
-        raw = NHWC(F, H, W, 8, dt, dev)
         Hp, Wp = int(math.ceil(H / 64.0) * 64), int(math.ceil(W / 64.0) * 64)
         rgb = NHWC(F, Hp, Wp, 8, dt, dev)
         bufs['offsets'] = torch.zeros(P, 2, H, W, dtype=torch.float32, device=dev)
@@ -858,11 +879,19 @@
         PJ = NHWC(F, H, W, r8(self.proj.cout), dt, dev) if self.wp_split is None else None
         sh = {'rgb': rgb, 'offsets': bufs['offsets'], 'om': om, 'E': E, 'PJ': PJ, 'Hp': Hp, 'Wp': Wp}
         grp = (0, B)
-        plan.add('pack_burst', lib.dbsr_pack_burst, B, N, H, W, bufs['burst'].data_ptr(), raw.d(0), Hp, Wp,
-                 rgb.d(0) if not self.zero_flow else L.NULL_TENSOR)
+        e = [NHWC(F, H, W, r8(self.enc_init.cout), dt, dev) for _ in range(3)]
+        planar = DBSREngine.PLANAR_FIRST_CONV and dt != torch.float32 and plan.conv_planar4(
+            'enc.init', self.enc_init, F, bufs['burst'], hw, e[0], L.ACT_RELU, dry=True) is not None
+        raw = None if planar else NHWC(F, H, W, 8, dt, dev)
+        rgb_d = rgb.d(0) if not self.zero_flow else L.NULL_TENSOR
+        if not planar:
+            plan.add('pack_burst', lib.dbsr_pack_burst, B, N, H, W, bufs['burst'].data_ptr(), raw.d(0), Hp, Wp, rgb_d)
         plan_cap = int(torch.cuda.get_device_properties(dev).multi_processor_count * DBSREngine.LANE0_CU_SHARE) \
             if Plan.MULTI_STREAM else 0
         plan.fork(1, dev, priority=0)
+        if planar and not self.zero_flow:
+            plan.add('pack_burst', lib.dbsr_pack_burst, B, N, H, W, bufs['burst'].data_ptr(), L.NULL_TENSOR, Hp, Wp,
+                     rgb_d)
         WP = self._emit_flow(plan, grp, N, H, W, sh)
         plan.switch(0)
         plan.max_blocks = plan.max_blocks_cap = plan_cap
@@ -871,8 +900,10 @@
             plan.early_names = set(names[:DBSREngine.LANE0_EARLY_CONVS])
             plan.early_cap = int(torch.cuda.get_device_properties(dev).multi_processor_count *
                                  DBSREngine.LANE0_EARLY_SHARE)
-        e = [NHWC(F, H, W, r8(self.enc_init.cout), dt, dev) for _ in range(3)]
-        plan.conv('enc.init', self.enc_init, F, raw, 0, hw, e[0], 0, L.ACT_RELU)
+        if planar:
+            plan.conv_planar4('enc.init', self.enc_init, F, bufs['burst'], hw, e[0], L.ACT_RELU)
+        else:
+            plan.conv('enc.init', self.enc_init, F, raw, 0, hw, e[0], 0, L.ACT_RELU)
         i = self._resblocks(plan, 'enc.res', self.enc_res, F, hw, e, 0, dt)
         plan.conv('enc.out', self.enc_out, F, e[i], 0, hw, E, 0, L.ACT_RELU)
         if self.wp_split is None:
@@ -932,7 +963,7 @@
         S = self.s
         gd = self.dec_init.cout
         g = [NHWC(B, H, W, gd, dt, dev) for _ in range(3)]
-        plan.conv('dec.init', self.dec_init, B, FUS, 0, hw, g[0], 0, L.ACT_RELU)
+        plan.conv('dec.init', self.dec_init, B, FUS, 0, hw, g[0], 0, L.ACT_RELU, kslice=DBSREngine.KSLICE_DEC_INIT)
         i = self._resblocks(plan, 'dec.pre', self.dec_pre, B, hw, g, 0, dt)
         pc = self.dec_up.cout // (S * S)
         sh = [NHWC(B, H * S, W * S, pc, dt, dev) for _ in range(3)]
diff --git a/include/dbsr_hip.h b/include/dbsr_hip.h
--- a/include/dbsr_hip.h
+++ b/include/dbsr_hip.h
@@ -81,6 +81,11 @@
                        int head_cout, dbsr_tensor head_out, void* stream);
 int dbsr_conv_head_ok(const dbsr_conv_desc* d);
 size_t dbsr_conv_workspace_bytes(const dbsr_conv_desc* d);
+int dbsr_conv3x3_planar4(const dbsr_conv_desc* d, const float* src, void* stream);
+int dbsr_conv3x3_planar4_ok(const dbsr_conv_desc* d);
+int dbsr_conv3x3_kslice(const dbsr_conv_desc* d, void* stream);
+int dbsr_conv3x3_kslice_ok(const dbsr_conv_desc* d);
+size_t dbsr_conv3x3_kslice_workspace_bytes(const dbsr_conv_desc* d);
 
 int dbsr_correlation(int n_pairs, int h, int w, int c, dbsr_tensor first, dbsr_tensor second,
                      dbsr_tensor out, int leaky, void* stream);
```

New measurement: 3424 bursts/s, median of 6. About the same (+0.4%).
